# SDFIdk/malstroem

Measured on AMD Instinct MI355X. Metric: Mcells/s fill->D8->accum->label on 16384^2 f32 DEM, higher is better.
Workload: dtype f32 fill / f64 no-flats+D8+accum / u8 flowdir / i32 labels; 1 GPU; 16384x16384 float32 DEM (spectral fBm beta=2 seed 42 (SURVEY 8d recipe)): fill+depths -> no-flats fill -> D8 -> accumulation -> CCL+label_stats -> watersheds+label_count -> pour points; parallelism=1 GPU, one device context, fill_rounds=8, noflat_rounds=85, fill_tiles=70225, fill_visits=43659, fill_cycles=0, noflat_visits=409461, noflat_cycles=409461, nlabels=4637017, fill_algorithm=1, fill_launches=8, noflat_algorithm=2, pour_algorithm=1

## Files before the change

### malstroem_amd/csrc/accum.hip

```cpp
#include "common.hpp"
#include <type_traits>

namespace mh {
namespace {

constexpr int AT = 64;
constexpr int PERIM = 4 * AT - 4;
constexpr int NODE_STRIDE = 256;
constexpr int FS = AT + 32;
constexpr int WOFF = 16;
constexpr uint64_t SRC = 1ull << 63;
constexpr uint64_t TAINT = 1ull << 63;
constexpr uint32_t TAINT32 = 1u << 31;
constexpr int R_SHIFT = 13;
constexpr uint32_t A_MASK = 0x1fffu, R_MASK = 0xfffu, SENT13 = A_MASK;
constexpr uint16_t NO_EXIT = 0xffffu;
#ifndef ACC_ATN
#define ACC_ATN 256
#endif
constexpr int ATN = ACC_ATN;
constexpr int CPT = AT * AT / ATN;
constexpr int MAX_DOUBLINGS = 12;
constexpr int G_SHIFT = 44;
constexpr uint64_t G_ONE = 1ull << G_SHIFT, G_SUM = G_ONE - 1, G_PEND = 0x7ffffull;
// ... 581 lines not shown
{
    const int tile = blockIdx.x;
    if (!touched[tile]) return;
    __shared__ unsigned long long S[AT * AT];
    __shared__ uint16_t P[AT * AT];
    __shared__ uint32_t wl_cell[PERIM + AT * 2];
    __shared__ unsigned long long wl_add[PERIM + AT * 2];
    __shared__ uint32_t wl_n;
    const int ti = tile / ntc, tj = tile - ti * ntc;
    const int64_t r0 = (int64_t)ti * AT, c0 = (int64_t)tj * AT;
    const int tid = threadIdx.x;
    auto halo_row = [&](int64_t rr) { return (fixed_top && rr == 0) || (fixed_bot && rr == H - 1); };
    if (tid == 0) wl_n = 0;
    for (int i = tid; i < AT * AT; i += ATN) {
        const int r = i / AT, c = i - r * AT;
        const int64_t rr = r0 + r, cc = c0 + c;
        const bool inside = rr < H && cc < W;
        const bool owned = inside && !halo_row(rr);
        const double own = owned ? out[rr * W + cc] : 0.0;
        S[i] = own > 0.0 ? (unsigned long long)own : 0ull;
        uint16_t nx = (uint16_t)SENT13;
        const unsigned code = inside ? fd[rr * W + cc] : 8u;
        if (owned && code <= 7u) {
            const int nr = r + dir_dr((int)code), nc = c + dir_dc((int)code);
            if (nr >= 0 && nr < AT && nc >= 0 && nc < AT && (r0 + nr) < H && (c0 + nc) < W && !halo_row(r0 + nr)) nx = (uint16_t)(nr * AT + nc);
        }
        P[i] = nx;
    }
    __syncthreads();
    if (tid < PERIM) {
        const unsigned long long d = nd.inflow[(int64_t)tile * NODE_STRIDE + tid];
        int r, c;
        perim_cell(tid, r, c);
        if (d != 0ull && (r0 + r) < H && (c0 + c) < W && !halo_row(r0 + r)) {
            const uint32_t kk = atomicAdd(&wl_n, 1u);
            wl_cell[kk] = (uint32_t)(r * AT + c);
            wl_add[kk] = d;
        }
    }
    for (int side = 0; side < 2; ++side) {
        const int64_t hr = side == 0 ? 0 : H - 1;
        if ((side == 0 ? !fixed_top : !fixed_bot) || hr < r0 || hr >= r0 + AT) continue;
        if (tid < AT && c0 + tid < W) {
            const int r = (int)(hr - r0), c = tid;
            const unsigned code = fd[hr * W + c0 + c];
            const double X = out[hr * W + c0 + c];
            if (code <= 7u && dir_dr((int)code) != 0 && X > 0.0) {
                const int nr = r + dir_dr((int)code), nc = c + dir_dc((int)code);
                if (nr >= 0 && nr < AT && nc >= 0 && nc < AT && (r0 + nr) < H && (c0 + nc) < W && !halo_row(r0 + nr)) {
                    const uint32_t kk = atomicAdd(&wl_n, 1u);
                    wl_cell[kk] = (uint32_t)(nr * AT + nc);
                    wl_add[kk] = (unsigned long long)X;
                }
            }
        }
    }
    __syncthreads();
    const uint32_t nw = wl_n;
    for (uint32_t w = tid; w < nw; w += ATN) {
        uint32_t a = wl_cell[w];
        const unsigned long long v = wl_add[w];
        do {
            if (S[a] == 0ull) break;
            atomicAdd(&S[a], v);
            a = P[a];
        } while (a != SENT13);
    }
    __syncthreads();
    for (int i = tid; i < AT * AT; i += ATN) {
        const int r = i / AT, c = i - r * AT;
        const int64_t rr = r0 + r, cc = c0 + c;
        if (rr < H && cc < W && !halo_row(rr)) out[rr * W + cc] = (double)S[i];
    }
}
}

int accum_band_delta_dev(const uint8_t *d_fd, double *d_out, int64_t H, int64_t W, hipStream_t s, int fixed_top, int fixed_bot, AccumKeep *keep, bool *done)
{
    *done = false;
    if (!keep || !keep->valid || keep->H != H || keep->W != W || keep->fixed_top != fixed_top || keep->fixed_bot != fixed_bot || !keep->nodes.p) return MHIP_OK;
    static const bool off = [] { const char *e = dev_env("MHIP_BAND_ACC"); return e && std::string(e) == "full"; }();
    if (off) return MHIP_OK;
    const int ntr = (int)cdiv(H, AT), ntc = (int)cdiv(W, AT);
    const int64_t ntiles = (int64_t)ntr * ntc, nnodes = ntiles * NODE_STRIDE;
    char *b = keep->nodes.as<char>();
    Nodes nd;
    nd.gstate = reinterpret_cast<uint64_t *>(b + keep->o[0]);
    nd.inflow = reinterpret_cast<uint64_t *>(b + keep->o[1]);
    nd.arrived = reinterpret_cast<uint32_t *>(b + keep->o[2]);
    nd.next = reinterpret_cast<int32_t *>(b + keep->o[3]);
    nd.dst = reinterpret_cast<int32_t *>(b + keep->o[4]);
    nd.exit_of = reinterpret_cast<uint16_t *>(b + keep->o[5]);
    nd.flags = reinterpret_cast<uint8_t *>(b + keep->o[6]);
    nd.halo_first = reinterpret_cast<int32_t *>(b + keep->o[7]);
    nd.bexit = reinterpret_cast<int32_t *>(b + keep->o[8]);
    DevBuf aux;
    MH_TRY(aux.alloc((size_t)ntiles + 64));
    uint8_t *touched = aux.as<uint8_t>() + 64;
    unsigned int *flag = aux.as<unsigned int>();
    MH_HIP(hipMemsetAsync(aux.p, 0, (size_t)ntiles + 64, s));
    MH_HIP(hipMemsetAsync(nd.inflow, 0, 8 * (size_t)nnodes, s));
    hipLaunchKernelGGL(accum_delta_graph_kernel, dim3((unsigned)cdiv(2 * W, 256)), dim3(256), 0, s, nd, d_fd, (const double *)d_out, H, W, ntc, ntiles, fixed_top,
                       fixed_bot, touched, flag);
    MH_HIP(hipGetLastError());
    unsigned int h_flag = 0;
    MH_HIP(hipMemcpyAsync(&h_flag, flag, 4, hipMemcpyDeviceToHost, s));
    MH_HIP(stream_sync(s));
    keep->valid = false;
    if (h_flag) return MHIP_OK;
    hipLaunchKernelGGL(accum_delta_tile_kernel, dim3((unsigned)ntiles), dim3(ATN), 0, s, d_fd, d_out, H, W, ntc, nd, fixed_top, fixed_bot, (const uint8_t *)touched);
    MH_HIP(hipGetLastError());
    MH_HIP(stream_sync(s));
    *done = true;
    return MHIP_OK;
}

namespace {
struct NodeLayout {
    size_t o_gstate, o_inflow, o_arrived, o_next, o_dst, o_exit, o_flags, o_halo, o_bexit, bytes;
    NodeLayout(int64_t nnodes, int64_t W, bool exit_map)
    {
        auto align = [](size_t x) { return (x + 255) & ~size_t(255); };
        o_gstate = 0; o_inflow = align(o_gstate + 8 * (size_t)nnodes); o_arrived = align(o_inflow + 8 * (size_t)nnodes);
        o_next = align(o_arrived + 4 * (size_t)nnodes); o_dst = align(o_next + 4 * (size_t)nnodes);
        o_exit = align(o_dst + 4 * (size_t)nnodes); o_flags = align(o_exit + 2 * (size_t)nnodes);
        o_halo = align(o_flags + (size_t)nnodes);
        o_bexit = align(o_halo + (exit_map ? 8 * (size_t)W : 0));
        bytes = o_bexit + (exit_map ? 4 * (size_t)nnodes : 0);
    }
};
inline int64_t accum_nodes(int64_t H, int64_t W) { return cdiv(H, AT) * cdiv(W, AT) * NODE_STRIDE; }
}

AccumPrep::~AccumPrep()
{
    if (valid && ready) (void)hipEventSynchronize(ready);
}

int accum_prepare_dev(AccumPrep *prep, int64_t H, int64_t W, hipStream_t s, hipEvent_t ready)
{
    prep->valid = false;
    const int64_t nnodes = accum_nodes(H, W);
    if (nnodes >= (int64_t)INT32_MAX || H * W >= (1ll << 37)) return MHIP_OK;
    const NodeLayout L(nnodes, W, false);
    MH_TRY(prep->nodes.alloc(L.bytes));
    MH_HIP(hipMemsetAsync(prep->nodes.as<char>() + L.o_inflow, 0, L.o_next - L.o_inflow, s));
    MH_HIP(hipEventRecord(ready, s));
    prep->ready = ready; prep->H = H; prep->W = W;
    prep->valid = true;
    return MHIP_OK;
}

int accum_dev(const uint8_t *d_fd, double *d_out, int64_t H, int64_t W, hipStream_t s, int fixed_top, int fixed_bot, int halo_zero,
              int32_t *d_exit_map, PourLink *pour, AccumKeep *keep, AccumPrep *prep)
{
    const int ntr = (int)cdiv(H, AT), ntc = (int)cdiv(W, AT);
    const int64_t ntiles = (int64_t)ntr * ntc, nnodes = ntiles * NODE_STRIDE;
    if (nnodes >= (int64_t)INT32_MAX || H * W >= (1ll << 37)) {
        set_error("accumulated_flow: raster too large for the int32 perimeter-node domain");
        return MHIP_ELIMIT;
    }
    DevBuf buf;
    const NodeLayout L(nnodes, W, d_exit_map != nullptr);
    const size_t o_gstate = L.o_gstate, o_inflow = L.o_inflow, o_arrived = L.o_arrived, o_next = L.o_next, o_dst = L.o_dst, o_exit = L.o_exit,
                 o_flags = L.o_flags, o_halo = L.o_halo, o_bexit = L.o_bexit;
    const bool prepared = prep && prep->valid && prep->H == H && prep->W == W && !d_exit_map && !keep;
    if (prepared) {
        buf.p = prep->nodes.p; buf.bytes = prep->nodes.bytes;
        prep->nodes.p = nullptr; prep->nodes.bytes = 0;
        prep->valid = false;
        MH_HIP(hipStreamWaitEvent(s, prep->ready, 0));
    } else
        MH_TRY(buf.alloc(L.bytes));
    char *b = buf.as<char>();
    Nodes nd;
    nd.gstate = reinterpret_cast<uint64_t *>(b + o_gstate);
    nd.inflow = reinterpret_cast<uint64_t *>(b + o_inflow);
    nd.arrived = reinterpret_cast<uint32_t *>(b + o_arrived);
    nd.next = reinterpret_cast<int32_t *>(b + o_next);
    nd.dst = reinterpret_cast<int32_t *>(b + o_dst);
    nd.exit_of = reinterpret_cast<uint16_t *>(b + o_exit);
    nd.flags = reinterpret_cast<uint8_t *>(b + o_flags);
    nd.halo_first = d_exit_map ? reinterpret_cast<int32_t *>(b + o_halo) : nullptr;
    nd.bexit = d_exit_map ? reinterpret_cast<int32_t *>(b + o_bexit) : nullptr;
    if (d_exit_map) MH_HIP(hipMemsetAsync(nd.halo_first, 0xff, 8 * (size_t)W, s));
    if (!prepared) MH_HIP(hipMemsetAsync(nd.inflow, 0, o_next - o_inflow, s));
    const unsigned gn = (unsigned)cdiv(nnodes, 256);
    const bool walk_final = (!(fixed_top || fixed_bot) || halo_zero) && (!d_exit_map || halo_zero) && H * W < (int64_t)0x7fffffff;
    if (walk_final)
        hipLaunchKernelGGL((accum_tile_kernel<false, false, true>), dim3((unsigned)ntiles), dim3(ATN), 0, s, d_fd, d_out, H, W, ntc, nd, fixed_top, fixed_bot, halo_zero);
    else if ((fixed_top || fixed_bot) && !halo_zero)
        hipLaunchKernelGGL((accum_tile_kernel<false, true>), dim3((unsigned)ntiles), dim3(ATN), 0, s, d_fd, d_out, H, W, ntc, nd, fixed_top, fixed_bot, halo_zero);
    else
        hipLaunchKernelGGL((accum_tile_kernel<false, false>), dim3((unsigned)ntiles), dim3(ATN), 0, s, d_fd, d_out, H, W, ntc, nd, fixed_top, fixed_bot, halo_zero);
    hipLaunchKernelGGL(accum_link_kernel, dim3(gn), dim3(256), 0, s, nd, nnodes);
    if (d_exit_map)
        hipLaunchKernelGGL(accum_band_exit_kernel, dim3((unsigned)cdiv(2 * W, 256)), dim3(256), 0, s, nd, H, W, ntc, ntiles, fixed_top, fixed_bot, d_exit_map);
    hipLaunchKernelGGL(accum_mark_kernel, dim3(gn), dim3(256), 0, s, nd, nnodes);
    hipLaunchKernelGGL(accum_graph_walk_kernel, dim3(gn), dim3(256), 0, s, nd, nnodes);
    if (walk_final) {
        PourCandDev pc;
        if (pour && pour->wait && pour->wait(pour->arg) == 1 && pour->dev.key) {
            MH_HIP(hipStreamWaitEvent(s, pour->ev, 0));
            pc = pour->dev;
            pour->consumed = true;
        }
        hipLaunchKernelGGL(accum_final_walk_kernel, dim3((unsigned)ntiles), dim3(ATN), 0, s, d_fd, d_out, H, W, ntc, nd, pc, fixed_top, fixed_bot);
    }
    else if ((!(fixed_top || fixed_bot) || halo_zero) && H * W < (int64_t)0x7fffffff)
        hipLaunchKernelGGL((accum_tile_kernel<true, false>), dim3((unsigned)ntiles), dim3(ATN), 0, s, d_fd, d_out, H, W, ntc, nd, fixed_top, fixed_bot, halo_zero);
    else
        hipLaunchKernelGGL((accum_tile_kernel<true, true>), dim3((unsigned)ntiles), dim3(ATN), 0, s, d_fd, d_out, H, W, ntc, nd, fixed_top, fixed_bot, halo_zero);
    MH_HIP(hipGetLastError());
    MH_HIP(stream_sync(s));
    if (keep) {
        keep->valid = false;
        if (d_exit_map) {
            keep->nodes.release();
            keep->nodes.p = buf.p; keep->nodes.bytes = buf.bytes;
            buf.p = nullptr; buf.bytes = 0;
            const size_t offs[9] = {o_gstate, o_inflow, o_arrived, o_next, o_dst, o_exit, o_flags, o_halo, o_bexit};
            for (int k = 0; k < 9; ++k) keep->o[k] = offs[k];
            keep->H = H; keep->W = W; keep->fixed_top = fixed_top; keep->fixed_bot = fixed_bot;
            keep->valid = true;
        }
    }
#ifdef MH_PROFILE_ACCUM
    {
        unsigned long long pr[2][8];
        MH_HIP(hipMemcpyFromSymbol(pr, HIP_SYMBOL(g_accum_prof), sizeof(pr)));
        for (int f = 0; f < 2; ++f)
            fprintf(stderr, "[accum profile phase %d] ticks/tile (thread 0): load=%.0f init=%.0f solve=%.0f publish/write=%.0f\n", f ? 3 : 1,
                    pr[f][0] / (double)ntiles, pr[f][1] / (double)ntiles, pr[f][2] / (double)ntiles, pr[f][3] / (double)ntiles);
        unsigned long long z[2][8] = {};
        MH_HIP(hipMemcpyToSymbol(HIP_SYMBOL(g_accum_prof), z, sizeof(z)));
    }
#endif
    return MHIP_OK;
}

}
```

### malstroem_amd/csrc/common.hpp

```cpp
#pragma once
#include <hip/hip_runtime.h>
#include <cstdint>
#include <cstdio>
#include <cstring>
#include <string>
#include <vector>

#include "../../include/malstroem_hip.h"

struct mhip_polygons;
struct mhip_flowpaths;

namespace mh {

void set_error(const char *fmt, ...);
const char *get_error();
const char *dev_env(const char *name);
hipError_t stream_sync(hipStream_t s);
int require_device();

#define MH_HIP(expr)                                                                             \
    do {                                                                                         \
        hipError_t _e = (expr);                                                                  \
        if (_e != hipSuccess) {                                                                  \
            mh::set_error("%s failed: %s (%s:%d)", #expr, hipGetErrorString(_e), __FILE__, __LINE__); \
            return MHIP_EHIP;                                                                    \
        }                                                                                        \
    } while (0)

#define MH_TRY(expr)                \
    do {                            \
        int _rc = (expr);           \
        if (_rc != MHIP_OK) return _rc; \
    } while (0)

#define MH_ARG(cond, msg)                   \
    do {                                    \
        if (!(cond)) {                      \
            mh::set_error("invalid argument: %s", msg); \
            return MHIP_EINVAL;             \
        }                                   \
    } while (0)

int pool_alloc(void **p, size_t bytes);
void pool_free(void *p, size_t bytes);

struct DevBuf {
    void *p = nullptr;
    size_t bytes = 0;
    DevBuf() = default;
    DevBuf(const DevBuf &) = delete;
    DevBuf &operator=(const DevBuf &) = delete;
    ~DevBuf() { release(); }
    int alloc(size_t n)
    {
        if (n == 0) n = 16;
        if (p && bytes >= n && bytes <= 2 * n + 4096) return MHIP_OK;
        release();
        MH_TRY(pool_alloc(&p, n));
        bytes = n;
        return MHIP_OK;
    }
    void release()
    {
        if (p) pool_free(p, bytes);
        p = nullptr;
        bytes = 0;
    }
    template <typename T> T *as() const { return reinterpret_cast<T *>(p); }
};

int upload(DevBuf &b, const void *host, size_t bytes, hipStream_t s);
int download(void *host, const DevBuf &b, size_t bytes, hipStream_t s);
int64_t build_rank_lut(const uint8_t *keep, int64_t nlab, std::vector<int32_t> &lut);
inline bool hyps_res_ok(double res) { return res > 0.0 && res <= 1.7976931348623157e308; }
int trace_on_device(const uint8_t *d_fd, const int32_t *d_lab, int64_t H, int64_t W, const int64_t *cells_rc, int64_t n, int use_bg,
                    int32_t bg, int32_t *out_label, int32_t *out_found, int64_t *out_len, const int64_t *offsets, int64_t *out_cells,
                    hipStream_t s);

__host__ __device__ inline int dir_dr(int k) { return (k == 0 || k == 1 || k == 7) ? -1 : (k >= 3 && k <= 5) ? 1 : 0; }
__host__ __device__ inline int dir_dc(int k) { return (k >= 1 && k <= 3) ? 1 : (k >= 5 && k <= 7) ? -1 : 0; }

__device__ __forceinline__ unsigned d8_code(double z, double u, double ur, double r, double dr, double d, double dl,
                                            double l, double ul)
{
    const double INV_SQRT2 = 0.7071067811865475;
    unsigned i = 8;
    double dzmax = 0.0, dz;
#define MH_D8_STEP(expr, k)          \
    dz = (expr);                     \
    i = dz > dzmax ? (k) : i;        \
    dzmax = fmax(dzmax, dz);
    MH_D8_STEP(__dsub_rn(z, u), 0u)
    MH_D8_STEP(__dmul_rn(__dsub_rn(z, ur), INV_SQRT2), 1u)
    MH_D8_STEP(__dsub_rn(z, r), 2u)
    MH_D8_STEP(__dmul_rn(__dsub_rn(z, dr), INV_SQRT2), 3u)
    MH_D8_STEP(__dsub_rn(z, d), 4u)
    MH_D8_STEP(__dmul_rn(__dsub_rn(z, dl), INV_SQRT2), 5u)
    MH_D8_STEP(__dsub_rn(z, l), 6u)
    MH_D8_STEP(__dmul_rn(__dsub_rn(z, ul), INV_SQRT2), 7u)
#undef MH_D8_STEP
    return i;
}

__device__ __forceinline__ unsigned edge_code(int64_t r, int64_t c, int64_t maxr, int64_t maxc)
{
    unsigned code = 8;
    if (r == 0) code = 0;
    if (r == maxr) code = 4;
    if (c == 0) code = 6;
    if (c == maxc) code = 2;
    if (r == 0 && c == 0) code = 7;
    if (r == 0 && c == maxc) code = 1;
    if (r == maxr && c == 0) code = 5;
    if (r == maxr && c == maxc) code = 3;
    return code;
}

__host__ __device__ inline uint32_t f32_key(float f)
{
    uint32_t u;
    memcpy(&u, &f, 4);
    return (u & 0x80000000u) ? ~u : (u | 0x80000000u);
}
__host__ __device__ inline float key_f32(uint32_t k)
{
    uint32_t u = (k & 0x80000000u) ? (k & 0x7fffffffu) : ~k;
    float f;
    memcpy(&f, &u, 4);
    return f;
}
__device__ __forceinline__ uint32_t dem_key(float v)
{
    if (v != v) return f32_key(__builtin_inff());
    return f32_key(v + 0.0f);
}
__host__ __device__ inline uint64_t f64_key(double f)
{
    uint64_t u;
    memcpy(&u, &f, 8);
    return (u & 0x8000000000000000ull) ? ~u : (u | 0x8000000000000000ull);
}
__host__ __device__ inline double key_f64(uint64_t k)
{
    uint64_t u = (k & 0x8000000000000000ull) ? (k & 0x7fffffffffffffffull) : ~k;
    double f;
    memcpy(&f, &u, 8);
    return f;
}

struct FillStats {
    int32_t rounds = 0;
    int64_t visits = 0;
    int64_t cycles = 0;
    int64_t tiles = 0;
    float hot_ms = 0;
    int32_t hot_launches = 0;
    int32_t algorithm = 0;
    uint32_t overflow = 0;
    bool have_minmax = false, dem_nan = false;
    float dem_min = 0.0f, dem_max = 0.0f;
    int32_t geo_reject = 0;
    int64_t geo_irregular = 0, geo_unreached = 0, geo_mismatch = 0;
};

struct FillRun {
    bool noflat = false;
    const float *dem = nullptr;
    void *out = nullptr;
    int64_t H = 0, W = 0;
    double sh = 0, dg = 0;
    const float *seed = nullptr;
    double seed_add = 0;
    int fixed_top = 0, fixed_bot = 0;
    int rounds_per_batch = 8;
    bool attach_only = false;
    struct Impl;
    Impl *impl;
    FillRun();
    ~FillRun();
    FillRun(const FillRun &) = delete;
    FillRun &operator=(const FillRun &) = delete;
    int begin(hipStream_t s, bool *active);
    int batch(hipStream_t s, bool *active);
    int activate_row(int side, hipStream_t s);
    int attach(hipStream_t s);
    int certify(hipStream_t s, bool *changed);
    int finish(hipStream_t s, FillStats *st);
};
void noflat_seed(FillRun &f, const float *d_filled, double sh, double dg, int64_t ncells_global);
struct PfRun;
struct FillHandover {
    PfRun *run = nullptr;
    const float *dem = nullptr;
    float *filled = nullptr, *depths = nullptr;
    int64_t H = 0, W = 0;
    const uint16_t *bslot = nullptr;
    const uint32_t *tabV = nullptr;
    int ntr = 0, ntc = 0;
    bool pending = false, queued = false, violated = false, repaired = false;
    bool suspect = false;
    FillStats st_repair;
    FillHandover() = default;
    FillHandover(const FillHandover &) = delete;
    FillHandover &operator=(const FillHandover &) = delete;
    ~FillHandover();
    void release();
};
int fill_handover_complete(FillHandover *ho, hipStream_t s);
int fill_handover_repair(FillHandover *ho, hipStream_t s);
int fill_plain_dev(const float *d_dem, float *d_out, int64_t H, int64_t W, hipStream_t s, FillStats *st, float *d_depths = nullptr,
                   bool *depths_done = nullptr, FillHandover *ho = nullptr);
int fill_check_f32_dev(const float *d_dem, const float *d_filled, int64_t H, int64_t W, int fixed_top, int fixed_bot, hipStream_t s,
                       unsigned int *d_flag);
int fill_plain_pflood_dev(const float *d_dem, float *d_out, float *d_depths, int64_t H, int64_t W, hipStream_t s, FillStats *st, bool *violated = nullptr,
                          uint32_t *overflow = nullptr, FillHandover *ho = nullptr);
struct PfRun {
    const float *dem = nullptr;
    float *out = nullptr;
    int64_t H = 0, W = 0;
    int fixed_top = 0, fixed_bot = 0;
    uint32_t overflow = 0;
    struct Impl;
    Impl *impl;
    PfRun();
    ~PfRun();
    PfRun(const PfRun &) = delete;
    PfRun &operator=(const PfRun &) = delete;
    int begin(hipStream_t s);
    int halo_changed(int side, hipStream_t s);
    int batch(hipStream_t s);
    int finish(hipStream_t s, float *d_depths, FillStats *st, bool *violated = nullptr, FillHandover *ho = nullptr);
    int finish_late(hipStream_t s, float *d_depths, bool *violated);
    int proof_flag(hipStream_t s, unsigned int *h_flag);
    int solve(hipStream_t s);
    int pack(hipStream_t s, int row0, int nrows);
    int publish_edges(hipStream_t s);
};
struct StageHook {
    enum Point { FIRST_VISIT = 0, TAIL_ROUNDS = 1, FINISH = 3 };
    void (*fn)(void *, hipStream_t) = nullptr;
    void *arg = nullptr;
    bool fired = false;
    int at = TAIL_ROUNDS;
    void fire(hipStream_t s)
    {
        if (fn && !fired) {
            fired = true;
            fn(arg, s);
        }
    }
    void fire_at(int point, hipStream_t s)
    {
        if (point == at) fire(s);
    }
};

struct GeoRun {
    const float *dem = nullptr, *filled = nullptr;
    double *out = nullptr;
    uint32_t *dist = nullptr;
    int64_t H = 0, W = 0;
    double sh = 0, dg = 0;
    int fixed_top = 0, fixed_bot = 0;
    bool allow_partial = false;
    double seed_add = 0;
    bool partial = false;
    StageHook *tail_hook = nullptr;
    uint8_t *d8_out = nullptr;
    unsigned int *d8_nodir = nullptr;
    bool d8_done = false;
    bool defer_out = false;
    bool out_deferred = false;
    FillHandover *handover = nullptr;
    struct Impl;
    Impl *impl;
    GeoRun();
    ~GeoRun();
    GeoRun(const GeoRun &) = delete;
    GeoRun &operator=(const GeoRun &) = delete;
    int begin(hipStream_t s, bool *applicable, bool *active);
    int batch(hipStream_t s, bool *active);
    int halo_changed(int side, hipStream_t s);
    int end(hipStream_t s, bool *ok, FillStats *st);
    int launch_rounds(hipStream_t s, int nb);
};
struct D8Sink {
    uint8_t *flowdir = nullptr;
    unsigned int *nodir = nullptr;
    bool done = false;
    uint32_t *dist = nullptr;
    bool defer = false, deferred = false;
};
int noflat_assemble_dev(const float *d_filled, const uint32_t *d_dist, double *d_out, int64_t n, double seed_add, hipStream_t s);
int fill_noflat_geodesic_dev(const float *d_dem, const float *d_filled, double *d_out, int64_t H, int64_t W, double sh, double dg, double seed_add,
                             hipStream_t s, FillStats *st, bool *partial, StageHook *tail_hook = nullptr, D8Sink *d8 = nullptr, FillHandover *ho = nullptr);
int noflat_verify_dev(const float *d_dem, const double *d_out, int64_t H, int64_t W, double sh, double dg, hipStream_t s, bool *ok, int fixed_top = 0,
                      int fixed_bot = 0);
int fill_noflat_dev(const float *d_dem, double *d_out, int64_t H, int64_t W, double sh, double dg, hipStream_t s,
                    FillStats *st = nullptr, const float *d_filled = nullptr, StageHook *tail_hook = nullptr, D8Sink *d8 = nullptr,
                    FillHandover *ho = nullptr);
int short_diag_dev(const float *d_dem, int64_t n, double *sh, double *dg, hipStream_t s);
int depths_dev(const float *d_filled, const float *d_dem, float *d_out, int64_t n, hipStream_t s);
int d8_dev(const double *d_z, uint8_t *d_out, int64_t H, int64_t W, int edges_outward, hipStream_t s, int64_t row_off = 0,
           int64_t Hg = 0, unsigned int *d_interior_nodir = nullptr);
void short_diag_from_minmax(float mn, float mx, bool has_nan, double *sh, double *dg);
int minmax_dev(const float *d_x, int64_t n, float *mn, float *mx, int *has_nan, hipStream_t s);
int row_update_dev(void *d_dst, const void *d_src, int64_t nbytes, int *changed, hipStream_t s);
int copy_bandwidth_dev(size_t bytes, int reps, double *gbs, hipStream_t s);
int read_bandwidth_dev(size_t bytes, int reps, double *gbs, hipStream_t s);
int row_update_async(void *d_dst, const void *d_src, int64_t nbytes, int *d_changed, hipStream_t s);
int trace_downstream_dev(const uint8_t *d_fd, const int32_t *d_lab, int64_t H, int64_t W, const int64_t *d_cells, int64_t n, int use_bg,
                         int32_t bg, int32_t *d_label, int32_t *d_found, int64_t *d_len, const int64_t *d_offsets, int64_t *d_out_cells,
                         hipStream_t s);
int comm_unique_id(void *id128);
int comm_available();
int comm_create(void **comm, const void *id128, int rank, int nranks);
void comm_destroy(void *comm);
int comm_exchange_rows(void *comm, int rank, int nranks, const void *first_row, const void *last_row, void *stage, size_t rowbytes,
                       hipStream_t s);
int comm_allreduce_max(void *comm, double *d_value, hipStream_t s);
struct PourCandDev {
    uint16_t *mask0 = nullptr;
    uint2 *list = nullptr;
    uint32_t *tile_cnt = nullptr;
    unsigned long long *tile_key0 = nullptr;
    uint32_t *flags = nullptr;
    int components = 0;
    unsigned long long *key = nullptr;
    uint32_t nlab = 0;
};
constexpr uint32_t POUR_TILE_CAP = 512;
struct PourLink {
    PourCandDev dev;
    hipEvent_t ev = nullptr;
    void (*notify)(void *, int) = nullptr;
    int (*wait)(void *) = nullptr;
    void *arg = nullptr;
    bool consumed = false;
};
struct AccumKeep {
    DevBuf nodes;
    size_t o[9] = {};
    int64_t H = 0, W = 0;
    int fixed_top = 0, fixed_bot = 0;
    bool valid = false;
};
struct AccumPrep {
    DevBuf nodes;
    int64_t H = 0, W = 0;
    hipEvent_t ready = nullptr;
    bool valid = false;
    ~AccumPrep();
};
int accum_prepare_dev(AccumPrep *prep, int64_t H, int64_t W, hipStream_t s, hipEvent_t ready);
int accum_dev(const uint8_t *d_fd, double *d_out, int64_t H, int64_t W, hipStream_t s, int fixed_top = 0, int fixed_bot = 0, int halo_zero = 0,
              int32_t *d_exit_map = nullptr, PourLink *pour = nullptr, AccumKeep *keep = nullptr, AccumPrep *prep = nullptr);
int accum_band_delta_dev(const uint8_t *d_fd, double *d_out, int64_t H, int64_t W, hipStream_t s, int fixed_top, int fixed_bot, AccumKeep *keep, bool *done);
int ccl8_f32_dev(const float *d_data, int32_t *d_labels, int32_t *d_tmp, int64_t H, int64_t W, int64_t *nlabels,
                 hipStream_t s, DevBuf *stats_out = nullptr);
int label_emit_stats_dev(const int32_t *d_parent, const unsigned long long *d_rootbits, const uint32_t *d_wordprefix, const float *d_data,
                         int32_t *d_labels, int64_t H, int64_t W, int64_t nlab, mhip_stat_record *d_rec, hipStream_t s);
int ccl8_u8_dev(const uint8_t *d_data, int32_t *d_labels, int32_t *d_tmp, int64_t H, int64_t W, int64_t *nlabels,
                hipStream_t s);
struct CclKeep {
    DevBuf bits, wprefix;
    int64_t H = 0, W = 0, nlocal = 0;
    bool valid = false;
};
int ccl8_f32_begin_dev(const float *d_data, int32_t *d_labels, int32_t *d_tmp, int64_t H, int64_t W, int64_t *nlabels, hipStream_t s, CclKeep *keep);
int ccl_emit_rows_dev(const int32_t *d_parent, const unsigned long long *d_rootbits, const uint32_t *d_wordprefix, int32_t *d_labels, int64_t base,
                      int64_t count, hipStream_t s);
int label_emit_sparse_dev(const int32_t *d_parent, const unsigned long long *d_rootbits, const uint32_t *d_wordprefix, const float *d_data,
                          int32_t *d_labels, int64_t H, int64_t W, int ht, int64_t H_owned, int64_t nlocal, int32_t offset,
                          const int32_t *d_dropped, const int32_t *d_target, int32_t ndropped, int64_t nlab_global, mhip_stat_record *d_rec,
                          hipStream_t s);
int relabel_lut_dev(int32_t *d_labels, const int32_t *d_lut, int64_t nlab, int64_t n, hipStream_t s);
int relabel_range_dev(int32_t *d_labels, int64_t n, int32_t lo, int32_t hi, const int32_t *d_lut, const int32_t *d_fid, const int32_t *d_fnew, int32_t nf,
                      hipStream_t s);
int band_trace_dev(const uint8_t *d_fd, const int32_t *d_lab, int64_t Hl, int64_t W, int64_t row_lo, int64_t own0, int64_t own1, int64_t Hg,
                   const int64_t *d_cells, const int32_t *d_src, int64_t n, int use_bg, int32_t bg, int32_t *d_label, int32_t *d_status,
                   int32_t *d_src_out, int64_t *d_exit, int64_t *d_len, const int64_t *d_offsets, int64_t *d_out_cells, hipStream_t s);
int relabel_sparse_dev(int32_t *d_labels, int64_t n, int64_t nlocal, int32_t offset, const int32_t *d_dropped, const int32_t *d_target,
                       int32_t ndropped, hipStream_t s);
int keep_mask_dev(const int32_t *d_labels, const uint8_t *d_keep, int64_t nlab, int64_t n, uint8_t *d_mask,
                  hipStream_t s);
int label_stats_dev(const float *d_data, const int32_t *d_labels, int64_t n, int64_t nlab, mhip_stat_record *d_rec,
                    hipStream_t s, int64_t W = 0, bool components = false);
int label_stats64_dev(const double *d_data, const int32_t *d_labels, int64_t n, int64_t nlab, mhip_stat_record *d_rec, hipStream_t s);
int label_stats_zero_sign_dev(const float *d_data, const int32_t *d_labels, int64_t n, int64_t nlab, mhip_stat_record *d_rec, hipStream_t s);
int label_stats_zero_sign_dev(const double *d_data, const int32_t *d_labels, int64_t n, int64_t nlab, mhip_stat_record *d_rec, hipStream_t s);
int label_arg_dev(const double *d_data, const int32_t *d_labels, int64_t H, int64_t W, int64_t nlab, bool is_max,
                  mhip_index_record *d_rec, hipStream_t s, bool components = false);
int label_count_dev(const int32_t *d_labels, int64_t n, int64_t nlab, int64_t *d_counts, hipStream_t s, int64_t W = 0);
int label_max_dev(const int32_t *d_labels, int64_t n, int32_t *out_max, hipStream_t s);
constexpr int64_t HYPS_MAX_BINS = (int64_t)1 << 30;
int hyps_layout_dev(const double *d_dmax, int64_t stride, int64_t nlab, double res, int64_t *d_offsets, int64_t *total, hipStream_t s);
int hyps_table_dev(const float *d_data, const int32_t *d_labels, int64_t n, int64_t W, int64_t nlab, double res, const int64_t *d_offsets,
                   int64_t total, uint32_t *d_counts, double *d_sums, int64_t *lds_spills, hipStream_t s, hipEvent_t ev0 = nullptr,
                   hipEvent_t ev1 = nullptr);
int hyps_levels_dev(int64_t nlab, const int64_t *d_offsets, const uint32_t *d_counts, const double *d_sums, const double *d_dmax, int64_t stride,
                    const double *d_q, mhip_final_record *d_rec, hipStream_t s);
int final_depths_dev(const float *d_data, const int32_t *d_labels, int64_t n, int64_t W, int64_t nlab, mhip_final_record *d_rec, float *d_out,
                     hipStream_t s, hipEvent_t ev0 = nullptr, hipEvent_t ev1 = nullptr);
bool wet_at_events_ok(int64_t K, const float *values);
int wet_at_dev(const float *d_data, const int32_t *d_labels, int64_t n, int64_t W, int64_t nlab, int K, const double *d_drawdown, int64_t stride,
               const float *values, float *d_out, int64_t *d_wet, int64_t wet_stride, hipStream_t s, hipEvent_t ev0 = nullptr,
               hipEvent_t ev1 = nullptr);
bool flow_distance_scale_ok(double scale);
int flow_distance_dev(const uint8_t *d_fd, const int32_t *d_lab, int64_t H, int64_t W, double scale, int64_t nlab, float *d_out, mhip_index_record *d_rec,
                      int64_t *unresolved, hipStream_t s);
int fdist_jumps_dev(uint4 *&cur, uint4 *&nxt, int64_t W, int64_t ntc, int64_t ntiles, unsigned int *d_open, hipStream_t s);
int hand_check(double threshold, double scale);
int hand_dev(const uint8_t *d_fd, const double *d_acc, const float *d_elev, const int32_t *d_lab, int64_t H, int64_t W, double threshold, double scale,
             float nodata, float *d_hand, float *d_dist, int64_t *undrained, hipStream_t s);
int burn_check(int64_t nseg, const mhip_burn_segment *segs, int64_t nline, const mhip_burn_line *lines, const mhip_burn_result *results);
int burn_lines_dev(float *d_dem, int64_t H, int64_t W, int64_t nseg, const mhip_burn_segment *segs, int64_t nline, const mhip_burn_line *lines,
                   double nodata, mhip_burn_result *results, hipStream_t s);
int zones_check(int64_t H, int64_t W, int64_t nvert, const double *xy, int64_t nring, const int64_t *ring_offsets, const int32_t *ring_zone,
                int64_t nzone, int grow);
int zones_rasterize_dev(int32_t *d_out, int64_t H, int64_t W, int64_t nvert, const double *xy, int64_t nring, const int64_t *ring_offsets,
                        const int32_t *ring_zone, int64_t nzone, int grow, hipStream_t s);
int zone_stats_dev(const float *d_data, const int32_t *d_zones, int64_t n, int64_t W, int64_t nzone, mhip_zone_record *d_rec, hipStream_t s);
int polygonize_check(int64_t H, int64_t W);
int polygons_fetch_dev(const mhip_polygons *p, int32_t *xy, int64_t *ring_offsets, int32_t *ring_label);
int polygonize_dev(const int32_t *d_lab, int64_t H, int64_t W, DevBuf &d_xy, DevBuf &d_off, DevBuf &d_rl, int64_t *nring, int64_t *nvert, hipStream_t s);
int flowpaths_check(int64_t H, int64_t W, double threshold);
int flowpaths_dev(const uint8_t *d_fd, const double *d_acc, const int32_t *d_lab, int64_t H, int64_t W, double threshold, mhip_flowpaths *p, hipStream_t s);
int flowpaths_fetch_dev(const mhip_flowpaths *p, int32_t *xy, int64_t *reach_offsets, mhip_reach_record *records);
int watersheds_dev(const uint8_t *d_fd, int32_t *d_labels, int64_t H, int64_t W, int32_t unassigned, hipStream_t s,
                   bool band_mode = false, const unsigned int *d_known_interior_nodir = nullptr, const int32_t *d_src = nullptr, PourLink *pour = nullptr);
int pour_finish_dev(unsigned long long *d_key, const unsigned long long *d_tile_key0, int64_t ntiles, int64_t nlab, int64_t W, mhip_index_record *d_rec,
                    hipStream_t s);
int band_pseudo_labels_dev(int32_t *d_ws, int64_t H, int64_t W, int top, int bottom, hipStream_t s);
int negative_lut_dev(int32_t *d_lab, int64_t n, const int32_t *d_lut, int64_t nlut, hipStream_t s);
constexpr int32_t BAND_ROOT = 1, BAND_ROOTLESS = 0x7fffffff;
int band_root_labels_dev(int32_t *d_out, int64_t H, int64_t W, int64_t row_off, int64_t Hg, hipStream_t s);
int band_hide_rootless_dev(const int32_t *d_lab, const int32_t *d_rooted, int32_t *d_out, int64_t n, hipStream_t s);
int band_show_rootless_dev(int32_t *d_ws, const int32_t *d_lab, int64_t n, hipStream_t s);

__host__ __device__ inline int64_t cdiv(int64_t a, int64_t b) { return (a + b - 1) / b; }

constexpr int TR = 32;
struct TileGeom {
    int64_t n, W;
    int64_t ntr, ntc;
};
__host__ __device__ inline TileGeom tile_geom(int64_t n, int64_t W)
{
    TileGeom g;
    g.n = n;
    g.W = (W > 0 && n % W == 0) ? W : 256;
    const int64_t H = cdiv(n, g.W);
    g.ntr = cdiv(H, TR);
    g.ntc = cdiv(g.W, 256);
    return g;
}
inline unsigned tile_grid(const TileGeom &g)
{
    const int64_t nt = g.ntr * g.ntc;
    return (unsigned)(nt < 2048 ? (nt > 0 ? nt : 1) : 2048);
}

#ifdef __HIPCC__
__device__ __forceinline__ int64_t downstream(const uint8_t *fd, int64_t i, int64_t H, int64_t W)
{
    const unsigned code = fd[i];
    if (code > 7u) return -1;
    const int64_t r = i / W, c = i - r * W;
    const int64_t nr = r + dir_dr((int)code), nc = c + dir_dc((int)code);
    if (nr < 0 || nr >= H || nc < 0 || nc >= W) return -1;
    return nr * W + nc;
}
constexpr int WS_TILE = 64;
__device__ __forceinline__ int ws_perim_slot(int lr, int lc)
{
    if (lr == 0) return lc;
    if (lr == WS_TILE - 1) return WS_TILE + lc;
    if (lc == 0) return 2 * WS_TILE + (lr - 1);
    if (lc == WS_TILE - 1) return 2 * WS_TILE + (WS_TILE - 2) + (lr - 1);
    return -1;
}
__device__ __forceinline__ int64_t ws_node_of(int32_t cell, uint32_t W, int ntc)
{
    const uint32_t r = (uint32_t)cell / W, c = (uint32_t)cell - r * W;
    const int slot = ws_perim_slot((int)(r & 63u), (int)(c & 63u));
    return slot < 0 ? -1 : (int64_t)((r >> 6) * (uint32_t)ntc + (c >> 6)) * 256 + slot;
}

constexpr int32_t FD_NONE = 0x7fffffff;
constexpr int32_t FD_DONE = (int32_t)0x80000000;
constexpr double FD_SQRT2 = 1.4142135623730951;
__device__ __forceinline__ uint32_t fd_step(unsigned code) { return (code & 1u) ? 0x10000u : 1u; }
__device__ __forceinline__ bool fd_resolve(uint2 s, const uint4 *__restrict__ Nn, uint32_t W, int ntc, uint32_t &no, uint32_t &nd, int32_t &T)
{
    int32_t t = (int32_t)s.x;
    no = s.y & 0xffffu;
    nd = s.y >> 16;
    if (t >= 0 && t != FD_NONE) {
        const int64_t node = ws_node_of(t, W, ntc);
        uint4 m = make_uint4((uint32_t)FD_NONE, 0u, 0u, 0u);
        if (node >= 0) m = Nn[node];
        t = (int32_t)m.x;
        no += m.y;
        nd += m.z;
    }
    T = t & ~FD_DONE;
    return t < 0;
}
__device__ __forceinline__ double fd_u(uint32_t no, uint32_t nd) { return __dadd_rn((double)no, __dmul_rn((double)nd, FD_SQRT2)); }
// ... 53 lines not shown
```

### malstroem_amd/csrc/ctx.hip

```cpp
#include <mutex>
#include <new>
#include <string>
#include <vector>

#include "ctx.hpp"

namespace mh {

static void drop_hyps(mhip_ctx *c)
{
    c->hyps_total = -1;
    c->have[MHIP_R_FINALDEPTHS] = false;
    c->wetat_events = -1;
    c->wetat_out.release();
}

static void drop_flow_distance(mhip_ctx *c)
{
    std::lock_guard<std::mutex> lk(c->fdist_mu);
    c->fdist_unresolved = -1;
    c->fdist_out.release();
    c->fdist_rec.release();
}

// ... 55 lines not shown
        break;
    }
}

int ctx_copy_rows(mhip_ctx *c, void *dev_base, size_t elem_bytes, int64_t row0, int64_t nrows, void *host, hipMemcpyKind kind)
{
    MH_HIP(hipSetDevice(c->device));
    const size_t rowb = elem_bytes * (size_t)c->W;
    char *dev = (char *)dev_base + rowb * (size_t)(c->ht + row0);
    const bool up = kind == hipMemcpyHostToDevice;
    MH_HIP(hipMemcpyAsync(up ? (void *)dev : host, up ? host : (void *)dev, rowb * (size_t)nrows, kind, cs(c)));
    MH_HIP(stream_sync(cs(c)));
    return MHIP_OK;
}

int ctx_noflat(mhip_ctx *c, double **g)
{
    if (c->noflat_pending) {
        MH_HIP(hipSetDevice(c->device));
        MH_TRY(noflat_assemble_dev(c->r[MHIP_R_FILLED].as<float>(), c->r[MHIP_R_NGDIST].as<uint32_t>(), c->r[MHIP_R_NOFLAT].as<double>(), c->H * c->W, 0.0,
                                   c->stream));
        c->noflat_pending = false;
        if (cs(c) != c->stream) MH_HIP(stream_sync(c->stream));
    }
    if (g) *g = c->r[MHIP_R_NOFLAT].as<double>();
    return MHIP_OK;
}

int ctx_fetch(mhip_ctx *c, const DevBuf &buf, size_t bytes, void *host)
{
    MH_HIP(hipSetDevice(c->device));
    return download(host, buf, bytes, c->stream);
}

int ctx_fork_join_events(mhip_ctx *c)
{
    if (c->ev_fork) return MHIP_OK;
    for (hipEvent_t *e : {&c->ev_flowdir, &c->ev_join, &c->ev_label, &c->ev_tail, &c->ev_fork}) MH_HIP(hipEventCreateWithFlags(e, hipEventDisableTiming));
    return MHIP_OK;
}

int ctx_ensure_labels_final(mhip_ctx *c, hipStream_t s)
{
    if (!c->labels_filtered) return ctx_apply_keep_on(c, nullptr, s);
    return MHIP_OK;
}

int ctx_label_max(mhip_ctx *c, hipStream_t s)
{
    if (c->nlabels < 0) {
        int32_t m = 0;
        MH_TRY(label_max_dev(c->r[MHIP_R_LABELS].as<int32_t>(), c->H * c->W, &m, s));
        c->nlabels = m < 0 ? 0 : m;
    }
    return MHIP_OK;
}

int ctx_apply_keep_on(mhip_ctx *c, const uint8_t *keep, hipStream_t s)
{
    MH_ARG(c && c->have[MHIP_R_LABELS] && c->nlabels_raw >= 0 && !c->labels_filtered, "ctx_apply_keep needs a fresh LABEL run");
    const int64_t n = c->H * c->W;
    const int64_t nraw = c->nlabels_raw;
    const bool components = c->labels_components;
    ctx_wrote(c, MHIP_R_LABELS);
    c->nlabels_raw = nraw;
    c->labels_components = components;
    if (keep) {
        std::vector<int32_t> lut;
        c->nlabels = build_rank_lut(keep, c->nlabels_raw, lut);
        DevBuf d_lut;
        MH_TRY(d_lut.alloc(lut.size() * 4));
        MH_HIP(hipMemcpyAsync(d_lut.p, lut.data(), lut.size() * 4, hipMemcpyHostToDevice, s));
        MH_TRY(relabel_lut_dev(c->r[MHIP_R_LABELS].as<int32_t>(), d_lut.as<int32_t>(), c->nlabels_raw, n, s));
        MH_TRY(c->stats.alloc(sizeof(mhip_stat_record) * (size_t)(c->nlabels + 1)));
        MH_TRY(label_stats_dev(c->r[MHIP_R_DEPTHS].as<float>(), c->r[MHIP_R_LABELS].as<int32_t>(), n, c->nlabels,
                               c->stats.as<mhip_stat_record>(), s, c->W, c->labels_components));
    } else {
        c->nlabels = c->nlabels_raw;
        MH_TRY(c->stats.alloc(sizeof(mhip_stat_record) * (size_t)(c->nlabels + 1)));
        MH_HIP(hipMemcpyAsync(c->stats.p, c->raw_stats.p, sizeof(mhip_stat_record) * (size_t)(c->nlabels + 1),
                              hipMemcpyDeviceToDevice, s));
    }
    c->labels_filtered = true;
    c->stats_valid = true;
    return MHIP_OK;
}

}

using namespace mh;

extern "C" {

int mhip_comm_available(void) { return comm_available(); }

int mhip_comm_unique_id(void *id128)
{
    MH_ARG(id128, "comm_unique_id(id128)");
    MH_TRY(require_device());
    return comm_unique_id(id128);
}

int mhip_ctx_create_band(mhip_ctx **out, int64_t H_global, int64_t W, int64_t row0, int64_t H_local, int device, int rank,
                         int nranks, const void *nccl_unique_id)
{
    MH_ARG(out && H_global >= 1 && W >= 1 && H_local >= 1 && row0 >= 0 && row0 + H_local <= H_global, "ctx_create_band geometry");
    MH_ARG(rank >= 0 && nranks >= 1 && rank < nranks, "ctx_create_band(rank, nranks)");
    MH_TRY(require_device());
    MH_HIP(hipSetDevice(device));
    void *comm = nullptr;
    if (nccl_unique_id) MH_TRY(comm_create(&comm, nccl_unique_id, rank, nranks));
    mhip_ctx *c = new mhip_ctx();
    c->comm = comm;
    c->ht = row0 > 0 ? 1 : 0;
    c->hb = row0 + H_local < H_global ? 1 : 0;
    c->H_owned = H_local;
    c->H = H_local + c->ht + c->hb;
    c->W = W; c->H_global = H_global; c->row0 = row0;
    c->device = device; c->rank = rank; c->nranks = nranks;
    int prio_least = 0, prio_greatest = 0;
    (void)hipDeviceGetStreamPriorityRange(&prio_least, &prio_greatest);
    if (hipStreamCreateWithPriority(&c->stream, hipStreamDefault, prio_greatest) != hipSuccess) {
        comm_destroy(c->comm);
        delete c;
        set_error("hipStreamCreate failed");
        return MHIP_EHIP;
    }
    *out = c;
    return MHIP_OK;
}

int mhip_ctx_create(mhip_ctx **out, int64_t H, int64_t W, int device)
{
    return mhip_ctx_create_band(out, H, W, 0, H, device, 0, 1, nullptr);
}

int mhip_ctx_destroy(mhip_ctx *c)
{
    if (!c) return MHIP_OK;
    (void)hipSetDevice(c->device);
    (void)stream_sync(c->stream);
    for (StageTimer &t : c->timers)
        for (hipEvent_t e : {t.a, t.b})
            if (e) (void)hipEventDestroy(e);
    (void)hipStreamDestroy(c->stream);
    for (hipStream_t st : {c->stream_b, c->stream_c}) {
        if (st) {
            (void)stream_sync(st);
            (void)hipStreamDestroy(st);
        }
    }
    for (hipEvent_t e : {c->ev_fork, c->ev_flowdir, c->ev_join, c->ev_label, c->ev_tail, c->ev_cand, c->ev_prep})
        if (e) (void)hipEventDestroy(e);
    delete c->geo;
    delete c->pf;
    delete c->run[0];
    delete c->run[1];
    comm_destroy(c->comm);
    comm_destroy(c->comm_b);
    delete c;
    return MHIP_OK;
}

int mhip_ctx_comm_add_side(mhip_ctx *c, const void *nccl_unique_id)
{
    MH_ARG(c && nccl_unique_id && c->comm && !c->comm_b, "ctx_comm_add_side(ctx, id) needs a band context with a communicator and no side communicator yet");
    MH_HIP(hipSetDevice(c->device));
    return comm_create(&c->comm_b, nccl_unique_id, c->rank, c->nranks);
}

int mhip_ctx_side_begin(mhip_ctx *c)
{
    MH_ARG(c, "ctx");
    MH_HIP(hipSetDevice(c->device));
    if (!c->stream_b) MH_HIP(hipStreamCreateWithFlags(&c->stream_b, hipStreamNonBlocking));
    MH_TRY(ctx_fork_join_events(c));
    MH_HIP(hipEventRecord(c->ev_fork, c->stream));
    MH_HIP(hipStreamWaitEvent(c->stream_b, c->ev_fork, 0));
    t_side_ctx = c;
    return MHIP_OK;
}

int mhip_ctx_side_end(mhip_ctx *c)
{
    MH_ARG(c && t_side_ctx == c, "ctx_side_end without ctx_side_begin on this thread");
    MH_HIP(hipSetDevice(c->device));
    MH_HIP(stream_sync(c->stream_b));
    t_side_ctx = nullptr;
    return MHIP_OK;
}

int mhip_ctx_upload(mhip_ctx *c, int which, const void *host)
{
    MH_ARG(c && host && which >= 0 && which < MHIP_R_COUNT_, "ctx_upload(ctx, which, host)");
    return mhip_ctx_upload_rows(c, which, 0, c->H_owned, host);
}

int mhip_ctx_upload_dem(mhip_ctx *c, const float *dem) { return mhip_ctx_upload(c, MHIP_R_DEM, dem); }

int mhip_ctx_upload_rows(mhip_ctx *c, int which, int64_t row0, int64_t nrows, const void *host)
{
    MH_ARG(c && host && which >= 0 && which < MHIP_R_COUNT_ && row0 >= 0 && nrows >= 1 && row0 + nrows <= c->H_owned,
           "ctx_upload_rows(ctx, which, row0, nrows, host)");
    MH_HIP(hipSetDevice(c->device));
    MH_TRY(ctx_raster(c, which));
    MH_TRY(ctx_settle(c, which, true));
    ctx_wrote(c, which, true);
    c->have[which] = false;
    MH_TRY(ctx_copy_rows(c, c->r[which].p, raster_elem(which), row0, nrows, const_cast<void *>(host), hipMemcpyHostToDevice));
    if (row0 + nrows == c->H_owned) {
        c->have[which] = true;
        if (which == MHIP_R_LABELS) c->labels_filtered = true;
    }
    return MHIP_OK;
}

int mhip_ctx_download_rows(mhip_ctx *c, int which, int64_t row0, int64_t nrows, void *host)
{
    MH_ARG(c && host && which >= 0 && which < MHIP_R_COUNT_ && row0 >= 0 && nrows >= 1 && row0 + nrows <= c->H_owned,
           "ctx_download_rows(ctx, which, row0, nrows, host)");
    MH_ARG(c->have[which], "raster has not been computed or uploaded");
    MH_TRY(ctx_settle(c, which, false));
    return ctx_copy_rows(c, c->r[which].p, raster_elem(which), row0, nrows, host, hipMemcpyDeviceToHost);
}

int mhip_ctx_download(mhip_ctx *c, int which, void *host)
{
    MH_ARG(c && host && which >= 0 && which < MHIP_R_COUNT_, "ctx_download(ctx, which, host)");
    return mhip_ctx_download_rows(c, which, 0, c->H_owned, host);
}

int mhip_ctx_trace_downstream(mhip_ctx *c, const int64_t *cells_rc, int64_t n, int use_background, int32_t background, int32_t *out_label,
                              int32_t *out_found, int64_t *out_len, const int64_t *offsets, int64_t *out_cells)
{
    MH_ARG(c && n >= 0 && (n == 0 || cells_rc), "ctx_trace_downstream(ctx, cells, n, ...)");
    MH_ARG(c->have[MHIP_R_FLOWDIR] && c->have[MHIP_R_LABELS], "ctx_trace_downstream needs flow directions and labels");
    MH_ARG(!c->ht && !c->hb, "stream tracing runs on an undivided raster");
    if (n == 0) return MHIP_OK;
    MH_HIP(hipSetDevice(c->device));
    return trace_on_device(c->r[MHIP_R_FLOWDIR].as<uint8_t>(), c->r[MHIP_R_LABELS].as<int32_t>(), c->H, c->W, cells_rc, n, use_background,
                           background, out_label, out_found, out_len, offsets, out_cells, c->stream);
}

int mhip_ctx_sync(mhip_ctx *c)
{
    MH_ARG(c, "ctx");
    MH_HIP(stream_sync(c->stream));
    return MHIP_OK;
}

int mhip_ctx_stage_ms(mhip_ctx *c, int stage, float *ms)
{
    MH_ARG(c && ms, "ctx_stage_ms(ctx, stage, ms)");
    const int k = timer_slot(stage);
    MH_ARG(k >= 0 && c->timers[k].valid, "stage has not been run");
    MH_HIP(hipEventSynchronize(c->timers[k].b));
    MH_HIP(hipEventElapsedTime(ms, c->timers[k].a, c->timers[k].b));
    return MHIP_OK;
}

int mhip_ctx_kernel_ms(mhip_ctx *c, const char *kernel, float *ms_total, int32_t *launches)
{
    MH_ARG(c && kernel && ms_total && launches, "ctx_kernel_ms(ctx, kernel, ms, launches)");
    const std::string k(kernel);
    if (k == "d8") {
        *launches = 1;
        return mhip_ctx_stage_ms(c, MHIP_STAGE_FLOWDIR, ms_total);
    }
    if (k == "d8_steady") {
        MH_ARG(c->have[MHIP_R_NOFLAT] && !c->ht && !c->hb, "d8_steady needs the no-flats surface on an undivided context");
        MH_HIP(hipSetDevice(c->device));
        double *g = nullptr;
        MH_TRY(ctx_noflat(c, &g));
        MH_TRY(ctx_raster(c, MHIP_R_FLOWDIR));
        MH_TRY(c->nodir_cnt.alloc(4));
        constexpr int REPS = 16;
        StageTimer *t;
        MH_TRY(ctx_timer(c, D8_STEADY_SLOT, &t));
        hipStream_t s = c->stream;
        ctx_wrote(c, MHIP_R_FLOWDIR);
        MH_HIP(hipMemsetAsync(c->nodir_cnt.p, 0, 4, s));
        for (int i = 0; i < REPS + 2; ++i) {
            if (i == 2) MH_HIP(hipEventRecord(t->a, s));
            MH_TRY(d8_dev(g, c->r[MHIP_R_FLOWDIR].as<uint8_t>(), c->H, c->W, 1, s, 0, c->H_global, c->nodir_cnt.as<unsigned int>()));
        }
        MH_HIP(hipEventRecord(t->b, s));
        MH_HIP(hipEventSynchronize(t->b));
        MH_HIP(hipEventElapsedTime(ms_total, t->a, t->b));
        c->have[MHIP_R_FLOWDIR] = true;
        c->nodir_valid = true;
        c->flowdir_own = true;
        *launches = REPS;
        return MHIP_OK;
    }
    if (k == "hyps_table" || k == "final_depths") {
        *launches = 1;
        return mhip_ctx_stage_ms(c, k == "hyps_table" ? HYPS_KERNEL_SLOT : FINAL_KERNEL_SLOT, ms_total);
    }
    if (k == "wet_at") {
        *launches = 1;
        return mhip_ctx_stage_ms(c, WETAT_KERNEL_SLOT, ms_total);
    }
    if (k == "fill_round") {
        *launches = c->fill_rounds;
        return mhip_ctx_stage_ms(c, MHIP_STAGE_FILL, ms_total);
    }
    if (k == "noflat_round") {
        *launches = c->noflat_rounds;
        return mhip_ctx_stage_ms(c, MHIP_STAGE_NOFLAT, ms_total);
    }
    set_error("unknown kernel family '%s'", kernel);
    return MHIP_EINVAL;
}

int mhip_ctx_get_i64(mhip_ctx *c, const char *key, int64_t *value)
{
    MH_ARG(c && key && value, "ctx_get_i64(ctx, key, value)");
    const std::string k(key);
    if (k == "nlabels_raw") *value = c->nlabels_raw;
    else if (k == "nlabels") {
        if (c->nlabels < 0 && c->have[MHIP_R_LABELS]) {
            MH_HIP(hipSetDevice(c->device));
            MH_TRY(ctx_label_max(c, c->stream));
        }
        *value = c->nlabels;
    }
    else if (k == "fill_rounds") *value = c->fill_rounds;
    else if (k == "noflat_rounds") *value = c->noflat_rounds;
    else if (k == "fill_visits") *value = c->fill_st.visits;
    else if (k == "fill_cycles") *value = c->fill_st.cycles;
    else if (k == "fill_tiles") *value = c->fill_st.tiles;
    else if (k == "fill_algorithm") *value = c->fill_st.algorithm;
    else if (k == "fill_handover") *value = c->fill_handover;
    else if (k == "fill_handover_rechecks") *value = c->fill_handover_rechecks;
    else if (k == "fill_overflow") *value = c->fill_st.overflow;
    else if (k == "fill_launches") *value = c->fill_st.rounds;
    else if (k == "fill_hot_launches") *value = c->fill_st.hot_launches;
    else if (k == "noflat_hot_launches") *value = c->noflat_st.hot_launches;
    else if (k == "accum_algorithm") *value = c->accum_algorithm;
    else if (k == "flowdir_computed") *value = (c->have[MHIP_R_FLOWDIR] && c->flowdir_own) ? 1 : 0;
    else if (k == "pour_algorithm") *value = c->pour_algorithm;
    else if (k == "noflat_algorithm") *value = c->noflat_st.algorithm;
    else if (k == "noflat_pending") *value = c->noflat_pending ? 1 : 0;
    else if (k == "noflat_visits") *value = c->noflat_st.visits;
    else if (k == "noflat_reject") *value = c->noflat_st.geo_reject;
    else if (k == "noflat_reject_irregular") *value = c->noflat_st.geo_irregular;
    else if (k == "noflat_reject_unreached") *value = c->noflat_st.geo_unreached;
    else if (k == "noflat_reject_mismatch") *value = c->noflat_st.geo_mismatch;
    else if (k == "noflat_cycles") *value = c->noflat_st.cycles;
    else if (k == "hyps_bins") *value = c->hyps_total;
    else if (k == "hyps_lds_spills") *value = c->hyps_spills;
    else if (k == "wet_at_events") *value = c->wetat_events;
    else if (k == "flow_distance_unresolved") *value = c->fdist_unresolved;
    else if (k == "hand_undrained") *value = c->hand_undrained;
    else if (k == "zones") *value = c->nzone;
    else if (k == "H") *value = c->H;
    else if (k == "W") *value = c->W;
    else {
        set_error("unknown key '%s'", key);
        return MHIP_EINVAL;
    }
    return MHIP_OK;
}

int mhip_ctx_get_f64(mhip_ctx *c, const char *key, double *value)
{
    MH_ARG(c && key && value, "ctx_get_f64(ctx, key, value)");
    const std::string k(key);
    if (k == "short") *value = c->sh;
    else if (k == "diag") *value = c->dg;
    else if (k == "fill_hot_ms") *value = c->fill_st.hot_ms;
    else if (k == "noflat_hot_ms") *value = c->noflat_st.hot_ms;
    else {
        set_error("unknown key '%s'", key);
        return MHIP_EINVAL;
    }
    return MHIP_OK;
}

int mhip_ctx_raw_stats(mhip_ctx *c, mhip_stat_record *records)
{
    MH_ARG(c && records && c->raw_stats.p && c->nlabels_raw >= 0, "ctx_raw_stats needs a LABEL run");
    return ctx_fetch(c, c->raw_stats, sizeof(mhip_stat_record) * (size_t)(c->nlabels_raw + 1), records);
}

int mhip_ctx_apply_keep(mhip_ctx *c, const uint8_t *keep)
{
    MH_ARG(c, "ctx");
    MH_HIP(hipSetDevice(c->device));
    return ctx_apply_keep_on(c, keep, c->stream);
}

int mhip_ctx_stats(mhip_ctx *c, mhip_stat_record *records)
{
    MH_ARG(c && records && c->stats_valid && c->labels_filtered, "ctx_stats needs LABEL + apply_keep (or mhip_ctx_hyps) on the resident depths and labels");
    return ctx_fetch(c, c->stats, sizeof(mhip_stat_record) * (size_t)(c->nlabels + 1), records);
}

int mhip_ctx_watershed_counts(mhip_ctx *c, int64_t *counts)
{
    MH_ARG(c && counts && c->ws_counts_valid, "ctx_watershed_counts needs a WATERSHED run on the resident labels");
    return ctx_fetch(c, c->ws_counts, 8 * (size_t)(c->nlabels + 1), counts);
}

int mhip_ctx_pourpoints(mhip_ctx *c, mhip_index_record *records)
{
    MH_ARG(c && records && c->pour_valid, "ctx_pourpoints needs a POURPOINTS run on the resident labels and accumulated flow");
    return ctx_fetch(c, c->pour, sizeof(mhip_index_record) * (size_t)(c->nlabels + 1), records);
}

int mhip_ctx_hyps(mhip_ctx *c, double res, int64_t *total)
{
    MH_ARG(c && total && hyps_res_ok(res), "ctx_hyps(ctx, 0 < res < inf, total)");
    MH_ARG(!(c->nranks > 1 || c->ht || c->hb), "hypsometry on a row band is not built (the tables of the bands add up: a later step); use an undivided context");
    MH_ARG(c->have[MHIP_R_DEPTHS] && c->have[MHIP_R_LABELS] && !c->ccl_pending, "ctx_hyps needs the DEPTHS and LABELS rasters");
    MH_ARG(c->labels_filtered, "ctx_hyps needs mhip_ctx_apply_keep after the LABEL run");
    MH_HIP(hipSetDevice(c->device));
    hipStream_t s = c->stream;
    const int64_t n = c->H * c->W;
    c->hyps_total = -1;
    if (!c->stats_valid) {
        MH_TRY(ctx_label_max(c, s));
        MH_TRY(c->stats.alloc(sizeof(mhip_stat_record) * (size_t)(c->nlabels + 1)));
        MH_TRY(label_stats_dev(c->r[MHIP_R_DEPTHS].as<float>(), c->r[MHIP_R_LABELS].as<int32_t>(), n, c->nlabels, c->stats.as<mhip_stat_record>(), s,
                               c->W, c->labels_components));
        c->stats_valid = true;
    }
    const int64_t nlab = c->nlabels;
    MH_TRY(c->hyps_off.alloc(8 * (size_t)(nlab + 2)));
    StageTimer *k;
    MH_TRY(ctx_timer(c, HYPS_KERNEL_SLOT, &k));
    MH_TRY(stage_begin(c, MHIP_STAGE_HYPS, s));
    int64_t tot = 0;
    MH_TRY(hyps_layout_dev(c->stats.as<double>() + 1, 4, nlab, res, c->hyps_off.as<int64_t>(), &tot, s));
    MH_TRY(c->hyps_cnt.alloc(4 * (size_t)tot));
    MH_TRY(c->hyps_sum.alloc(8 * (size_t)tot));
    MH_TRY(hyps_table_dev(c->r[MHIP_R_DEPTHS].as<float>(), c->r[MHIP_R_LABELS].as<int32_t>(), n, c->W, nlab, res, c->hyps_off.as<int64_t>(), tot,
                          c->hyps_cnt.as<uint32_t>(), c->hyps_sum.as<double>(), &c->hyps_spills, s, k->a, k->b));
    MH_TRY(stage_end(c, MHIP_STAGE_HYPS, s));
    k->valid = true;
    c->hyps_total = tot;
    *total = tot;
    return MHIP_OK;
}

int mhip_ctx_hyps_fetch(mhip_ctx *c, int64_t *offsets, int64_t *counts, double *sums)
{
    MH_ARG(c && offsets && counts && sums, "ctx_hyps_fetch(ctx, offsets, counts, sums)");
    MH_ARG(c->hyps_total >= 0, "ctx_hyps_fetch needs mhip_ctx_hyps on the resident depths and labels");
    MH_HIP(hipSetDevice(c->device));
    hipStream_t s = c->stream;
    const size_t tot = (size_t)c->hyps_total;
    std::vector<uint32_t> c32(tot + 1);
    MH_HIP(hipMemcpyAsync(offsets, c->hyps_off.p, 8 * (size_t)(c->nlabels + 2), hipMemcpyDeviceToHost, s));
    if (tot) {
        MH_HIP(hipMemcpyAsync(c32.data(), c->hyps_cnt.p, 4 * tot, hipMemcpyDeviceToHost, s));
        MH_HIP(hipMemcpyAsync(sums, c->hyps_sum.p, 8 * tot, hipMemcpyDeviceToHost, s));
    }
    MH_HIP(stream_sync(s));
    for (size_t k = 0; k < tot; ++k) counts[k] = (int64_t)c32[k];
    return MHIP_OK;
}

int mhip_ctx_final_depths(mhip_ctx *c, const double *q, mhip_final_record *records)
{
    MH_ARG(c && q && records, "ctx_final_depths(ctx, q, records)");
    MH_ARG(c->hyps_total >= 0 && c->stats_valid, "ctx_final_depths needs mhip_ctx_hyps on the resident depths and labels");
    MH_HIP(hipSetDevice(c->device));
    hipStream_t s = c->stream;
    const int64_t nlab = c->nlabels, n = c->H * c->W;
    DevBuf d_q;
    MH_TRY(upload(d_q, q, 8 * (size_t)(nlab + 1), s));
    MH_TRY(c->hyps_rec.alloc(sizeof(mhip_final_record) * (size_t)(nlab + 1)));
    MH_TRY(ctx_raster(c, MHIP_R_FINALDEPTHS));
    c->have[MHIP_R_FINALDEPTHS] = false;
    StageTimer *k;
    MH_TRY(ctx_timer(c, FINAL_KERNEL_SLOT, &k));
    MH_TRY(stage_begin(c, MHIP_STAGE_FINALDEPTHS, s));
    MH_TRY(hyps_levels_dev(nlab, c->hyps_off.as<int64_t>(), c->hyps_cnt.as<uint32_t>(), c->hyps_sum.as<double>(), c->stats.as<double>() + 1, 4,
                           d_q.as<double>(), c->hyps_rec.as<mhip_final_record>(), s));
    MH_TRY(final_depths_dev(c->r[MHIP_R_DEPTHS].as<float>(), c->r[MHIP_R_LABELS].as<int32_t>(), n, c->W, nlab, c->hyps_rec.as<mhip_final_record>(),
                            c->r[MHIP_R_FINALDEPTHS].as<float>(), s, k->a, k->b));
    MH_TRY(stage_end(c, MHIP_STAGE_FINALDEPTHS, s));
    k->valid = true;
    c->have[MHIP_R_FINALDEPTHS] = true;
    return ctx_fetch(c, c->hyps_rec, sizeof(mhip_final_record) * (size_t)(nlab + 1), records);
}
// ... 230 lines not shown
```

### malstroem_amd/csrc/ctx.hpp

```cpp
#pragma once
#include <atomic>
#include <condition_variable>
#include <functional>
#include <mutex>
#include <thread>

#include "common.hpp"

namespace mh {

class SideThread {
    std::thread th_;
    std::mutex mu_;
    std::condition_variable cv_;
    std::function<void()> task_;
    bool busy_ = false, stop_ = false;

public:
    ~SideThread()
    {
        {
            std::lock_guard<std::mutex> lk(mu_);
            stop_ = true;
        }
        cv_.notify_all();
        if (th_.joinable()) th_.join();
    }
    void run(std::function<void()> f)
    {
        std::unique_lock<std::mutex> lk(mu_);
        if (!th_.joinable())
            th_ = std::thread([this] {
                std::unique_lock<std::mutex> l2(mu_);
                for (;;) {
                    cv_.wait(l2, [this] { return stop_ || (busy_ && task_); });
                    if (stop_) return;
                    std::function<void()> f2 = std::move(task_);
                    task_ = nullptr;
                    l2.unlock();
                    f2();
                    l2.lock();
                    busy_ = false;
                    cv_.notify_all();
                }
            });
        task_ = std::move(f);
        busy_ = true;
        cv_.notify_all();
    }
    void wait()
    {
        std::unique_lock<std::mutex> lk(mu_);
        cv_.wait(lk, [this] { return !busy_; });
    }
};

struct StageTimer {
    hipEvent_t a = nullptr, b = nullptr;
    bool valid = false;
};
constexpr int N_STAGE_BITS = 9;
constexpr int WETAT_KERNEL_SLOT = 1 << 27, FINAL_KERNEL_SLOT = 1 << 28, HYPS_KERNEL_SLOT = 1 << 29, D8_STEADY_SLOT = 1 << 30;
constexpr int N_TIMERS = N_STAGE_BITS + 4;

}

struct mhip_ctx {
    mh::SideThread side;
    int64_t H = 0, W = 0;
    int64_t H_global = 0, row0 = 0, H_owned = 0;
    int ht = 0, hb = 0;
    mh::FillRun *run[2] = {nullptr, nullptr};
    mh::GeoRun *geo = nullptr;
    uint32_t pf_overflow = 0;
    mh::PfRun *pf = nullptr;
    bool pf_done = false;
    mh::DevBuf nodir_cnt;
    bool nodir_valid = false;
    bool flowdir_own = false;
    int device = 0, rank = 0, nranks = 1;
    hipStream_t stream = nullptr;
    mh::DevBuf r[MHIP_R_COUNT_];
    bool have[MHIP_R_COUNT_] = {};
    bool noflat_pending = false;
    mh::DevBuf tmp_i32;
    mh::CclKeep ccl_keep;
    bool ccl_pending = false;
    bool pf_depths = false;
    mh::DevBuf raw_stats, stats, ws_counts, pour;
    mh::AccumKeep acc_keep;
    int accum_algorithm = 0;
    mh::DevBuf pp_mask0, pp_list, pp_tiles, pp_misc, pp_key;
    hipEvent_t ev_cand = nullptr;
    hipEvent_t ev_prep = nullptr;
    int pour_algorithm = 0;
    int64_t nlabels_raw = -1, nlabels = -1;
    bool labels_components = false;
    bool labels_filtered = false;
    std::atomic<bool> stats_valid{false};
    std::atomic<bool> ws_counts_valid{false};
    std::atomic<bool> pour_valid{false};
    mh::DevBuf hyps_off, hyps_cnt, hyps_sum, hyps_rec;
    int64_t hyps_total = -1, hyps_spills = 0;
    mh::DevBuf wetat_out;
    int wetat_events = -1;
    mh::DevBuf fdist_out, fdist_rec;
    std::atomic<int64_t> fdist_unresolved{-1};
    std::mutex fdist_mu;
    mh::DevBuf hand_out, hand_dist;
    std::atomic<int64_t> hand_undrained{-1};
    int hand_src = -1;
    bool hand_labels = false;
    std::mutex hand_mu;
    mh::DevBuf zones;
    int64_t nzone = -1;
    double sh = 0, dg = 0;
    int32_t fill_rounds = 0, noflat_rounds = 0;
    int64_t fill_handover_rechecks = 0;
    int32_t fill_handover = 0;
    mh::FillStats fill_st, noflat_st;
    mh::StageTimer timers[mh::N_TIMERS];
    void *comm = nullptr;
    void *comm_b = nullptr;
    mh::DevBuf comm_stage, comm_word, comm_flags, comm_stage_b;
    hipStream_t stream_b = nullptr, stream_c = nullptr;
    hipEvent_t ev_fork = nullptr, ev_flowdir = nullptr, ev_join = nullptr, ev_label = nullptr, ev_tail = nullptr;
};

namespace mh {

inline size_t raster_elem(int which)
{
    switch (which) {
    case MHIP_R_DEM: case MHIP_R_FILLED: case MHIP_R_DEPTHS: case MHIP_R_LABELS: case MHIP_R_WATERSHEDS: case MHIP_R_NGDIST:
    case MHIP_R_FINALDEPTHS: return 4;
    case MHIP_R_NOFLAT: case MHIP_R_ACCUM: return 8;
    case MHIP_R_FLOWDIR: return 1;
    default: return 0;
    }
}

inline int ctx_raster(mhip_ctx *c, int which)
{
    if (!c->r[which].p) MH_TRY(c->r[which].alloc(raster_elem(which) * (size_t)(c->H * c->W)));
    return MHIP_OK;
}

inline int timer_slot(int stage)
{
    for (int b = 0; b < N_STAGE_BITS; ++b)
        if (stage == 1 << b) return b;
    return stage == FINAL_KERNEL_SLOT ? N_STAGE_BITS : stage == HYPS_KERNEL_SLOT ? N_STAGE_BITS + 1 : stage == D8_STEADY_SLOT ? N_STAGE_BITS + 2 :
           stage == WETAT_KERNEL_SLOT ? N_STAGE_BITS + 3 : -1;
}
inline int ctx_timer(mhip_ctx *c, int stage, StageTimer **t)
{
    const int k = timer_slot(stage);
    MH_ARG(k >= 0, "not a stage");
    *t = &c->timers[k];
    if (!(*t)->a) {
        hipEvent_t e0, e1;
        MH_HIP(hipEventCreate(&e0));
        MH_HIP(hipEventCreate(&e1));
        (*t)->a = e0;
        (*t)->b = e1;
    }
    return MHIP_OK;
}
inline int stage_begin(mhip_ctx *c, int stage, hipStream_t s)
{
    StageTimer *t;
    MH_TRY(ctx_timer(c, stage, &t));
    MH_HIP(hipEventRecord(t->a, s));
    return MHIP_OK;
}
inline int stage_end(mhip_ctx *c, int stage, hipStream_t s)
{
    StageTimer &t = c->timers[timer_slot(stage)];
    MH_HIP(hipEventRecord(t.b, s));
    t.valid = true;
    return MHIP_OK;
}

inline thread_local mhip_ctx *t_side_ctx = nullptr;
static inline hipStream_t cs(mhip_ctx *c) { return (t_side_ctx == c && c->stream_b) ? c->stream_b : c->stream; }
static inline bool on_side(mhip_ctx *c) { return t_side_ctx == c; }

void ctx_wrote(mhip_ctx *c, int which, bool uploaded = false);
int ctx_noflat(mhip_ctx *c, double **g = nullptr);
inline int ctx_settle(mhip_ctx *c, int which, bool write)
{
    if (which == MHIP_R_NOFLAT || (write && (which == MHIP_R_FILLED || which == MHIP_R_NGDIST))) return ctx_noflat(c);
    return MHIP_OK;
}
int ctx_copy_rows(mhip_ctx *c, void *dev_base, size_t elem_bytes, int64_t row0, int64_t nrows, void *host, hipMemcpyKind kind);
int ctx_fetch(mhip_ctx *c, const DevBuf &buf, size_t bytes, void *host);
int ctx_fork_join_events(mhip_ctx *c);
int ctx_apply_keep_on(mhip_ctx *c, const uint8_t *keep, hipStream_t s);
int ctx_ensure_labels_final(mhip_ctx *c, hipStream_t s);
int ctx_label_max(mhip_ctx *c, hipStream_t s);

}
```

### malstroem_amd/csrc/ctx_run.hip

```cpp
#include <atomic>
#include <future>
#include <string>

#include "ctx.hpp"

using namespace mh;

constexpr int LABEL_START_DEFAULT = 3;
constexpr int FILL_HANDOVER_DEFAULT = 1;
constexpr int NOFLAT_LAZY_DEFAULT = 1;

static bool fill_handover_env()
{
    const char *e = dev_env("MHIP_FILL_HANDOVER");
    return e ? e[0] != '0' : FILL_HANDOVER_DEFAULT != 0;
}

static bool noflat_lazy_env()
{
    const char *e = dev_env("MHIP_NOFLAT_LAZY");
    return e ? e[0] != '0' : NOFLAT_LAZY_DEFAULT != 0;
}

static int stage_depths(mhip_ctx *c, hipStream_t s)
{
    MH_ARG(c->have[MHIP_R_FILLED] && c->have[MHIP_R_DEM], "depths need the filled surface");
    MH_TRY(ctx_raster(c, MHIP_R_DEPTHS));
    MH_TRY(depths_dev(c->r[MHIP_R_FILLED].as<float>(), c->r[MHIP_R_DEM].as<float>(), c->r[MHIP_R_DEPTHS].as<float>(), c->H * c->W, s));
    ctx_wrote(c, MHIP_R_DEPTHS);
    c->have[MHIP_R_DEPTHS] = true;
    return MHIP_OK;
}

static int stage_fill(mhip_ctx *c, hipStream_t s, bool with_depths = true, FillHandover *ho = nullptr)
{
    const int64_t H = c->H, W = c->W;
    MH_ARG(c->have[MHIP_R_DEM], "FILL needs the DEM");
    MH_TRY(ctx_raster(c, MHIP_R_FILLED));
    MH_TRY(ctx_raster(c, MHIP_R_DEPTHS));
    MH_TRY(stage_begin(c, MHIP_STAGE_FILL, s));
    FillStats st;
    bool depths_done = false;
    MH_TRY(fill_plain_dev(c->r[MHIP_R_DEM].as<float>(), c->r[MHIP_R_FILLED].as<float>(), H, W, s, &st, c->r[MHIP_R_DEPTHS].as<float>(),
                          &depths_done, ho));
    ctx_wrote(c, MHIP_R_FILLED);
    ctx_wrote(c, MHIP_R_DEPTHS);
    const bool owed = ho && ho->pending;
    c->have[MHIP_R_FILLED] = !owed;
    c->have[MHIP_R_DEPTHS] = depths_done && !owed;
    if (with_depths && !depths_done) MH_TRY(stage_depths(c, s));
    MH_TRY(stage_end(c, MHIP_STAGE_FILL, s));
    c->fill_rounds = st.rounds;
    c->fill_st = st;
    return MHIP_OK;
}

static void ctx_handover_settled(mhip_ctx *c, FillHandover *ho)
{
    if (!ho || ho->pending || c->have[MHIP_R_FILLED]) return;
    c->have[MHIP_R_FILLED] = true;
    c->have[MHIP_R_DEPTHS] = true;
    c->fill_handover = ho->queued ? 1 : 0;
    if (ho->suspect) ++c->fill_handover_rechecks;
    if (ho->repaired) {
        c->fill_st.algorithm = 4;
        c->fill_st.rounds += ho->st_repair.rounds;
        c->fill_st.visits += ho->st_repair.visits;
        c->fill_st.cycles += ho->st_repair.cycles;
        c->fill_rounds = c->fill_st.rounds;
    }
}

static int stage_noflat(mhip_ctx *c, hipStream_t s, bool shdg_done = false, StageHook *tail_hook = nullptr, bool with_flowdir = false,
                        bool *flowdir_done = nullptr, FillHandover *ho = nullptr)
{
    const int64_t H = c->H, W = c->W, n = H * W;
    MH_ARG(c->have[MHIP_R_DEM], "NOFLAT needs the DEM");
    MH_TRY(ctx_raster(c, MHIP_R_NOFLAT));
    c->noflat_pending = false;
    MH_TRY(stage_begin(c, MHIP_STAGE_NOFLAT, s));
    if (!shdg_done) {
        if ((c->have[MHIP_R_FILLED] || (ho && ho->pending)) && c->fill_st.have_minmax) short_diag_from_minmax(c->fill_st.dem_min, c->fill_st.dem_max, c->fill_st.dem_nan, &c->sh, &c->dg);
        else MH_TRY(short_diag_dev(c->r[MHIP_R_DEM].as<float>(), n, &c->sh, &c->dg, s));
    }
    FillStats st;
    if (!c->have[MHIP_R_FILLED] && !(ho && ho->pending)) {
        MH_TRY(ctx_raster(c, MHIP_R_FILLED));
        FillStats st0;
        MH_TRY(fill_plain_dev(c->r[MHIP_R_DEM].as<float>(), c->r[MHIP_R_FILLED].as<float>(), H, W, s, &st0));
        ctx_wrote(c, MHIP_R_FILLED);
        c->have[MHIP_R_FILLED] = true;
    }
    D8Sink d8;
    static const bool fuse_d8 = [] { const char *e = dev_env("MHIP_D8_FUSE"); return !(e && e[0] == '0'); }();
    if (with_flowdir && fuse_d8 && !c->ht && !c->hb) {
        MH_TRY(ctx_raster(c, MHIP_R_FLOWDIR));
        MH_TRY(c->nodir_cnt.alloc(4));
        MH_HIP(hipMemsetAsync(c->nodir_cnt.p, 0, 4, s));
        d8.flowdir = c->r[MHIP_R_FLOWDIR].as<uint8_t>();
        d8.nodir = c->nodir_cnt.as<unsigned int>();
        if (c->nranks == 1 && noflat_lazy_env()) {
            MH_TRY(ctx_raster(c, MHIP_R_NGDIST));
            d8.dist = c->r[MHIP_R_NGDIST].as<uint32_t>();
            d8.defer = true;
        }
    }
    const int rc_nf = fill_noflat_dev(c->r[MHIP_R_DEM].as<float>(), c->r[MHIP_R_NOFLAT].as<double>(), H, W, c->sh, c->dg, s, &st,
                                      c->r[MHIP_R_FILLED].as<float>(), tail_hook, d8.flowdir ? &d8 : nullptr, ho);
    ctx_handover_settled(c, ho);
    MH_TRY(rc_nf);
    if (flowdir_done) *flowdir_done = d8.done;
    MH_TRY(stage_end(c, MHIP_STAGE_NOFLAT, s));
    c->noflat_rounds = st.rounds;
    c->noflat_st = st;
    ctx_wrote(c, MHIP_R_NOFLAT);
    c->have[MHIP_R_NOFLAT] = true;
    c->noflat_pending = d8.deferred;
    return MHIP_OK;
}

static int stage_flowdir(mhip_ctx *c, hipStream_t s)
{
    MH_ARG(c->have[MHIP_R_NOFLAT], "FLOWDIR needs the no-flats surface");
    double *g = nullptr;
    MH_TRY(ctx_noflat(c, &g));
    MH_TRY(ctx_raster(c, MHIP_R_FLOWDIR));
    MH_TRY(stage_begin(c, MHIP_STAGE_FLOWDIR, s));
    ctx_wrote(c, MHIP_R_FLOWDIR);
    MH_TRY(c->nodir_cnt.alloc(4));
    MH_HIP(hipMemsetAsync(c->nodir_cnt.p, 0, 4, s));
    MH_TRY(d8_dev(g, c->r[MHIP_R_FLOWDIR].as<uint8_t>(), c->H, c->W, 1, s, c->row0 - c->ht, c->H_global, c->nodir_cnt.as<unsigned int>()));
    MH_TRY(stage_end(c, MHIP_STAGE_FLOWDIR, s));
    c->have[MHIP_R_FLOWDIR] = true;
    c->flowdir_own = true;
    c->nodir_valid = !c->ht && !c->hb;
    return MHIP_OK;
}

static int stage_flowdir_fused(mhip_ctx *c, hipStream_t s)
{
    MH_TRY(stage_begin(c, MHIP_STAGE_FLOWDIR, s));
    MH_TRY(stage_end(c, MHIP_STAGE_FLOWDIR, s));
    ctx_wrote(c, MHIP_R_FLOWDIR);
    c->have[MHIP_R_FLOWDIR] = true;
    c->nodir_valid = true;
    c->flowdir_own = true;
    return MHIP_OK;
}

static int stage_accum(mhip_ctx *c, hipStream_t s, PourLink *pour = nullptr, AccumPrep *prep = nullptr)
{
    MH_ARG(c->have[MHIP_R_FLOWDIR], "ACCUM needs flow directions");
    MH_TRY(ctx_raster(c, MHIP_R_ACCUM));
    MH_TRY(stage_begin(c, MHIP_STAGE_ACCUM, s));
    bool delta_done = false;
    if ((c->ht || c->hb) && c->acc_keep.valid)
        MH_TRY(accum_band_delta_dev(c->r[MHIP_R_FLOWDIR].as<uint8_t>(), c->r[MHIP_R_ACCUM].as<double>(), c->H, c->W, s, c->ht, c->hb, &c->acc_keep, &delta_done));
    c->accum_algorithm = delta_done ? 1 : 0;
    ctx_wrote(c, MHIP_R_ACCUM);
    if (!delta_done)
        MH_TRY(accum_dev(c->r[MHIP_R_FLOWDIR].as<uint8_t>(), c->r[MHIP_R_ACCUM].as<double>(), c->H, c->W, s, c->ht, c->hb, 0, nullptr, pour, nullptr,
                         prep));
    MH_TRY(stage_end(c, MHIP_STAGE_ACCUM, s));
    c->have[MHIP_R_ACCUM] = true;
    return MHIP_OK;
}

static int stage_label(mhip_ctx *c, hipStream_t s)
{
    const int64_t H = c->H, W = c->W, n = H * W;
    MH_ARG(c->have[MHIP_R_DEPTHS] || c->have[MHIP_R_FILLED], "LABEL needs bluespot depths");
    MH_TRY(ctx_raster(c, MHIP_R_LABELS));
    if (!c->tmp_i32.p) MH_TRY(c->tmp_i32.alloc(4 * (size_t)n));
    MH_TRY(stage_begin(c, MHIP_STAGE_LABEL, s));
    if (!c->have[MHIP_R_DEPTHS]) MH_TRY(stage_depths(c, s));
    ctx_wrote(c, MHIP_R_LABELS);
    MH_TRY(ccl8_f32_dev(c->r[MHIP_R_DEPTHS].as<float>(), c->r[MHIP_R_LABELS].as<int32_t>(), c->tmp_i32.as<int32_t>(), H, W,
                        &c->nlabels_raw, s, &c->raw_stats));
    MH_TRY(stage_end(c, MHIP_STAGE_LABEL, s));
    c->have[MHIP_R_LABELS] = true;
    c->labels_components = true;
    c->labels_filtered = false;
    c->nlabels = c->nlabels_raw;
    return MHIP_OK;
}

static int pour_link_buffers(mhip_ctx *c, PourLink *pl, hipStream_t s)
{
    const int64_t H = c->H, W = c->W;
    const int64_t ntiles = cdiv(H, 64) * cdiv(W, 64);
    MH_TRY(c->pp_mask0.alloc(2 * 256 * (size_t)ntiles));
    MH_TRY(c->pp_list.alloc(8 * (size_t)POUR_TILE_CAP * (size_t)ntiles));
    MH_TRY(c->pp_tiles.alloc(12 * (size_t)ntiles));
    MH_TRY(c->pp_misc.alloc(16));
    MH_TRY(c->pp_key.alloc(8 * (size_t)(c->nlabels + 1)));
    MH_HIP(hipMemsetAsync(c->pp_misc.p, 0, 16, s));
    MH_HIP(hipMemsetAsync(c->pp_key.p, 0, 8 * (size_t)(c->nlabels + 1), s));
    pl->dev.mask0 = c->pp_mask0.as<uint16_t>();
    pl->dev.list = c->pp_list.as<uint2>();
    pl->dev.tile_key0 = c->pp_tiles.as<unsigned long long>();
    pl->dev.tile_cnt = reinterpret_cast<uint32_t *>(c->pp_tiles.as<unsigned long long>() + ntiles);
    pl->dev.flags = c->pp_misc.as<uint32_t>() + 1;
    pl->dev.components = c->labels_components ? 1 : 0;
    pl->dev.key = c->pp_key.as<unsigned long long>();
    pl->dev.nlab = (uint32_t)c->nlabels;
    pl->ev = c->ev_cand;
    return MHIP_OK;
}

static int stage_watershed(mhip_ctx *c, hipStream_t s, PourLink *pour = nullptr)
{
    const int64_t H = c->H, W = c->W, n = H * W;
    MH_ARG(c->have[MHIP_R_LABELS] && c->have[MHIP_R_FLOWDIR], "WATERSHED needs labels and flow directions");
    MH_TRY(ctx_ensure_labels_final(c, s));
    MH_TRY(ctx_label_max(c, s));
    MH_TRY(ctx_raster(c, MHIP_R_WATERSHEDS));
    MH_TRY(stage_begin(c, MHIP_STAGE_WATERSHED, s));
    ctx_wrote(c, MHIP_R_WATERSHEDS);
    if (pour) MH_TRY(pour_link_buffers(c, pour, s));
    MH_TRY(watersheds_dev(c->r[MHIP_R_FLOWDIR].as<uint8_t>(), c->r[MHIP_R_WATERSHEDS].as<int32_t>(), H, W, 0, s, false,
                          c->nodir_valid ? c->nodir_cnt.as<unsigned int>() : nullptr, c->r[MHIP_R_LABELS].as<int32_t>(), pour));
    MH_TRY(c->ws_counts.alloc(8 * (size_t)(c->nlabels + 1)));
    MH_TRY(label_count_dev(c->r[MHIP_R_WATERSHEDS].as<int32_t>(), n, c->nlabels, c->ws_counts.as<int64_t>(), s, W));
    MH_TRY(stage_end(c, MHIP_STAGE_WATERSHED, s));
    c->have[MHIP_R_WATERSHEDS] = true;
    c->ws_counts_valid = true;
    return MHIP_OK;
}

static int stage_pourpoints(mhip_ctx *c, hipStream_t s, PourLink *pour = nullptr)
{
    const int64_t H = c->H, W = c->W;
    MH_ARG(c->have[MHIP_R_LABELS] && (c->have[MHIP_R_ACCUM] || c->have[MHIP_R_NOFLAT]),
           "POURPOINTS needs labels and accumulated flow or the no-flats surface");
    MH_TRY(ctx_ensure_labels_final(c, s));
    MH_TRY(ctx_label_max(c, s));
    MH_TRY(c->pour.alloc(sizeof(mhip_index_record) * (size_t)(c->nlabels + 1)));
    double *g = nullptr;
    if (!c->have[MHIP_R_ACCUM]) MH_TRY(ctx_noflat(c, &g));
    MH_TRY(stage_begin(c, MHIP_STAGE_POURPOINTS, s));
    bool from_keys = false;
    if (pour && pour->consumed && c->have[MHIP_R_ACCUM]) {
        uint32_t h[3] = {0, 1, 1};
        MH_HIP(hipMemcpyAsync(h, c->pp_misc.p, 12, hipMemcpyDeviceToHost, s));
        MH_TRY(pour_finish_dev(c->pp_key.as<unsigned long long>(), c->pp_tiles.as<unsigned long long>(), cdiv(H, 64) * cdiv(W, 64), c->nlabels, W,
                               c->pour.as<mhip_index_record>(), s));
        MH_HIP(stream_sync(s));
        from_keys = !h[1] && !h[2];
    }
    c->pour_algorithm = from_keys ? 1 : 0;
    if (from_keys) {
    } else if (c->have[MHIP_R_ACCUM])
        MH_TRY(label_arg_dev(c->r[MHIP_R_ACCUM].as<double>(), c->r[MHIP_R_LABELS].as<int32_t>(), H, W, c->nlabels, true,
                             c->pour.as<mhip_index_record>(), s, c->labels_components));
    else
        MH_TRY(label_arg_dev(g, c->r[MHIP_R_LABELS].as<int32_t>(), H, W, c->nlabels, false, c->pour.as<mhip_index_record>(), s));
    MH_TRY(stage_end(c, MHIP_STAGE_POURPOINTS, s));
    c->pour_valid = true;
    return MHIP_OK;
}

static int label_start_env()
{
    const char *e = dev_env("MHIP_LABEL_START");
    const int v = e ? atoi(e) : LABEL_START_DEFAULT;
    return v >= 0 && v <= 3 ? v : LABEL_START_DEFAULT;
}

extern "C" int mhip_ctx_run(mhip_ctx *c, int mask)
{
    MH_ARG(c, "ctx");
    MH_HIP(hipSetDevice(c->device));
    hipStream_t s = c->stream;
    if (c->nranks > 1 || c->ht || c->hb) {
        MH_ARG((mask & ~(MHIP_STAGE_FLOWDIR | MHIP_STAGE_ACCUM)) == 0,
               "this stage runs through the band entry points on a row band (mhip_ctx_fill_*, mhip_ctx_band_*)");
    }
    const bool serial_env = [] { const char *e = dev_env("MHIP_SERIAL"); return e && e[0] == '1'; }();
    const int side_a = mask & (MHIP_STAGE_NOFLAT | MHIP_STAGE_FLOWDIR | MHIP_STAGE_ACCUM);
    const int side_b = mask & (MHIP_STAGE_LABEL | MHIP_STAGE_WATERSHED);
    const bool overlap = side_a && side_b && !serial_env;
    FillHandover handover;
    FillHandover *const ho =
        ((mask & MHIP_STAGE_FILL) && (mask & MHIP_STAGE_NOFLAT) && c->nranks == 1 && !c->ht && !c->hb && fill_handover_env()) ? &handover : nullptr;
    c->fill_handover = 0;

    if (!overlap) {
        if (mask & MHIP_STAGE_FILL) MH_TRY(stage_fill(c, s, true, ho));
        bool fd_done = false;
        if (mask & MHIP_STAGE_NOFLAT) MH_TRY(stage_noflat(c, s, false, nullptr, (mask & MHIP_STAGE_FLOWDIR) != 0, &fd_done, ho));
        if (mask & MHIP_STAGE_FLOWDIR) MH_TRY(fd_done ? stage_flowdir_fused(c, s) : stage_flowdir(c, s));
        if (mask & MHIP_STAGE_ACCUM) MH_TRY(stage_accum(c, s));
        if (mask & MHIP_STAGE_LABEL) MH_TRY(stage_label(c, s));
        if (mask & MHIP_STAGE_WATERSHED) MH_TRY(stage_watershed(c, s));
        if (mask & MHIP_STAGE_POURPOINTS) MH_TRY(stage_pourpoints(c, s));
        return MHIP_OK;
    }

    StageTimer *t;
    for (int st : {MHIP_STAGE_FILL, MHIP_STAGE_NOFLAT, MHIP_STAGE_FLOWDIR, MHIP_STAGE_ACCUM, MHIP_STAGE_LABEL, MHIP_STAGE_WATERSHED,
                   MHIP_STAGE_POURPOINTS})
        if (mask & st) MH_TRY(ctx_timer(c, st, &t));
    auto side_stream = [&](hipStream_t *st) -> int {
        int least = 0, greatest = 0;
        MH_HIP(hipDeviceGetStreamPriorityRange(&least, &greatest));
        MH_HIP(hipStreamCreateWithPriority(st, hipStreamNonBlocking, least));
        return MHIP_OK;
    };
    if (!c->stream_b) MH_TRY(side_stream(&c->stream_b));
    if (!c->stream_c) MH_TRY(side_stream(&c->stream_c));
    MH_TRY(ctx_fork_join_events(c));
    if (!c->ev_cand) MH_HIP(hipEventCreateWithFlags(&c->ev_cand, hipEventDisableTiming));
    if (!c->ev_prep) MH_HIP(hipEventCreateWithFlags(&c->ev_prep, hipEventDisableTiming));
    hipStream_t sb = c->stream_b;
    const bool do_fill = (mask & MHIP_STAGE_FILL) != 0;
    MH_ARG(c->have[MHIP_R_DEM] || !(mask & (MHIP_STAGE_FILL | MHIP_STAGE_NOFLAT)), "FILL / NOFLAT need the DEM");

    std::promise<int> fill_done, shdg_done, flowdir_ready, label_ready, tail_reached;
    std::future<int> fill_fut = fill_done.get_future(), shdg_fut = shdg_done.get_future(), tail_fut = tail_reached.get_future();
    struct TailCtx {
        mhip_ctx *c;
        std::promise<int> *p;
        FillHandover *ho;
    } tail_ctx{c, &tail_reached, ho};
    StageHook tail_hook;
    tail_hook.arg = &tail_ctx;
    tail_hook.fn = [](void *arg, hipStream_t st) {
        TailCtx *t = static_cast<TailCtx *>(arg);
        ctx_handover_settled(t->c, t->ho);
        t->p->set_value(hipEventRecord(t->c->ev_tail, st) == hipSuccess ? MHIP_OK : MHIP_EHIP);
    };
    std::future<int> flowdir_fut = flowdir_ready.get_future(), label_fut = label_ready.get_future();
    struct CandHand {
        std::promise<int> p;
        std::future<int> f;
        std::atomic<bool> set{false};
    } cand_hand;
    cand_hand.f = cand_hand.p.get_future();
    PourLink pour_link;
    pour_link.arg = &cand_hand;
    pour_link.notify = [](void *a, int v) {
        CandHand *h = static_cast<CandHand *>(a);
        if (!h->set.exchange(true)) h->p.set_value(v);
    };
    pour_link.wait = [](void *a) { return static_cast<CandHand *>(a)->f.get(); };
    static const bool pour_pass = [] { const char *e = dev_env("MHIP_POUR"); return e && std::string(e) == "pass"; }();
    PourLink *const pour = ((mask & MHIP_STAGE_ACCUM) && (mask & MHIP_STAGE_WATERSHED) && (mask & MHIP_STAGE_POURPOINTS) && !pour_pass) ? &pour_link : nullptr;
    AccumPrep acc_prep;
    const bool prep_accum = (mask & MHIP_STAGE_ACCUM) && (mask & (MHIP_STAGE_NOFLAT | MHIP_STAGE_FLOWDIR)) && !c->ht && !c->hb;
    const bool ws_needs_new_flowdir = (mask & MHIP_STAGE_WATERSHED) && (mask & MHIP_STAGE_FLOWDIR);
    int rc_b = MHIP_OK;
    char err_b[512] = "";
    bool shdg_set = false, label_set = false;
    c->side.run([&] {
        rc_b = [&]() -> int {
            MH_HIP(hipSetDevice(c->device));
            int rc_e = MHIP_OK;
            if ((mask & MHIP_STAGE_NOFLAT) && !do_fill) rc_e = short_diag_dev(c->r[MHIP_R_DEM].as<float>(), c->H * c->W, &c->sh, &c->dg, sb);
            if (rc_e != MHIP_OK) snprintf(err_b, sizeof(err_b), "%s", get_error());
            shdg_done.set_value(rc_e);
            shdg_set = true;
            int rc_l = rc_e == MHIP_OK ? fill_fut.get() : rc_e;
            if (rc_l == MHIP_OK) rc_l = tail_fut.get();
            if (rc_l == MHIP_OK && hipStreamWaitEvent(sb, c->ev_tail, 0) != hipSuccess) rc_l = MHIP_EHIP;
            if (rc_l == MHIP_OK && (mask & MHIP_STAGE_LABEL)) rc_l = stage_label(c, sb);
            else if (rc_l == MHIP_OK && do_fill && !c->have[MHIP_R_DEPTHS]) rc_l = stage_depths(c, sb);
            if (rc_l == MHIP_OK && (mask & (MHIP_STAGE_WATERSHED | MHIP_STAGE_POURPOINTS)) && c->have[MHIP_R_LABELS]) {
                rc_l = ctx_ensure_labels_final(c, sb);
                if (rc_l == MHIP_OK) rc_l = ctx_label_max(c, sb);
            }
            if (rc_l == MHIP_OK && hipEventRecord(c->ev_label, sb) != hipSuccess) rc_l = MHIP_EHIP;
            if (rc_l != MHIP_OK && !err_b[0]) snprintf(err_b, sizeof(err_b), "%s", get_error());
            label_ready.set_value(rc_l);
            label_set = true;
            MH_TRY(rc_l);
            hipStream_t sw = sb;
            if (mask & MHIP_STAGE_WATERSHED) {
                sw = c->stream_c;
                MH_HIP(hipStreamWaitEvent(sw, c->ev_label, 0));
                if (ws_needs_new_flowdir) {
                    MH_TRY(flowdir_fut.get());
                    MH_HIP(hipStreamWaitEvent(sw, c->ev_flowdir, 0));
                }
                MH_TRY(stage_watershed(c, sw, pour));
            }
            MH_HIP(hipEventRecord(c->ev_join, sw));
            return MHIP_OK;
        }();
        if (rc_b != MHIP_OK && !err_b[0]) snprintf(err_b, sizeof(err_b), "%s", get_error());
        if (!shdg_set) shdg_done.set_value(rc_b);
        if (!label_set) label_ready.set_value(rc_b);
        pour_link.notify(pour_link.arg, 0);
    });
    int rc_a = MHIP_OK;
    if (do_fill) rc_a = stage_fill(c, s, false, ho);
    if (rc_a == MHIP_OK && hipEventRecord(c->ev_fork, s) != hipSuccess) rc_a = MHIP_EHIP;
    fill_done.set_value(rc_a);
    const int rc_e = shdg_fut.get();
    if (rc_a == MHIP_OK) rc_a = [&]() -> int {
        MH_TRY(rc_e);
        if (do_fill && (mask & MHIP_STAGE_NOFLAT)) {
            if (c->fill_st.have_minmax) short_diag_from_minmax(c->fill_st.dem_min, c->fill_st.dem_max, c->fill_st.dem_nan, &c->sh, &c->dg);
            else MH_TRY(short_diag_dev(c->r[MHIP_R_DEM].as<float>(), c->H * c->W, &c->sh, &c->dg, s));
        }
        if (prep_accum) MH_TRY(accum_prepare_dev(&acc_prep, c->H, c->W, c->stream_c, c->ev_prep));
        const int label_start = label_start_env();
        const bool owed = ho && ho->pending;
        if (label_start == 0 && !owed) tail_hook.fire(s);
        tail_hook.at = label_start;
        const bool armed = label_start == StageHook::TAIL_ROUNDS || label_start == StageHook::FINISH || (label_start == StageHook::FIRST_VISIT && owed);
        bool fd_done = false;
        if (mask & MHIP_STAGE_NOFLAT)
            MH_TRY(stage_noflat(c, s, true, armed ? &tail_hook : nullptr, (mask & MHIP_STAGE_FLOWDIR) != 0, &fd_done, ho));
        if (mask & MHIP_STAGE_FLOWDIR) {
            MH_TRY(fd_done ? stage_flowdir_fused(c, s) : stage_flowdir(c, s));
            MH_HIP(hipEventRecord(c->ev_flowdir, s));
        }
        return MHIP_OK;
    }();
    tail_hook.fire(s);
    flowdir_ready.set_value(rc_a);
    if (rc_a == MHIP_OK && (mask & MHIP_STAGE_ACCUM)) rc_a = stage_accum(c, s, pour, &acc_prep);
    const int rc_l = label_fut.get();
    if (rc_a == MHIP_OK && rc_l == MHIP_OK && (mask & MHIP_STAGE_POURPOINTS)) {
        rc_a = hipStreamWaitEvent(s, c->ev_label, 0) == hipSuccess ? stage_pourpoints(c, s, pour) : MHIP_EHIP;
    }
    c->side.wait();
    if (rc_a != MHIP_OK) return rc_a;
    if (rc_b != MHIP_OK) {
        set_error("%s", err_b);
        return rc_b;
    }
    MH_HIP(hipStreamWaitEvent(s, c->ev_join, 0));
    return MHIP_OK;
}
```

### malstroem_amd/csrc/noflat_geo.hip

```cpp
#include <algorithm>
#include <cmath>
#include <cstdlib>
#include <mutex>
#include <string>
#include <type_traits>
#include <vector>

#include "common.hpp"
#include "handover_addr.hpp"

namespace mh {

namespace {

constexpr int WN = 64;
constexpr int TI = 62;
constexpr uint32_t DINF = 0xE0000000u;
constexpr uint32_t WMAX = 1u << 28;
constexpr uint32_t D_IRR = 0xFFFFFFFFu;
constexpr uint32_t M_NOFLAT = 0xFF00u;
constexpr uint32_t M_IRR = 0xFD00u;
constexpr uint32_t M_WALL = 0xFE00u;
constexpr int DPP_WF_SL1 = 0x130;
constexpr int DPP_WF_SR1 = 0x138;
#ifndef NG_MAXCYC
#define NG_MAXCYC 1
#endif
enum { C_IRREGULAR = 0, C_UNREACHED = 1, C_MISMATCH = 2, C_FATAL = 3, C_PROOF = 4, C_STATS = 8 };
static_assert(WN == ho::WN && TI == ho::TI, "handover_addr.hpp cuts the raster like this file");

__device__ __forceinline__ uint32_t from_left(uint32_t v) { return (uint32_t)__builtin_amdgcn_update_dpp(0, (int)v, DPP_WF_SR1, 0xf, 0xf, true); }
__device__ __forceinline__ uint32_t from_right(uint32_t v) { return (uint32_t)__builtin_amdgcn_update_dpp(0, (int)v, DPP_WF_SL1, 0xf, 0xf, true); }

__device__ __forceinline__ float fleft(float v)
{
    return __int_as_float(__builtin_amdgcn_update_dpp(0x7f800000, __float_as_int(v), DPP_WF_SR1, 0xf, 0xf, false));
}
__device__ __forceinline__ float fright(float v)
{
    return __int_as_float(__builtin_amdgcn_update_dpp(0x7f800000, __float_as_int(v), DPP_WF_SL1, 0xf, 0xf, false));
}

__device__ __forceinline__ uint32_t class_above(float V)
{
    const uint32_t b = __float_as_uint(V), ex = (b >> 23) & 0xffu;
    const uint32_t e = ((b >> 31) && (b & 0x7fffffu) == 0u) ? ex - 1u : ex;
    return (ex == 0u || ex == 255u) ? 255u : e;
}
__device__ __forceinline__ double class_ulp(uint32_t e) { return __longlong_as_double((long long)(e + 1023u - 127u - 52u) << 52); }

struct GeoArgs {
    int64_t H, W;
    int ntr, ntc, nt;
    const float *F;
    uint32_t *d;
    uint32_t *blk;
    uint32_t *hdr;
    uint8_t *mark;
    const int *list;
    const uint32_t *count;
    const uint32_t *tab;
    unsigned long long *counters;
    int maxcyc;
    int append, round_next;
    int *amark;
    int *list_next;
    uint32_t *count_next;
    int fixed_top, fixed_bot;
    const float *ho_dem;
    const uint16_t *ho_bslot;
    const uint32_t *ho_tabV;
    float *ho_F, *ho_depths;
};

template <int R> __device__ __forceinline__ void lds_put(uint32_t addr, uint32_t v) { asm volatile("ds_write_b32 %0, %1 offset:%2" : : "v"(addr), "v"(v), "n"(R) : "memory"); }
template <int R> __device__ __forceinline__ uint32_t lds_get(uint32_t addr)
{
    uint32_t v;
    asm volatile("ds_read_b32 %0, %1 offset:%2" : "=v"(v) : "v"(addr), "n"(R) : "memory");
    return v;
}
__device__ __forceinline__ void lds_wait() { asm volatile("s_waitcnt lgkmcnt(0)" : : : "memory"); }
template <int R0, int N> __device__ __forceinline__ void lds_put_rows(uint32_t addr, const uint32_t (&x)[WN])
{
    if constexpr (N > 0) {
        lds_put<R0 * (WN + 1) * 4>(addr, x[R0]);
        lds_put_rows<R0 + 1, N - 1>(addr, x);
    }
}
template <int R0, int N> __device__ __forceinline__ void lds_get_rows(uint32_t addr, uint32_t (&x)[WN])
{
    if constexpr (N > 0) {
        x[R0] = lds_get<R0 * (WN + 1) * 4>(addr);
        lds_get_rows<R0 + 1, N - 1>(addr, x);
    }
}
template <int C0, int N> __device__ __forceinline__ void lds_get_cols(uint32_t addr, uint32_t (&x)[WN])
{
    if constexpr (N > 0) {
        x[C0] = lds_get<C0 * 4>(addr);
        lds_get_cols<C0 + 1, N - 1>(addr, x);
    }
}
__device__ __forceinline__ void transpose32(uint32_t (&x)[WN], uint32_t scr_b, int lane)
{
    lds_put_rows<0, WN>(scr_b + 4u * lane, x);
    lds_wait();
    lds_get_cols<0, WN>(scr_b + 4u * (WN + 1) * lane, x);
    lds_wait();
#pragma unroll
    for (int c = 0; c < WN; ++c) asm volatile("" : "+v"(x[c]));
}

struct LaneW {
    __device__ __forceinline__ void get(uint32_t mword, const uint32_t *tab_l, uint32_t &s, uint32_t &g) const
    {
        const uint32_t e = (mword >> 8) & 0xffu;
        s = tab_l[e];
        g = tab_l[256 + e];
    }
};

template <bool DOWN, typename WT>
__device__ __forceinline__ void pass(uint32_t (&d)[WN], uint32_t (&ni)[WN], const WT wt, const uint32_t *tab_l, uint32_t &acc_all,
                                     uint32_t &acc_first, uint32_t &acc_last)
{
    constexpr int first = DOWN ? 1 : TI, dir = DOWN ? 1 : -1;
    constexpr int bC = DOWN ? 0 : 4, bL = DOWN ? 7 : 5, bR = DOWN ? 1 : 3;
#pragma unroll
    for (int r = 0; r < WN; ++r) asm volatile("" : "+v"(d[r]), "+v"(ni[r]));
#pragma unroll
    for (int i = 0; i < TI; ++i) {
        const int r = first + dir * i;
        const uint32_t behind = d[r - dir];
        const uint32_t bl = from_left(behind), br = from_right(behind);
        const uint32_t w = ni[r];
        uint32_t S, G;
        wt.get(w, tab_l, S, G);
        const uint32_t c0 = (behind + S) | (uint32_t)__builtin_amdgcn_sbfe((int)w, bC, 1);
        const uint32_t c1 = (bl + G) | (uint32_t)__builtin_amdgcn_sbfe((int)w, bL, 1);
        const uint32_t c2 = (br + G) | (uint32_t)__builtin_amdgcn_sbfe((int)w, bR, 1);
        const uint32_t cu = d[r];
        const uint32_t nv = min(min(c0, c1), min(c2, cu));
        const uint32_t x = nv ^ cu;
        acc_all |= x;
        asm volatile("" : "+v"(acc_all));
        if (r == 1) acc_first |= (w & 0x83u) != 0x83u ? x : 0u;
        if (r == TI) acc_last |= (w & 0x38u) != 0x38u ? x : 0u;
        d[r] = nv;
        __builtin_amdgcn_sched_barrier(0);
    }
}

template <typename WT>
__device__ __forceinline__ void relax(uint32_t (&d)[WN], uint32_t (&ni)[WN], const WT wt, const uint32_t *tab_l, uint32_t scr_b, int lane, int maxcyc,
                                      unsigned &wake, bool &changed, bool &capped, unsigned &cycles)
{
    const uint64_t INNER = ((1ull << TI) - 1) << 1, B1 = 2ull, B62 = 1ull << TI;
    capped = true;
#pragma nounroll
    for (int cyc = 0; cyc < maxcyc; ++cyc) {
        uint64_t chg = 0;
// ... 1003 lines not shown
        if (mine) {
            const double dv = (double)dem[r * W + c];
            double want = dv;
            if (r > 0 && r < H - 1 && inner_col) {
                const double md = fmin(fmin(al, ar), fmin(nl, nr)) + dg;
                const double me = fmin(fmin(a, bl), fmin(br, n)) + sh;
                want = fmax(fmin(md, me), dv);
            }
            const bool halo = (r == 0 && fixed_top) || (r == H - 1 && fixed_bot);
            bad += (b == want || halo) ? 0u : 1u;
            if (STORE) G[r * W + c] = b;
            if (D8) {
                unsigned code;
                if (r == 0 || r == H - 1 || c == 0 || c == W - 1) code = edge_code(r, c, H - 1, W - 1);
                else {
                    code = d8_code(b, a, ar, br, nr, n, nl, bl, al);
                    anynodir |= code == 8u ? 1u : 0u;
                }
                flowdir[r * W + c] = (uint8_t)code;
            }
        }
        a = b;
        b = n;
    }
    if (unreached) atomicAdd(&counters[C_UNREACHED], (unsigned long long)unreached);
    if (bad) atomicAdd(&counters[C_MISMATCH], (unsigned long long)bad);
    if (D8 && __any(anynodir != 0u) && lane == 0) *nodir = 1u;
}

#ifndef NG_FINISH_AHEAD
#define NG_FINISH_AHEAD 1
#endif
#ifndef NG_FINISH_WAVES
#define NG_FINISH_WAVES 8
#endif
#if NG_FINISH_WAVES < 8
#define NG_FINISH_RESIDENCY __attribute__((amdgpu_waves_per_eu(1, NG_FINISH_WAVES)))
#else
#define NG_FINISH_RESIDENCY
#endif
#if NG_FINISH_AHEAD
template <bool STORE>
__device__ __forceinline__ void ng_finish_ahead(const float *__restrict__ F, const uint32_t *__restrict__ d, const float *__restrict__ dem,
                                                double *__restrict__ G, int64_t H, int64_t W, double sh, double dg, double seed_add, int fixed_top,
                                                int fixed_bot, unsigned long long *counters, uint8_t *__restrict__ flowdir, unsigned int *nodir)
{
    const int lane = threadIdx.x & 63, wave = threadIdx.x >> 6;
    const int64_t c = ((int64_t)blockIdx.x * 4 + wave) * TI + lane - 1;
    const int64_t rb = (int64_t)blockIdx.y * FRB;
    const bool col_in = c >= 0 && c < W;
    const int64_t cc = c < 0 ? 0 : (c < W ? c : W - 1);
    const bool mine = lane >= 1 && lane <= TI && col_in;
    const bool inner_col = c > 0 && c + 1 < W;
    const double PINF = __builtin_inf();
    unsigned unreached = 0, bad = 0, anynodir = 0;
    struct Row {
        float f, z;
        uint32_t dd;
    };
    auto load = [&](int64_t r) -> Row {
        const int64_t at = (r < 0 ? 0 : (r < H ? r : H - 1)) * W + cc;
        return Row{F[at], dem[at], d[at]};
    };
    auto value = [&](int64_t r, const Row &x) -> double {
        if (!(r >= 0 && r < H && col_in)) return PINF;
        bool beyond;
        const double v = ng_value(x.f, x.dd, seed_add, &beyond);
        unreached += beyond && mine && r >= rb && r < rb + FRB ? 1u : 0u;
        return v;
    };
    const Row xa = load(rb - 1), xb = load(rb);
    Row x0 = load(rb + 1), x1{0.0f, 0.0f, 0u};
    double a = value(rb - 1, xa), b = value(rb, xb);
    double dvb = (double)xb.z;
    auto row = [&](int i, const Row &xn, Row &xnn, auto more) {
        const int64_t r = rb + i;
        const double dv = dvb;
        if (decltype(more)::value) xnn = load(r + 2);
        const double n = value(r + 1, xn);
        dvb = (double)xn.z;
        asm volatile("" : "+v"(dvb));
        const double al = dleft(a), ar = dright(a), bl = dleft(b), br = dright(b), nl = dleft(n), nr = dright(n);
        if (mine && r < H) {
            double want = dv;
            if (r > 0 && r < H - 1 && inner_col) {
                const double md = fmin(fmin(al, ar), fmin(nl, nr)) + dg;
                const double me = fmin(fmin(a, bl), fmin(br, n)) + sh;
                want = fmax(fmin(md, me), dv);
            }
            const bool halo = (r == 0 && fixed_top) || (r == H - 1 && fixed_bot);
            bad += (b == want || halo) ? 0u : 1u;
            if (STORE) G[r * W + c] = b;
            unsigned code;
            if (r == 0 || r == H - 1 || c == 0 || c == W - 1) code = edge_code(r, c, H - 1, W - 1);
            else {
                code = d8_code(b, a, ar, br, nr, n, nl, bl, al);
                anynodir |= code == 8u ? 1u : 0u;
            }
            flowdir[r * W + c] = (uint8_t)code;
        }
        a = b;
        b = n;
    };
    static_assert(FRB % 2 == 0, "rows in pairs");
    int i = 0;
    for (; i < FRB - 2 && rb + i < H; i += 2) {
        row(i, x0, x1, std::true_type());
        row(i + 1, x1, x0, std::true_type());
    }
    if (i == FRB - 2 && rb + i < H) {
        row(i, x0, x1, std::true_type());
        row(i + 1, x1, x0, std::false_type());
    }
    if (unreached) atomicAdd(&counters[C_UNREACHED], (unsigned long long)unreached);
    if (bad) atomicAdd(&counters[C_MISMATCH], (unsigned long long)bad);
    if (__any(anynodir != 0u) && lane == 0) *nodir = 1u;
}
#define NG_FINISH_AHEAD_KERNEL(STORE)                                                                                                                  \
    template <>                                                                                                                                        \
    __global__ __launch_bounds__(256) NG_FINISH_RESIDENCY void ng_finish_kernel<true, STORE>(                                                          \
        const float *__restrict__ F, const uint32_t *__restrict__ d, const float *__restrict__ dem, double *__restrict__ G, int64_t H, int64_t W,      \
        double sh, double dg, double seed_add, int fixed_top, int fixed_bot, unsigned long long *counters, uint8_t *__restrict__ flowdir,              \
        unsigned int *nodir)                                                                                                                           \
    {                                                                                                                                                  \
        ng_finish_ahead<STORE>(F, d, dem, G, H, W, sh, dg, seed_add, fixed_top, fixed_bot, counters, flowdir, nodir);                                  \
    }
NG_FINISH_AHEAD_KERNEL(true)
NG_FINISH_AHEAD_KERNEL(false)
#undef NG_FINISH_AHEAD_KERNEL
#endif

uint32_t class_weight(double eps, int e)
{
    if (!(eps > 0.0) || std::isinf(eps)) return 0;
    int q;
    const double fr = std::frexp(eps, &q);
    const uint64_t M = (uint64_t)std::ldexp(fr, 53);
    const int k = (e - 127 - 52) - (q - 53);
    if (k <= 24 || k > 52) return 0;
    const uint64_t half = 1ull << (k - 1), rem = M & ((1ull << k) - 1);
    if (rem == half) return 0;
    const uint64_t w = (M >> k) + (rem > half ? 1 : 0);
    return (w >= 1 && w < WMAX) ? (uint32_t)w : 0;
}

}

struct GeoRun::Impl {
    DevBuf ws;
    uint32_t *d_tab = nullptr, *d_any = nullptr, *d_hdr = nullptr, *d_blk = nullptr;
    unsigned long long *d_cnt = nullptr;
    uint8_t *d_mark = nullptr;
    int *d_list = nullptr, *d_list2 = nullptr, *d_amark = nullptr;
    int ntr = 0, ntc = 0, round = 0, used = 0;
    std::vector<std::pair<hipEvent_t, hipEvent_t>> span;
    int span_rounds = 0;
    uint32_t last_count = 0xffffffffu;
    bool light = false;
    int light_from = 0;
    int64_t nt = 0;
    size_t lds = 0;
    int maxcyc = NG_MAXCYC;
    bool debug = false;
    unsigned long long irregular = 0;
};
namespace {
constexpr int MAXR = 8192, BATCH = 32, BATCH_HEAD = 16;
constexpr uint32_t LIGHT_TILES = 6144;
__global__ void ng_mark_row_kernel(uint8_t *mark, int ti, int ntc)
{
    const int tj = blockIdx.x * blockDim.x + threadIdx.x;
    if (tj < ntc) mark[(int64_t)ti * ntc + tj] = 1;
}
}

GeoRun::GeoRun() : impl(new Impl) {}
GeoRun::~GeoRun()
{
    for (auto &e : impl->span) {
        (void)hipEventDestroy(e.first);
        (void)hipEventDestroy(e.second);
    }
    delete impl;
}

int GeoRun::launch_rounds(hipStream_t s, int nb)
{
    {
        Impl &mm = *impl;
        hipEvent_t e0, e1;
        MH_HIP(hipEventCreate(&e0));
        MH_HIP(hipEventCreate(&e1));
        mm.span.emplace_back(e0, e1);
        MH_HIP(hipEventRecord(e0, s));
    }
    struct CloseSpan {
        Impl &m;
        hipStream_t s;
        ~CloseSpan() { (void)hipEventRecord(m.span.back().second, s); }
    } close_span{*impl, s};
    Impl &m = *impl;
    GeoArgs a;
    a.H = H; a.W = W; a.ntr = m.ntr; a.ntc = m.ntc; a.nt = (int)m.nt; a.F = filled; a.d = dist; a.tab = m.d_tab; a.counters = m.d_cnt;
    a.blk = m.d_blk; a.hdr = m.d_hdr; a.mark = m.d_mark; a.list = m.d_list; a.fixed_top = fixed_top; a.fixed_bot = fixed_bot;
    a.append = 0; a.round_next = 0; a.amark = m.d_amark; a.list_next = nullptr; a.count_next = nullptr;
    a.ho_dem = nullptr; a.ho_bslot = nullptr; a.ho_tabV = nullptr; a.ho_F = nullptr; a.ho_depths = nullptr;
    const unsigned grid = (unsigned)std::min<int64_t>((m.nt + 3) / 4, 512);
    for (int k = 0; k < nb; ++k, ++m.round) {
        a.maxcyc = m.maxcyc;
        a.count = m.d_any + m.round;
        if (!m.round && handover && handover->pending) {
            a.ho_dem = handover->dem; a.ho_bslot = handover->bslot; a.ho_tabV = handover->tabV;
            a.ho_F = handover->filled; a.ho_depths = handover->depths;
            hipLaunchKernelGGL(ng_handover_kernel, dim3(grid), dim3(256), m.lds, s, a);
            handover->queued = true;
            (void)hipEventRecord(m.span.back().first, s);
            continue;
        }
        if (!m.round) {
            hipLaunchKernelGGL(ng_first_kernel, dim3(grid), dim3(256), m.lds, s, a);
            (void)hipEventRecord(m.span.back().first, s);
            continue;
        }
        if (!m.light || m.round == m.light_from)
            hipLaunchKernelGGL(ng_compact_kernel, dim3((unsigned)(((m.nt + 7) / 8 + 255) / 256)), dim3(256), 0, s, reinterpret_cast<unsigned long long *>(m.d_mark),
                               (int)((m.nt + 7) / 8), m.d_list, m.d_any + m.round);
        if (m.light) {
            const bool odd = ((m.round - m.light_from) & 1) != 0;
            a.append = 1;
            a.round_next = m.round + 1;
            a.list = odd ? m.d_list2 : m.d_list;
            a.list_next = odd ? m.d_list : m.d_list2;
            a.count_next = m.d_any + m.round + 1;
        }
        if (m.light && tail_hook && tail_hook->at == StageHook::TAIL_ROUNDS)
            hipLaunchKernelGGL(ng_round_w1_kernel, dim3((unsigned)std::min<int64_t>(m.nt, 2048)), dim3(64), (WN * (WN + 1) + 512) * sizeof(uint32_t), s, a);
        else
            hipLaunchKernelGGL(ng_round_kernel, dim3(grid), dim3(256), m.lds, s, a);
    }
    MH_HIP(hipGetLastError());
    return MHIP_OK;
}

int GeoRun::begin(hipStream_t s, bool *applicable, bool *active)
{
    Impl &m = *impl;
    static const bool off = [] { const char *e = dev_env("MHIP_NOFLAT"); return e && std::string(e) == "iterative"; }();
    m.debug = dev_env("MHIP_NG_DEBUG") != nullptr;
    *applicable = false;
    *active = false;
    if (off || !filled || H < 3 || W < 3) return MHIP_OK;
    if (!(sh > 0.0) || !(dg > 0.0) || std::isinf(sh) || std::isinf(dg)) return MHIP_OK;
    std::vector<uint32_t> tab(512, 0u);
    bool any_class = false;
    for (int e = 0; e < 255; ++e) {
        const uint32_t S = class_weight(sh, e), G = class_weight(dg, e);
        if (S && G) {
            tab[e] = S;
            tab[256 + e] = G;
            any_class = true;
        }
    }
    if (!any_class) return MHIP_OK;

    const int64_t n = H * W;
    m.ntr = (int)((H - 2 + TI - 1) / TI);
    m.ntc = (int)((W - 2 + TI - 1) / TI);
    m.nt = (int64_t)m.ntr * m.ntc;
    auto align = [](size_t x) { return (x + 255) & ~size_t(255); };
    const size_t o_d = 0, o_tab = align(o_d + (dist ? 0 : 4 * (size_t)n)), o_cnt = align(o_tab + 2048);
    const size_t o_any = align(o_cnt + 8 * (C_STATS + 128 + 16)), o_mark = align(o_any + 4 * (size_t)(MAXR + BATCH));
    const size_t o_amark = align(o_mark + (size_t)m.nt + 8), o_list = align(o_amark + 4 * (size_t)m.nt), o_list2 = align(o_list + 4 * (size_t)m.nt);
    const size_t o_hdr = align(o_list2 + 4 * (size_t)m.nt), o_blk = align(o_hdr + 4 * (size_t)m.nt);
    MH_TRY(m.ws.alloc(o_blk + 4 * (size_t)m.nt * WN * WN + 256));
    char *b = m.ws.as<char>();
    if (!dist) dist = reinterpret_cast<uint32_t *>(b + o_d);
    m.d_tab = reinterpret_cast<uint32_t *>(b + o_tab);
    m.d_cnt = reinterpret_cast<unsigned long long *>(b + o_cnt);
    m.d_any = reinterpret_cast<uint32_t *>(b + o_any);
    m.d_mark = reinterpret_cast<uint8_t *>(b + o_mark);
    m.d_list = reinterpret_cast<int *>(b + o_list);
    m.d_list2 = reinterpret_cast<int *>(b + o_list2);
    m.d_amark = reinterpret_cast<int *>(b + o_amark);
    m.d_hdr = reinterpret_cast<uint32_t *>(b + o_hdr);
    m.d_blk = reinterpret_cast<uint32_t *>(b + o_blk);
    MH_HIP(hipMemsetAsync(b + o_cnt, 0, o_list - o_cnt, s));
    MH_HIP(hipMemcpyAsync(m.d_tab, tab.data(), 2048, hipMemcpyHostToDevice, s));
    if (fixed_top) MH_HIP(hipMemsetAsync(dist, 0xE0, 4 * (size_t)W, s));
    if (fixed_bot) MH_HIP(hipMemsetAsync(dist + (H - 1) * W, 0xE0, 4 * (size_t)W, s));

    m.lds = (4 * WN * (WN + 1) + 512) * sizeof(uint32_t);
    {
        static std::mutex mu;
        static bool attr_done[64] = {};
        int dev = 0;
        MH_HIP(hipGetDevice(&dev));
        std::lock_guard<std::mutex> lk(mu);
        if (dev < 0 || dev >= 64 || !attr_done[dev]) {
            MH_HIP(hipFuncSetAttribute((const void *)ng_round_kernel, hipFuncAttributeMaxDynamicSharedMemorySize, (int)m.lds));
            MH_HIP(hipFuncSetAttribute((const void *)ng_first_kernel, hipFuncAttributeMaxDynamicSharedMemorySize, (int)m.lds));
            MH_HIP(hipFuncSetAttribute((const void *)ng_handover_kernel, hipFuncAttributeMaxDynamicSharedMemorySize, (int)m.lds));
            if (dev >= 0 && dev < 64) attr_done[dev] = true;
        }
    }
    m.round = 0;
    m.last_count = 0xffffffffu;
    m.used = 0;
    if (handover && handover->pending &&
        !(handover->ntr == m.ntr && handover->ntc == m.ntc && handover->H == H && handover->W == W && handover->filled == filled && handover->dem == dem &&
          !fixed_top && !fixed_bot))
        MH_TRY(fill_handover_complete(handover, s));
    const bool took = handover && handover->pending;
    MH_TRY(launch_rounds(s, 1));
    unsigned long long h_c[5] = {0, 0, 0, 0, 0};
    MH_HIP(hipMemcpyAsync(h_c, m.d_cnt, sizeof(h_c), hipMemcpyDeviceToHost, s));
    MH_HIP(stream_sync(s));
    if (took) {
        if (h_c[C_PROOF] != 0 || dev_env("MHIP_HO_RECHECK") != nullptr) {
            handover->suspect = true;
            m.ws.release();
            return MHIP_OK;
        }
        handover->release();
    }
    m.used = 1;
    m.irregular = h_c[C_IRREGULAR];
    if (h_c[C_FATAL] || (m.irregular && !allow_partial)) {
        if (m.debug) fprintf(stderr, "[noflat geodesic] %llu irregular flat cells, %llu NaN cells: float64 relaxation\n", m.irregular, h_c[C_FATAL]);
        return MHIP_OK;
    }
    *applicable = true;
    *active = true;
    return MHIP_OK;
}

int GeoRun::batch(hipStream_t s, bool *active)
{
    Impl &m = *impl;
    const char *eb = dev_env("MHIP_NG_BATCH");
    const int nb_env = eb && atoi(eb) >= 1 && atoi(eb) <= BATCH ? atoi(eb) : 0;
    for (;;) {
        const int nb = nb_env ? nb_env : (!m.light ? BATCH_HEAD : (m.last_count <= 64 ? 8 : (m.last_count <= 512 ? 16 : BATCH)));
        if (m.round + BATCH > MAXR) {
            set_error("no-flats fill (geodesic) did not converge within %d rounds", MAXR);
            return MHIP_ENOTCONV;
        }
        MH_TRY(launch_rounds(s, nb));
        if (tail_hook) tail_hook->fire_at(StageHook::TAIL_ROUNDS, s);
        uint32_t h_any[BATCH];
        MH_HIP(hipMemcpyAsync(h_any, m.d_any + (m.round - nb), sizeof(uint32_t) * nb, hipMemcpyDeviceToHost, s));
        MH_HIP(stream_sync(s));
        for (int k = 0; k < nb; ++k) {
            if (!h_any[k]) {
                *active = false;
                m.light = false;
                return MHIP_OK;
            }
            ++m.used;
        }
        m.last_count = h_any[nb - 1];
        if (!m.light && h_any[nb - 1] <= LIGHT_TILES) {
            m.light = true;
            m.light_from = m.round;
        }
    }
}

int GeoRun::halo_changed(int side, hipStream_t s)
{
    Impl &m = *impl;
    hipLaunchKernelGGL(ng_mark_row_kernel, dim3((unsigned)((m.ntc + 255) / 256)), dim3(256), 0, s, m.d_mark, side == 0 ? 0 : m.ntr - 1, m.ntc);
    MH_HIP(hipGetLastError());
    return MHIP_OK;
}

int GeoRun::end(hipStream_t s, bool *ok, FillStats *st)
{
    Impl &m = *impl;
    const int64_t n = H * W;
    partial = m.irregular != 0 && allow_partial;
    if (dev_env("MHIP_NG_CORRUPT") && W > 8)
        MH_HIP(hipMemsetAsync(dist + (H / 2) * W + 1, 0x01, 4 * (size_t)(W - 2), s));
    d8_done = false;
    const bool with_d8 = !partial && d8_out && d8_nodir && !fixed_top && !fixed_bot;
    if (tail_hook) tail_hook->fire_at(StageHook::FINISH, s);
    const bool no_store = with_d8 && defer_out;
    out_deferred = false;
    if (no_store)
        hipLaunchKernelGGL((ng_finish_kernel<true, false>), dim3((unsigned)((W + 4 * TI - 1) / (4 * TI)), (unsigned)((H + FRB - 1) / FRB)), dim3(256), 0, s, filled, dist,
                           dem, out, H, W, sh, dg, seed_add, fixed_top, fixed_bot, m.d_cnt, d8_out, d8_nodir);
    else if (with_d8)
        hipLaunchKernelGGL(ng_finish_kernel<true>, dim3((unsigned)((W + 4 * TI - 1) / (4 * TI)), (unsigned)((H + FRB - 1) / FRB)), dim3(256), 0, s, filled, dist, dem,
                           out, H, W, sh, dg, seed_add, fixed_top, fixed_bot, m.d_cnt, d8_out, d8_nodir);
    else if (!partial)
        hipLaunchKernelGGL(ng_finish_kernel<false>, dim3((unsigned)((W + 4 * TI - 1) / (4 * TI)), (unsigned)((H + FRB - 1) / FRB)), dim3(256), 0, s, filled, dist, dem,
                           out, H, W, sh, dg, seed_add, fixed_top, fixed_bot, m.d_cnt, (uint8_t *)nullptr, (unsigned int *)nullptr);
    else
        hipLaunchKernelGGL(ng_assemble_kernel, dim3((unsigned)((n + 1023) / 1024)), dim3(256), 0, s, filled, dist, out, n, seed_add, m.d_cnt);
    MH_HIP(hipGetLastError());
    unsigned long long h_all[C_STATS + 128 + 16];
    MH_HIP(hipMemcpyAsync(h_all, m.d_cnt, sizeof(h_all), hipMemcpyDeviceToHost, s));
    MH_HIP(stream_sync(s));
    if (allow_partial && h_all[C_UNREACHED]) partial = true;
    if (st) {
        *st = FillStats();
        st->geo_irregular = (int64_t)m.irregular;
        st->geo_unreached = (int64_t)h_all[C_UNREACHED];
        st->geo_mismatch = (int64_t)h_all[C_MISMATCH];
        st->rounds = m.used;
        st->tiles = m.nt;
        st->algorithm = partial ? 3 : 2;
        for (auto &e : m.span) {
            float ms = 0;
            if (hipEventElapsedTime(&ms, e.first, e.second) == hipSuccess) st->hot_ms += ms;
            else (void)hipGetLastError();
        }
        st->hot_launches = m.used > 0 ? m.used - 1 : 0;
        for (int k = 0; k < 64; ++k) {
            st->visits += (int64_t)h_all[C_STATS + 2 * k];
            st->cycles += (int64_t)h_all[C_STATS + 2 * k + 1];
        }
    }
    if (m.debug) {
        std::vector<uint32_t> cnt((size_t)m.round);
        MH_HIP(hipMemcpy(cnt.data(), m.d_any, 4 * (size_t)m.round, hipMemcpyDeviceToHost));
        unsigned long long v = 0, cy = 0;
        for (int k = 0; k < 64; ++k) {
            v += h_all[C_STATS + 2 * k];
            cy += h_all[C_STATS + 2 * k + 1];
        }
        fprintf(stderr, "[noflat geodesic] tiles %lld, visits %llu, cycles %llu; tiles per round:", (long long)m.nt, v, cy);
        for (int k = 1; k < m.round && k < 200; ++k) fprintf(stderr, " %u", cnt[k]);
#ifdef NG_PROFILE
        for (int o = 0; o < 2; ++o) {
            const unsigned long long *q = h_all + C_STATS + 128 + 8 * o;
            if (q[0]) fprintf(stderr, "\n[noflat visits, %s] %llu: ticks per visit: setup+issue %.0f, wait for loads %.0f, relax %.0f, store %.0f", o ? "open" : "masked", q[0],
                              (double)q[1] / q[0], (double)q[2] / q[0], (double)q[3] / q[0], (double)q[4] / q[0]);
        }
#endif
        fprintf(stderr, "\n[noflat geodesic] %lld x %lld: rounds %d, unreached %llu, mismatches %llu\n", (long long)H, (long long)W, m.used, h_all[C_UNREACHED],
                h_all[C_MISMATCH]);
    }
    *ok = partial ? true : !(h_all[C_UNREACHED] || h_all[C_MISMATCH]);
    d8_done = with_d8 && !partial && *ok;
    if (no_store) {
        if (d8_done) out_deferred = true;
        else MH_TRY(noflat_assemble_dev(filled, dist, out, n, seed_add, s));
    }
    m.ws.release();
    return MHIP_OK;
}

int noflat_assemble_dev(const float *d_filled, const uint32_t *d_dist, double *d_out, int64_t n, double seed_add, hipStream_t s)
{
    hipLaunchKernelGGL(ng_assemble_kernel, dim3((unsigned)((n + 1023) / 1024)), dim3(256), 0, s, d_filled, d_dist, d_out, n, seed_add,
                       (unsigned long long *)nullptr);
    MH_HIP(hipGetLastError());
    return MHIP_OK;
}

int noflat_verify_dev(const float *d_dem, const double *d_out, int64_t H, int64_t W, double sh, double dg, hipStream_t s, bool *ok, int fixed_top,
                      int fixed_bot)
{
    DevBuf cnt;
    MH_TRY(cnt.alloc(8 * (C_STATS + 128 + 16)));
    MH_HIP(hipMemsetAsync(cnt.p, 0, 8 * (C_STATS + 128), s));
    hipLaunchKernelGGL(ng_verify_kernel, dim3((unsigned)((W + 255) / 256), (unsigned)((H + VRB - 1) / VRB)), dim3(256), 0, s, d_dem, d_out, H, W, sh, dg, fixed_top,
                       fixed_bot, cnt.as<unsigned long long>());
    MH_HIP(hipGetLastError());
    unsigned long long bad = 0;
    MH_HIP(hipMemcpyAsync(&bad, cnt.as<unsigned long long>() + C_MISMATCH, 8, hipMemcpyDeviceToHost, s));
    MH_HIP(stream_sync(s));
    *ok = bad == 0;
    return MHIP_OK;
}

int fill_noflat_geodesic_dev(const float *d_dem, const float *d_filled, double *d_out, int64_t H, int64_t W, double sh, double dg, double seed_add,
                             hipStream_t s, FillStats *st, bool *partial, StageHook *tail_hook, D8Sink *d8, FillHandover *ho)
{
    GeoRun g;
    g.handover = ho;
    g.tail_hook = tail_hook;
    if (d8) {
        g.d8_out = d8->flowdir; g.d8_nodir = d8->nodir; d8->done = false; d8->deferred = false;
        if (d8->dist) g.dist = d8->dist;
        g.defer_out = d8->defer && d8->dist;
    }
    g.dem = d_dem; g.filled = d_filled; g.out = d_out; g.H = H; g.W = W; g.sh = sh; g.dg = dg;
    g.allow_partial = partial != nullptr && seed_add == seed_add && seed_add < 1e300;
    g.seed_add = seed_add;
    bool applicable = false, active = false, ok = false;
    MH_TRY(g.begin(s, &applicable, &active));
    if (ho && ho->pending) {
        const bool again = ho->suspect;
        MH_TRY(fill_handover_complete(ho, s));
        if (again) {
            g.handover = nullptr;
            MH_TRY(g.begin(s, &applicable, &active));
        }
    }
    if (tail_hook) tail_hook->fire_at(StageHook::FIRST_VISIT, s);
    if (!applicable) {
        if (st) st->geo_reject = 1;
        return MHIP_ELIMIT;
    }
    while (active) MH_TRY(g.batch(s, &active));
    MH_TRY(g.end(s, &ok, st));
    if (partial) *partial = g.partial;
    if (d8) { d8->done = g.d8_done; d8->deferred = g.out_deferred; }
    if (!ok && st) st->geo_reject = 2;
    return ok ? MHIP_OK : MHIP_ELIMIT;
}

}
```

### malstroem_amd/csrc/pflood.hip

```cpp
#include "common.hpp"
#include <algorithm>
#include <vector>

namespace mh {

namespace {

constexpr int WN = 64, TI = 62, NC = WN * WN;
constexpr int NBMAX = 1024;
constexpr int HE = 2048;
constexpr int HEU = 2032;
constexpr int SE = 512;
constexpr int SPMAX = 192;
constexpr int LMAX = 256;
constexpr int NSMAX = 128;
constexpr int LH = 1024;
constexpr uint32_t KINV = 0xFFFFFFFFu;
constexpr uint32_t EMPTY = 0xFFFFFFFFu;
constexpr int OCEAN = 255, NOLAB = 254;
constexpr unsigned PF_OV_NB = 1u, PF_OV_PAIRS = 2u, PF_OV_NS = 4u, PF_OV_SPILL = 8u, PF_OV_LINKS = 16u, PF_OV_EMAX = 32u, PF_OV_HALO = 64u;
constexpr uint8_t C_VALID = 1, C_BORDER = 2, C_RING = 4;

struct PfArgs {
    int64_t H, W;
// ... 1352 lines not shown
                const uint32_t lab = a.ringLab[(size_t)tile * 256 + ring_pos(hs == 0 ? 0 : WN - 1, t)];
                if (lab < (uint32_t)NSMAX) atomicMin(&minw[lab], dem_key(filled[r * a.W + c]));
            }
        }
    }
    __syncthreads();
    const int nl0 = a.tileNL0[tile];
    if (t < NSMAX && minw[t] != EMPTY && minw[t] < f32_key(__builtin_inff())) {
        const int i = nl0 + atomicAdd(&s_n, 1);
        if (i < LMAX) a.links[(size_t)tile * LMAX + i] = ((unsigned long long)((uint32_t)t << 16 | 4u << 8 | (uint32_t)OCEAN) << 32) | minw[t];
        else atomicOr(a.flags, PF_OV_HALO);
    }
    __syncthreads();
    const int n = min(nl0 + s_n, LMAX);
    for (int i = n + t; i < LMAX; i += 128) a.links[(size_t)tile * LMAX + i] = ~0ull;
    if (t == 0) a.tileNL[tile] = n;
}

__global__ __launch_bounds__(256) void pf_edge_rows_kernel(PfArgs a, float *__restrict__ filled, int64_t r)
{
    const int64_t c = (int64_t)blockIdx.x * 256 + threadIdx.x;
    if (c >= a.W) return;
    const float d = a.dem[r * a.W + c];
    float f = d;
    if (c > 0 && c < a.W - 1) {
        const int tile = (int)((r - 1) / TI) * a.ntc + (int)((c - 1) / TI);
        const size_t i = (size_t)tile * NBMAX + a.bslot[r * a.W + c];
        const int lab = a.tabL[i];
        const uint32_t lev = max(a.tabV[i], lab == OCEAN ? 0u : a.Lv[(size_t)tile * NSMAX + lab]);
        const uint32_t k = max(dem_key(d), lev);
        f = k >= f32_key(__builtin_inff()) ? __builtin_inff() : key_f32(k);
    }
    filled[r * a.W + c] = f;
}

__global__ void pf_append_row_kernel(unsigned int *mark, int *list, unsigned int *count, int first, int n)
{
    const int i = blockIdx.x * blockDim.x + threadIdx.x;
    if (i < n && atomicExch(&mark[first + i], 1u) == 0u) list[atomicAdd(count, 1u)] = first + i;
}
__global__ void pf_fill_f32_kernel(float *p, int64_t n, float v)
{
    const int64_t i = (int64_t)blockIdx.x * blockDim.x + threadIdx.x;
    if (i < n) p[i] = v;
}
__global__ void pf_raise_level_kernel(PfArgs a, int64_t r, int64_t c, uint32_t key)
{
    const int tile = (int)((r - 1) / TI) * a.ntc + (int)((c - 1) / TI);
    const size_t i = (size_t)tile * NBMAX + min((int)a.bslot[r * a.W + c], NBMAX - 1);
    a.tabV[i] = max(a.tabV[i], key);
}

}

__global__ __launch_bounds__(256) void pf_minmax_kernel(const uint32_t *__restrict__ mm, int64_t npairs, uint32_t *out)
{
    __shared__ uint32_t lo_l[4], hi_l[4];
    uint32_t klo = 0xffffffffu, khi = 0u;
    for (int64_t i = (int64_t)blockIdx.x * 256 + threadIdx.x; i < npairs; i += (int64_t)gridDim.x * 256) {
        const uint2 v = reinterpret_cast<const uint2 *>(mm)[i];
        klo = v.x < klo ? v.x : klo;
        khi = v.y > khi ? v.y : khi;
    }
#pragma unroll
    for (int o = 32; o > 0; o >>= 1) {
        const uint32_t lo2 = (uint32_t)__shfl_xor((int)klo, o), hi2 = (uint32_t)__shfl_xor((int)khi, o);
        klo = lo2 < klo ? lo2 : klo;
        khi = hi2 > khi ? hi2 : khi;
    }
    if ((threadIdx.x & 63) == 0) { lo_l[threadIdx.x >> 6] = klo; hi_l[threadIdx.x >> 6] = khi; }
    __syncthreads();
    if (threadIdx.x == 0) {
        for (int k = 1; k < 4; ++k) { klo = lo_l[k] < klo ? lo_l[k] : klo; khi = hi_l[k] > khi ? hi_l[k] : khi; }
        atomicMin(&out[0], klo);
        atomicMax(&out[1], khi);
    }
}

struct PfRun::Impl {
    DevBuf ws;
    PfArgs a;
    unsigned int *mark = nullptr;
    int *list = nullptr;
    unsigned int *any = nullptr;
    unsigned long long *visits = nullptr;
    unsigned long long *eblk = nullptr;
    int *ecount = nullptr;
    PfQueue *queue = nullptr;
    size_t queue_bytes = 0;
    unsigned int queue_cap = 0;
    unsigned long long queue_visits = 0;
    bool rounds_ran = false;
    bool solved_once = false;
    int64_t ntiles = 0;
    size_t nslots = 0;
    int nbr = 0, nbc = 0, round = 0, launches = 0;
    bool halo_dirty = false;
    uint32_t *mmout = nullptr;
    uint32_t h_mm[2] = {0xffffffffu, 0u};
    bool mm_valid = false;
    hipEvent_t k1_e0 = nullptr, k1_e1 = nullptr;
    ~Impl()
    {
        if (k1_e0) (void)hipEventDestroy(k1_e0);
        if (k1_e1) (void)hipEventDestroy(k1_e1);
    }
};
namespace {
constexpr int PF_MAXR = 1 << 14, PF_BATCH = 32;
}

PfRun::PfRun() : impl(new Impl) {}
PfRun::~PfRun() { delete impl; }

int PfRun::pack(hipStream_t s, int row0, int nrows)
{
    Impl &m = *impl;
    SolveArgs sa = {};
    sa.a = m.a;
    sa.nbr = m.nbr;
    sa.nbc = m.nbc;
    sa.eblk = m.eblk;
    sa.ecount = m.ecount;
    sa.row0 = row0;
    hipLaunchKernelGGL(pf_pack_kernel, dim3((unsigned)m.nbc, (unsigned)nrows), dim3(ST), 0, s, sa);
    MH_HIP(hipGetLastError());
    return MHIP_OK;
}

int PfRun::solve(hipStream_t s)
{
    Impl &m = *impl;
    std::vector<unsigned int> h_cnt(PF_BATCH + 1);
    unsigned int h_flag = 0;
    static const bool use_rounds = [] { const char *e = dev_env("MHIP_PF_SOLVE"); return e && std::string(e) == "rounds"; }();
    if (!use_rounds) {
        const int mode = m.solved_once ? 1 : 0;
        MH_HIP(hipMemsetAsync(m.queue, 0, offsetof(PfQueue, abort), s));
        MH_HIP(hipMemsetAsync(m.queue->slots, 0, (size_t)m.queue_cap * 4, s));
        const int n_init = mode == 0 ? ((m.nbr == 1 || m.nbc == 1) ? m.nbr * m.nbc : 2 * (m.nbc - 1) + 2 * (m.nbr - 1)) : 2 * m.nbc;
        hipLaunchKernelGGL(pf_queue_init_kernel, dim3((unsigned)cdiv(n_init, 256)), dim3(256), 0, s, m.queue, m.mark, m.nbr, m.nbc, mode, 0, m.nbr - 1, m.queue_cap - 1u);
        SolveArgs sa = {};
        sa.a = m.a;
        sa.mark_cur = m.mark;
        sa.visits = m.visits;
        sa.nbr = m.nbr;
        sa.nbc = m.nbc;
        sa.eblk = m.eblk;
        sa.first = dev_env("MHIP_PF_DEBUG") ? 2 : 0;
        hipLaunchKernelGGL(pf_solve_queue_kernel, dim3((unsigned)std::min<size_t>(m.nslots, 768)), dim3(ST), 0, s, sa, m.queue, (const int *)m.ecount);
        MH_HIP(hipGetLastError());
        m.launches += 2;
        unsigned int h_hdr[256 * 4 / 4];
        MH_HIP(hipMemcpyAsync(h_hdr, m.queue, sizeof(h_hdr), hipMemcpyDeviceToHost, s));
        MH_HIP(stream_sync(s));
        const PfQueue *hq = reinterpret_cast<const PfQueue *>(h_hdr);
        const unsigned int h_q[4] = {hq->head, hq->tail, hq->finished, hq->abort};
        h_flag = hq->flags[0];
        overflow = h_flag;
        if (!m.mm_valid) { m.h_mm[0] = hq->mm[0]; m.h_mm[1] = hq->mm[1]; }
        m.mm_valid = true;
        m.solved_once = true;
        if (h_flag) return MHIP_ELIMIT;
        if (dev_env("MHIP_PF_DEBUG")) {
            unsigned int h_d[2] = {0, 0};
            MH_HIP(hipMemcpy(h_d, m.queue->pad2, 8, hipMemcpyDeviceToHost));
            fprintf(stderr, "[pf_solve queue] tickets taken %u, handed out %u, visits finished %u (lowered a seed: %u, LDS sweeps %u), abort %u\n", h_q[0], h_q[1], h_q[2],
                    h_d[0], h_d[1], h_q[3]);
        }
        m.queue_visits += h_q[2];
        if (!h_q[3] && h_q[2] == h_q[1]) return MHIP_OK;
        MH_HIP(hipMemsetAsync(m.mark, 0, m.nslots * 2 * 4, s));
        m.round = 0;
        MH_HIP(hipMemsetAsync(m.any, 0, (size_t)(PF_MAXR + 2) * 4, s));
    }
    m.rounds_ran = true;
    for (;;) {
        if (m.round + PF_BATCH + 1 >= PF_MAXR) {
            set_error("priority-flood seed graph did not converge within %d rounds", PF_MAXR);
            return MHIP_ENOTCONV;
        }
        for (int k = 0; k < PF_BATCH; ++k) {
            const int r = m.round + k;
            SolveArgs sa;
            sa.a = m.a;
            sa.mark_cur = m.mark + (size_t)(r & 1) * m.nslots;
            sa.mark_nxt = m.mark + (size_t)((r + 1) & 1) * m.nslots;
            sa.list_cur = m.list + (size_t)(r & 1) * m.nslots;
            sa.list_nxt = m.list + (size_t)((r + 1) & 1) * m.nslots;
            sa.count_cur = m.any + r;
            sa.count_nxt = m.any + r + 1;
            sa.visits = m.visits;
            sa.nbr = m.nbr;
            sa.nbc = m.nbc;
            sa.first = r == 0;
            sa.eblk = m.eblk;
            sa.row0 = 0;
            hipLaunchKernelGGL(pf_solve_kernel, dim3((unsigned)std::min<size_t>(m.nslots, 768)), dim3(ST), 0, s, sa);
        }
        m.launches += PF_BATCH;
        MH_HIP(hipGetLastError());
        MH_HIP(hipMemcpyAsync(h_cnt.data(), m.any + m.round + 1, sizeof(unsigned int) * PF_BATCH, hipMemcpyDeviceToHost, s));
        MH_HIP(hipMemcpyAsync(&h_flag, m.a.flags, 4, hipMemcpyDeviceToHost, s));
        if (!m.mm_valid) MH_HIP(hipMemcpyAsync(m.h_mm, m.mmout, 8, hipMemcpyDeviceToHost, s));
        MH_HIP(stream_sync(s));
        m.mm_valid = true;
        overflow = h_flag;
        if (h_flag) return MHIP_ELIMIT;
        if (dev_env("MHIP_PF_DEBUG")) {
            fprintf(stderr, "[pf_solve] rounds %d..%d appended work:", m.round, m.round + PF_BATCH - 1);
            for (int k = 0; k < PF_BATCH; ++k) fprintf(stderr, " %u", h_cnt[k]);
            fprintf(stderr, "\n");
        }
        m.round += PF_BATCH;
        for (int k = 0; k < PF_BATCH; ++k)
            if (h_cnt[k] == 0) {
                m.launches -= PF_BATCH - (k + 1);
                return MHIP_OK;
            }
    }
}

int PfRun::publish_edges(hipStream_t s)
{
    Impl &m = *impl;
    const unsigned g = (unsigned)cdiv(W, 256);
    if (fixed_top) hipLaunchKernelGGL(pf_edge_rows_kernel, dim3(g), dim3(256), 0, s, m.a, out, (int64_t)1);
    if (fixed_bot) hipLaunchKernelGGL(pf_edge_rows_kernel, dim3(g), dim3(256), 0, s, m.a, out, H - 2);
    MH_HIP(hipGetLastError());
    return MHIP_OK;
}

int PfRun::begin(hipStream_t s)
{
    Impl &m = *impl;
    if (H < 3 || W < 3) return MHIP_ELIMIT;
    if (fixed_bot && (H - 2) % TI != 0) return MHIP_ELIMIT;
    const int ntr = (int)cdiv(H - 2, TI), ntc = (int)cdiv(W - 2, TI);
    const int64_t ntiles = (int64_t)ntr * ntc;
    const size_t n = (size_t)(H * W);
    auto al = [](size_t x) { return (x + 255) & ~size_t(255); };
    size_t off = 0;
    const size_t o_bslot = off; off = al(off + n * 2);
    const size_t o_tabV = off; off = al(off + (size_t)ntiles * NBMAX * 4);
    const size_t o_tabL = off; off = al(off + (size_t)ntiles * NBMAX);
    const size_t o_ring = off; off = al(off + (size_t)ntiles * 256);
    const size_t o_spill = off; off = al(off + (size_t)ntiles * SPMAX * 8);
    const size_t o_links = off; off = al(off + (size_t)ntiles * LMAX * 8);
    const size_t o_rrec = off; off = al(off + (size_t)ntiles * 256 * 8);
    const size_t o_lv = off; off = al(off + (size_t)ntiles * NSMAX * 4);
    m.nbr = (int)cdiv(ntr, BT);
    m.nbc = (int)cdiv(ntc, BT);
    m.nslots = (size_t)m.nbr * m.nbc;
    m.ntiles = ntiles;
    const size_t o_nb = off; off = al(off + (size_t)ntiles * 4);
    const size_t o_ns = off; off = al(off + (size_t)ntiles * 4);
    const size_t o_nl = off; off = al(off + (size_t)ntiles * 4);
    const size_t o_nl0 = off; off = al(off + (size_t)ntiles * 4);
    const size_t o_ecnt = off; off = al(off + m.nslots * 4);
    const size_t o_act = off; off = al(off + m.nslots * 2 * 4);
    const size_t o_list = off; off = al(off + m.nslots * 2 * 4);
    const size_t o_cnt = off; off = al(off + (size_t)(PF_MAXR + 2) * 4 + 64 + 32 * 8);
    const size_t o_eblk = off; off = al(off + m.nslots * EMAX * 8);
    const size_t o_mm = off; off = al(off + (size_t)ntiles * (NT / 64) * 2 * 4 + 64);
    m.queue_cap = 1024;
    while (m.queue_cap < 2 * m.nslots + 1024) m.queue_cap <<= 1;
    m.queue_bytes = sizeof(PfQueue) + (size_t)m.queue_cap * 4;
    const size_t o_queue = off; off = al(off + m.queue_bytes);
    MH_TRY(m.ws.alloc(off));
    char *b = m.ws.as<char>();
    MH_HIP(hipMemsetAsync(b + o_nb, 0, o_eblk - o_nb, s));
    MH_HIP(hipMemsetAsync(b + o_ring, NOLAB, (size_t)ntiles * 256, s));
    PfArgs &a = m.a;
    a.H = H; a.W = W; a.ntr = ntr; a.ntc = ntc; a.dem = dem; a.fixed_top = fixed_top; a.fixed_bot = fixed_bot; a.stop = 0;
    a.bslot = reinterpret_cast<uint16_t *>(b + o_bslot);
    a.tabV = reinterpret_cast<uint32_t *>(b + o_tabV);
    a.tabL = reinterpret_cast<uint8_t *>(b + o_tabL);
    a.tileNB = reinterpret_cast<int *>(b + o_nb);
    a.ringLab = reinterpret_cast<uint8_t *>(b + o_ring);
    a.spill = reinterpret_cast<unsigned long long *>(b + o_spill);
    a.tileNS = reinterpret_cast<int *>(b + o_ns);
    a.links = reinterpret_cast<unsigned long long *>(b + o_links);
    a.ringRec = reinterpret_cast<unsigned long long *>(b + o_rrec);
    a.tileNL = reinterpret_cast<int *>(b + o_nl);
    a.tileNL0 = reinterpret_cast<int *>(b + o_nl0);
    a.Lv = reinterpret_cast<uint32_t *>(b + o_lv);
    m.any = reinterpret_cast<unsigned int *>(b + o_cnt);
    m.visits = reinterpret_cast<unsigned long long *>(m.any + (PF_MAXR + 2) + 2);
    a.prof = m.visits + 1;
    m.mark = reinterpret_cast<unsigned int *>(b + o_act);
    m.list = reinterpret_cast<int *>(b + o_list);
    m.eblk = reinterpret_cast<unsigned long long *>(b + o_eblk);
    a.mm = reinterpret_cast<uint32_t *>(b + o_mm);
    m.ecount = reinterpret_cast<int *>(b + o_ecnt);
    m.queue = reinterpret_cast<PfQueue *>(b + o_queue);
    a.flags = m.queue->flags;
    m.mmout = m.queue->mm;
    MH_HIP(hipMemsetAsync(&m.queue->abort, 0, 256, s));
    m.solved_once = false;
    m.queue_visits = 0;
    m.rounds_ran = false;
    m.mm_valid = false;
    {
        const uint32_t init[2] = {0xffffffffu, 0u};
        MH_HIP(hipMemcpyAsync(m.mmout, init, sizeof(init), hipMemcpyHostToDevice, s));
    }
    m.round = 0;
    m.halo_dirty = false;
// ... 232 lines not shown
```

### malstroem_amd/csrc/runtime.hip

```cpp
#include <cstdarg>
#include <chrono>
#include <map>
#include <mutex>

#include "common.hpp"

namespace mh {

static thread_local char g_err[512] = "";

void set_error(const char *fmt, ...)
{
    va_list ap;
    va_start(ap, fmt);
    vsnprintf(g_err, sizeof(g_err), fmt, ap);
    va_end(ap);
}
const char *get_error() { return g_err; }
const char *dev_env(const char *name)
{
    static const bool on = [] { const char *e = getenv("MHIP_DEVELOPER"); return e && e[0] == '1'; }();
    return on ? getenv(name) : nullptr;
}

hipError_t stream_sync(hipStream_t s)
{
    static const long spin_us = [] { const char *e = getenv("MALSTROEM_HIP_SPIN_US"); return e ? atol(e) : 3000L; }();
    if (spin_us > 0) {
        const auto t0 = std::chrono::steady_clock::now();
        for (;;) {
            const hipError_t e = hipStreamQuery(s);
            if (e != hipErrorNotReady) return e;
            if (std::chrono::duration_cast<std::chrono::microseconds>(std::chrono::steady_clock::now() - t0).count() > spin_us) break;
        }
    }
    return hipStreamSynchronize(s);
}

namespace {
std::mutex g_pool_mu;
std::multimap<std::pair<int, size_t>, void *> g_pool;
size_t g_pool_bytes = 0;
constexpr size_t POOL_CAP = 96ull << 30;
size_t round_size(size_t n) { return n < (1u << 20) ? ((n + 255) & ~size_t(255)) : ((n + (1u << 20) - 1) & ~size_t((1u << 20) - 1)); }
bool pool_poison()
{
    static const bool on = [] {
        const char *d = getenv("MHIP_DEVELOPER");
        if (!(d && d[0] == '1')) return false;
        const char *e = getenv("MHIP_POOL_POISON");
        return !(e && e[0] == '0');
    }();
    return on;
}
int poison_block(void *p, size_t rs)
{
    MH_HIP(hipMemsetAsync(p, 0xA5, rs, 0));
    MH_HIP(hipStreamSynchronize(0));
    return MHIP_OK;
}
}

int pool_alloc(void **p, size_t bytes)
{
    int dev = 0;
    (void)hipGetDevice(&dev);
    const size_t rs = round_size(bytes);
    {
        std::unique_lock<std::mutex> lk(g_pool_mu);
        auto it = g_pool.find({dev, rs});
        if (it != g_pool.end()) {
            *p = it->second;
            g_pool.erase(it);
            g_pool_bytes -= rs;
            lk.unlock();
            return pool_poison() ? poison_block(*p, rs) : MHIP_OK;
        }
    }
    hipError_t e = hipMalloc(p, rs);
    if (e != hipSuccess) {
        (void)hipGetLastError();
        {
            std::lock_guard<std::mutex> lk(g_pool_mu);
            for (auto &kv : g_pool) (void)hipFree(kv.second);
            g_pool.clear();
            g_pool_bytes = 0;
        }
        e = hipMalloc(p, rs);
    }
    if (e != hipSuccess) {
        *p = nullptr;
        set_error("hipMalloc(%zu) failed: %s", rs, hipGetErrorString(e));
        return MHIP_EHIP;
    }
    return pool_poison() ? poison_block(*p, rs) : MHIP_OK;
}

void pool_free(void *p, size_t bytes)
{
    int dev = 0;
    (void)hipGetDevice(&dev);
    const size_t rs = round_size(bytes);
    std::lock_guard<std::mutex> lk(g_pool_mu);
    if (g_pool_bytes + rs > POOL_CAP) {
        (void)hipFree(p);
        return;
    }
    g_pool.emplace(std::make_pair(dev, rs), p);
    g_pool_bytes += rs;
}

int require_device()
{
    int n = 0;
    if (hipGetDeviceCount(&n) != hipSuccess || n < 1) {
        (void)hipGetLastError();
        set_error("no HIP device available (libmalstroem_hip has no CPU fallback)");
        return MHIP_ENODEV;
    }
    return MHIP_OK;
}

int upload(DevBuf &b, const void *host, size_t bytes, hipStream_t s)
{
    MH_TRY(b.alloc(bytes));
    MH_HIP(hipMemcpyAsync(b.p, host, bytes, hipMemcpyHostToDevice, s));
    return MHIP_OK;
}
int download(void *host, const DevBuf &b, size_t bytes, hipStream_t s)
{
    MH_HIP(hipMemcpyAsync(host, b.p, bytes, hipMemcpyDeviceToHost, s));
    MH_HIP(stream_sync(s));
    return MHIP_OK;
}

int64_t build_rank_lut(const uint8_t *keep, int64_t nlab, std::vector<int32_t> &lut)
{
    lut.assign((size_t)nlab + 1, 0);
    int32_t run = 0;
    for (int64_t l = 1; l <= nlab; ++l)
        if (!keep || keep[l]) lut[(size_t)l] = ++run;
    return run;
}

}

using namespace mh;

extern "C" {

const char *mhip_last_error(void) { return get_error(); }
const char *mhip_version(void) { return "malstroem_hip 0.1 (gfx950)"; }

int mhip_device_count(void)
{
    int n = 0;
    if (hipGetDeviceCount(&n) != hipSuccess) {
        (void)hipGetLastError();
        return 0;
    }
    return n;
}

int mhip_set_device(int device)
{
    MH_TRY(require_device());
    MH_HIP(hipSetDevice(device));
    return MHIP_OK;
}

int mhip_read_bandwidth(int64_t bytes, int32_t reps, double *gbs)
{
    MH_ARG(bytes >= (1 << 20) && reps >= 1 && gbs, "read_bandwidth(bytes >= 1 MiB, reps >= 1, gbs)");
    MH_TRY(require_device());
    return read_bandwidth_dev((size_t)bytes & ~size_t(15), reps, gbs, 0);
}

int mhip_copy_bandwidth(int64_t bytes, int32_t reps, double *gbs)
{
    MH_ARG(bytes >= (1 << 20) && reps >= 1 && gbs, "copy_bandwidth(bytes >= 1 MiB, reps >= 1, gbs)");
    MH_TRY(require_device());
    return copy_bandwidth_dev((size_t)bytes & ~size_t(15), reps, gbs, 0);
}

}
```

Before: 12830 Mcells/s.

## Pipeline host readbacks via pinned mailbox and queue accumulation ahead of noflat sync

```diff
diff --git a/malstroem_amd/csrc/accum.hip b/malstroem_amd/csrc/accum.hip
--- a/malstroem_amd/csrc/accum.hip
+++ b/malstroem_amd/csrc/accum.hip
@@ -757,8 +757,9 @@
 }
 
 int accum_dev(const uint8_t *d_fd, double *d_out, int64_t H, int64_t W, hipStream_t s, int fixed_top, int fixed_bot, int halo_zero,
-              int32_t *d_exit_map, PourLink *pour, AccumKeep *keep, AccumPrep *prep)
-{
+              int32_t *d_exit_map, PourLink *pour, AccumKeep *keep, AccumPrep *prep, DevBuf *hold, AccumSplit *split)
+{
+    if (d_exit_map || keep) split = nullptr;
     const int ntr = (int)cdiv(H, AT), ntc = (int)cdiv(W, AT);
     const int64_t ntiles = (int64_t)ntr * ntc, nnodes = ntiles * NODE_STRIDE;
     if (nnodes >= (int64_t)INT32_MAX || H * W >= (1ll << 37)) {
@@ -770,11 +771,19 @@
     const size_t o_gstate = L.o_gstate, o_inflow = L.o_inflow, o_arrived = L.o_arrived, o_next = L.o_next, o_dst = L.o_dst, o_exit = L.o_exit,
                  o_flags = L.o_flags, o_halo = L.o_halo, o_bexit = L.o_bexit;
     const bool prepared = prep && prep->valid && prep->H == H && prep->W == W && !d_exit_map && !keep;
-    if (prepared) {
+    const bool resume = split && split->queued;
+    if (resume) {
+        buf.p = split->nodes.p; buf.bytes = split->nodes.bytes;
+        split->nodes.p = nullptr; split->nodes.bytes = 0;
+        split->queued = false;
+    } else if (prepared) {
         buf.p = prep->nodes.p; buf.bytes = prep->nodes.bytes;
         prep->nodes.p = nullptr; prep->nodes.bytes = 0;
         prep->valid = false;
-        MH_HIP(hipStreamWaitEvent(s, prep->ready, 0));
+        if (hipEventQuery(prep->ready) != hipSuccess) {
+            (void)hipGetLastError();
+            MH_HIP(hipStreamWaitEvent(s, prep->ready, 0));
+        }
     } else
         MH_TRY(buf.alloc(L.bytes));
     char *b = buf.as<char>();
@@ -789,20 +798,30 @@
     nd.halo_first = d_exit_map ? reinterpret_cast<int32_t *>(b + o_halo) : nullptr;
     nd.bexit = d_exit_map ? reinterpret_cast<int32_t *>(b + o_bexit) : nullptr;
     if (d_exit_map) MH_HIP(hipMemsetAsync(nd.halo_first, 0xff, 8 * (size_t)W, s));
-    if (!prepared) MH_HIP(hipMemsetAsync(nd.inflow, 0, o_next - o_inflow, s));
+    if (!prepared && !resume) MH_HIP(hipMemsetAsync(nd.inflow, 0, o_next - o_inflow, s));
     const unsigned gn = (unsigned)cdiv(nnodes, 256);
     const bool walk_final = (!(fixed_top || fixed_bot) || halo_zero) && (!d_exit_map || halo_zero) && H * W < (int64_t)0x7fffffff;
-    if (walk_final)
-        hipLaunchKernelGGL((accum_tile_kernel<false, false, true>), dim3((unsigned)ntiles), dim3(ATN), 0, s, d_fd, d_out, H, W, ntc, nd, fixed_top, fixed_bot, halo_zero);
-    else if ((fixed_top || fixed_bot) && !halo_zero)
-        hipLaunchKernelGGL((accum_tile_kernel<false, true>), dim3((unsigned)ntiles), dim3(ATN), 0, s, d_fd, d_out, H, W, ntc, nd, fixed_top, fixed_bot, halo_zero);
-    else
-        hipLaunchKernelGGL((accum_tile_kernel<false, false>), dim3((unsigned)ntiles), dim3(ATN), 0, s, d_fd, d_out, H, W, ntc, nd, fixed_top, fixed_bot, halo_zero);
-    hipLaunchKernelGGL(accum_link_kernel, dim3(gn), dim3(256), 0, s, nd, nnodes);
-    if (d_exit_map)
-        hipLaunchKernelGGL(accum_band_exit_kernel, dim3((unsigned)cdiv(2 * W, 256)), dim3(256), 0, s, nd, H, W, ntc, ntiles, fixed_top, fixed_bot, d_exit_map);
-    hipLaunchKernelGGL(accum_mark_kernel, dim3(gn), dim3(256), 0, s, nd, nnodes);
-    hipLaunchKernelGGL(accum_graph_walk_kernel, dim3(gn), dim3(256), 0, s, nd, nnodes);
+    if (!resume) {
+        if (walk_final)
+            hipLaunchKernelGGL((accum_tile_kernel<false, false, true>), dim3((unsigned)ntiles), dim3(ATN), 0, s, d_fd, d_out, H, W, ntc, nd, fixed_top, fixed_bot, halo_zero);
+        else if ((fixed_top || fixed_bot) && !halo_zero)
+            hipLaunchKernelGGL((accum_tile_kernel<false, true>), dim3((unsigned)ntiles), dim3(ATN), 0, s, d_fd, d_out, H, W, ntc, nd, fixed_top, fixed_bot, halo_zero);
+        else
+            hipLaunchKernelGGL((accum_tile_kernel<false, false>), dim3((unsigned)ntiles), dim3(ATN), 0, s, d_fd, d_out, H, W, ntc, nd, fixed_top, fixed_bot, halo_zero);
+        hipLaunchKernelGGL(accum_link_kernel, dim3(gn), dim3(256), 0, s, nd, nnodes);
+        if (d_exit_map)
+            hipLaunchKernelGGL(accum_band_exit_kernel, dim3((unsigned)cdiv(2 * W, 256)), dim3(256), 0, s, nd, H, W, ntc, ntiles, fixed_top, fixed_bot, d_exit_map);
+        hipLaunchKernelGGL(accum_mark_kernel, dim3(gn), dim3(256), 0, s, nd, nnodes);
+        hipLaunchKernelGGL(accum_graph_walk_kernel, dim3(gn), dim3(256), 0, s, nd, nnodes);
+    }
+    if (split && split->queue_only) {
+        MH_HIP(hipGetLastError());
+        split->nodes.release();
+        split->nodes.p = buf.p; split->nodes.bytes = buf.bytes;
+        buf.p = nullptr; buf.bytes = 0;
+        split->queued = true;
+        return MHIP_OK;
+    }
     if (walk_final) {
         PourCandDev pc;
         if (pour && pour->wait && pour->wait(pour->arg) == 1 && pour->dev.key) {
@@ -817,6 +836,12 @@
     else
         hipLaunchKernelGGL((accum_tile_kernel<true, true>), dim3((unsigned)ntiles), dim3(ATN), 0, s, d_fd, d_out, H, W, ntc, nd, fixed_top, fixed_bot, halo_zero);
     MH_HIP(hipGetLastError());
+    if (hold && !keep) {
+        hold->release();
+        hold->p = buf.p; hold->bytes = buf.bytes;
+        buf.p = nullptr; buf.bytes = 0;
+        return MHIP_OK;
+    }
     MH_HIP(stream_sync(s));
     if (keep) {
         keep->valid = false;
diff --git a/malstroem_amd/csrc/common.hpp b/malstroem_amd/csrc/common.hpp
--- a/malstroem_amd/csrc/common.hpp
+++ b/malstroem_amd/csrc/common.hpp
@@ -17,6 +17,34 @@
 const char *get_error();
 const char *dev_env(const char *name);
 hipError_t stream_sync(hipStream_t s);
+hipError_t event_sync(hipEvent_t e);
+
+constexpr int AHEAD_MAILBOX = 1;
+constexpr int AHEAD_STEP_END = 2;
+constexpr int AHEAD_ROUNDS = 4;
+constexpr int AHEAD_FINISH = 8;
+constexpr int AHEAD_ALL = 15;
+constexpr size_t MAIL_PF_HDR = 0, MAIL_GEO_CNT = 1024, MAIL_GEO_ANY = 4096, MAIL_POUR = 4608, MAIL_BYTES = 8192;
+struct Mailbox {
+    char *host = nullptr;
+    hipEvent_t ev = nullptr;
+    int mask = 0;
+    int redone = 0;
+    template <typename T> const T *at(size_t off) const { return reinterpret_cast<const T *>(host + off); }
+    bool on(int bit) const { return (mask & AHEAD_MAILBOX) && (mask & bit); }
+};
+int mailbox_create(Mailbox *mb);
+void mailbox_destroy(Mailbox *mb);
+Mailbox *mailbox();
+struct MailScope {
+    Mailbox *prev;
+    explicit MailScope(Mailbox *mb);
+    ~MailScope();
+    MailScope(const MailScope &) = delete;
+    MailScope &operator=(const MailScope &) = delete;
+};
+int mail_fetch(Mailbox *mb, size_t off, const void *dev, size_t bytes, hipStream_t s);
+inline hipError_t mail_wait(Mailbox *mb) { return event_sync(mb->ev); }
 int require_device();
 
 #define MH_HIP(expr)                                                                             \
@@ -272,6 +300,8 @@
     bool d8_done = false;
     bool defer_out = false;
     bool out_deferred = false;
+    void (*d8_ahead)(void *, hipStream_t) = nullptr;
+    void *d8_ahead_arg = nullptr;
     FillHandover *handover = nullptr;
     struct Impl;
     Impl *impl;
@@ -283,7 +313,8 @@
     int batch(hipStream_t s, bool *active);
     int halo_changed(int side, hipStream_t s);
     int end(hipStream_t s, bool *ok, FillStats *st);
-    int launch_rounds(hipStream_t s, int nb);
+    int launch_rounds(hipStream_t s, int nb, bool keep_open = false);
+    void close_span(hipStream_t s);
 };
 struct D8Sink {
     uint8_t *flowdir = nullptr;
@@ -291,6 +322,8 @@
     bool done = false;
     uint32_t *dist = nullptr;
     bool defer = false, deferred = false;
+    void (*ahead)(void *, hipStream_t) = nullptr;
+    void *ahead_arg = nullptr;
 };
 int noflat_assemble_dev(const float *d_filled, const uint32_t *d_dist, double *d_out, int64_t n, double seed_add, hipStream_t s);
 int fill_noflat_geodesic_dev(const float *d_dem, const float *d_filled, double *d_out, int64_t H, int64_t W, double sh, double dg, double seed_add,
@@ -346,6 +379,10 @@
     int fixed_top = 0, fixed_bot = 0;
     bool valid = false;
 };
+struct AccumSplit {
+    DevBuf nodes;
+    bool queue_only = false, queued = false;
+};
 struct AccumPrep {
     DevBuf nodes;
     int64_t H = 0, W = 0;
@@ -355,7 +392,7 @@
 };
 int accum_prepare_dev(AccumPrep *prep, int64_t H, int64_t W, hipStream_t s, hipEvent_t ready);
 int accum_dev(const uint8_t *d_fd, double *d_out, int64_t H, int64_t W, hipStream_t s, int fixed_top = 0, int fixed_bot = 0, int halo_zero = 0,
-              int32_t *d_exit_map = nullptr, PourLink *pour = nullptr, AccumKeep *keep = nullptr, AccumPrep *prep = nullptr);
+              int32_t *d_exit_map = nullptr, PourLink *pour = nullptr, AccumKeep *keep = nullptr, AccumPrep *prep = nullptr, DevBuf *hold = nullptr, AccumSplit *split = nullptr);
 int accum_band_delta_dev(const uint8_t *d_fd, double *d_out, int64_t H, int64_t W, hipStream_t s, int fixed_top, int fixed_bot, AccumKeep *keep, bool *done);
 int ccl8_f32_dev(const float *d_data, int32_t *d_labels, int32_t *d_tmp, int64_t H, int64_t W, int64_t *nlabels,
                  hipStream_t s, DevBuf *stats_out = nullptr);
diff --git a/malstroem_amd/csrc/ctx.hip b/malstroem_amd/csrc/ctx.hip
--- a/malstroem_amd/csrc/ctx.hip
+++ b/malstroem_amd/csrc/ctx.hip
@@ -231,6 +231,7 @@
     }
     for (hipEvent_t e : {c->ev_fork, c->ev_flowdir, c->ev_join, c->ev_label, c->ev_tail, c->ev_cand, c->ev_prep})
         if (e) (void)hipEventDestroy(e);
+    mailbox_destroy(&c->mail);
     delete c->geo;
     delete c->pf;
     delete c->run[0];
@@ -412,6 +413,8 @@
     else if (k == "fill_algorithm") *value = c->fill_st.algorithm;
     else if (k == "fill_handover") *value = c->fill_handover;
     else if (k == "fill_handover_rechecks") *value = c->fill_handover_rechecks;
+    else if (k == "ahead_mask") *value = c->mail.mask;
+    else if (k == "ahead_redone") *value = c->mail.redone;
     else if (k == "fill_overflow") *value = c->fill_st.overflow;
     else if (k == "fill_launches") *value = c->fill_st.rounds;
     else if (k == "fill_hot_launches") *value = c->fill_st.hot_launches;
diff --git a/malstroem_amd/csrc/ctx.hpp b/malstroem_amd/csrc/ctx.hpp
--- a/malstroem_amd/csrc/ctx.hpp
+++ b/malstroem_amd/csrc/ctx.hpp
@@ -125,6 +125,7 @@
     mh::DevBuf comm_stage, comm_word, comm_flags, comm_stage_b;
     hipStream_t stream_b = nullptr, stream_c = nullptr;
     hipEvent_t ev_fork = nullptr, ev_flowdir = nullptr, ev_join = nullptr, ev_label = nullptr, ev_tail = nullptr;
+    mh::Mailbox mail;
 };
 
 namespace mh {
diff --git a/malstroem_amd/csrc/ctx_run.hip b/malstroem_amd/csrc/ctx_run.hip
--- a/malstroem_amd/csrc/ctx_run.hip
+++ b/malstroem_amd/csrc/ctx_run.hip
@@ -71,8 +71,20 @@
     }
 }
 
+struct AccumAhead {
+    mhip_ctx *c = nullptr;
+    hipStream_t s = nullptr;
+    PourLink *pour = nullptr;
+    AccumPrep *prep = nullptr;
+    AccumSplit split;
+    bool fired = false, accepted = false;
+    int rc = MHIP_OK;
+    ~AccumAhead() { if (split.nodes.p) (void)stream_sync(s); }
+    static void fire(void *arg, hipStream_t st);
+};
+
 static int stage_noflat(mhip_ctx *c, hipStream_t s, bool shdg_done = false, StageHook *tail_hook = nullptr, bool with_flowdir = false,
-                        bool *flowdir_done = nullptr, FillHandover *ho = nullptr)
+                        bool *flowdir_done = nullptr, FillHandover *ho = nullptr, AccumAhead *ahead = nullptr)
 {
     const int64_t H = c->H, W = c->W, n = H * W;
     MH_ARG(c->have[MHIP_R_DEM], "NOFLAT needs the DEM");
@@ -104,13 +116,21 @@
             d8.dist = c->r[MHIP_R_NGDIST].as<uint32_t>();
             d8.defer = true;
         }
+        if (ahead) {
+            d8.ahead = AccumAhead::fire;
+            d8.ahead_arg = ahead;
+        }
     }
     const int rc_nf = fill_noflat_dev(c->r[MHIP_R_DEM].as<float>(), c->r[MHIP_R_NOFLAT].as<double>(), H, W, c->sh, c->dg, s, &st,
                                       c->r[MHIP_R_FILLED].as<float>(), tail_hook, d8.flowdir ? &d8 : nullptr, ho);
     ctx_handover_settled(c, ho);
     MH_TRY(rc_nf);
     if (flowdir_done) *flowdir_done = d8.done;
-    MH_TRY(stage_end(c, MHIP_STAGE_NOFLAT, s));
+    if (ahead && ahead->fired) {
+        MH_TRY(ahead->rc);
+        ahead->accepted = d8.done;
+    }
+    if (!(ahead && ahead->accepted)) MH_TRY(stage_end(c, MHIP_STAGE_NOFLAT, s));
     c->noflat_rounds = st.rounds;
     c->noflat_st = st;
     ctx_wrote(c, MHIP_R_NOFLAT);
@@ -137,10 +157,12 @@
     return MHIP_OK;
 }
 
-static int stage_flowdir_fused(mhip_ctx *c, hipStream_t s)
-{
-    MH_TRY(stage_begin(c, MHIP_STAGE_FLOWDIR, s));
-    MH_TRY(stage_end(c, MHIP_STAGE_FLOWDIR, s));
+static int stage_flowdir_fused(mhip_ctx *c, hipStream_t s, bool events = true)
+{
+    if (events) {
+        MH_TRY(stage_begin(c, MHIP_STAGE_FLOWDIR, s));
+        MH_TRY(stage_end(c, MHIP_STAGE_FLOWDIR, s));
+    }
     ctx_wrote(c, MHIP_R_FLOWDIR);
     c->have[MHIP_R_FLOWDIR] = true;
     c->nodir_valid = true;
@@ -148,10 +170,17 @@
     return MHIP_OK;
 }
 
-static int stage_accum(mhip_ctx *c, hipStream_t s, PourLink *pour = nullptr, AccumPrep *prep = nullptr)
+static int stage_accum(mhip_ctx *c, hipStream_t s, PourLink *pour = nullptr, AccumPrep *prep = nullptr, DevBuf *hold = nullptr, AccumAhead *ahead = nullptr)
 {
     MH_ARG(c->have[MHIP_R_FLOWDIR], "ACCUM needs flow directions");
     MH_TRY(ctx_raster(c, MHIP_R_ACCUM));
+    if (ahead && ahead->accepted && ahead->split.queued) {
+        MH_TRY(accum_dev(c->r[MHIP_R_FLOWDIR].as<uint8_t>(), c->r[MHIP_R_ACCUM].as<double>(), c->H, c->W, s, 0, 0, 0, nullptr, pour, nullptr, prep, hold,
+                         &ahead->split));
+        MH_TRY(stage_end(c, MHIP_STAGE_ACCUM, s));
+        c->have[MHIP_R_ACCUM] = true;
+        return MHIP_OK;
+    }
     MH_TRY(stage_begin(c, MHIP_STAGE_ACCUM, s));
     bool delta_done = false;
     if ((c->ht || c->hb) && c->acc_keep.valid)
@@ -160,10 +189,32 @@
     ctx_wrote(c, MHIP_R_ACCUM);
     if (!delta_done)
         MH_TRY(accum_dev(c->r[MHIP_R_FLOWDIR].as<uint8_t>(), c->r[MHIP_R_ACCUM].as<double>(), c->H, c->W, s, c->ht, c->hb, 0, nullptr, pour, nullptr,
-                         prep));
+                         prep, hold));
     MH_TRY(stage_end(c, MHIP_STAGE_ACCUM, s));
     c->have[MHIP_R_ACCUM] = true;
     return MHIP_OK;
+}
+
+void AccumAhead::fire(void *arg, hipStream_t st)
+{
+    AccumAhead *a = static_cast<AccumAhead *>(arg);
+    mhip_ctx *c = a->c;
+    a->fired = true;
+    a->rc = [&]() -> int {
+        MH_TRY(stage_end(c, MHIP_STAGE_NOFLAT, st));
+        MH_TRY(stage_begin(c, MHIP_STAGE_FLOWDIR, st));
+        MH_TRY(stage_end(c, MHIP_STAGE_FLOWDIR, st));
+        MH_HIP(hipEventRecord(c->ev_flowdir, st));
+        MH_TRY(stage_begin(c, MHIP_STAGE_ACCUM, st));
+        c->accum_algorithm = 0;
+        ctx_wrote(c, MHIP_R_ACCUM);
+        c->have[MHIP_R_ACCUM] = false;
+        a->split.queue_only = true;
+        const int rc = accum_dev(c->r[MHIP_R_FLOWDIR].as<uint8_t>(), c->r[MHIP_R_ACCUM].as<double>(), c->H, c->W, st, 0, 0, 0, nullptr, a->pour, nullptr,
+                                 a->prep, nullptr, &a->split);
+        a->split.queue_only = false;
+        return rc;
+    }();
 }
 
 static int stage_label(mhip_ctx *c, hipStream_t s)
@@ -228,7 +279,7 @@
     return MHIP_OK;
 }
 
-static int stage_pourpoints(mhip_ctx *c, hipStream_t s, PourLink *pour = nullptr)
+static int stage_pourpoints(mhip_ctx *c, hipStream_t s, PourLink *pour = nullptr, DevBuf *held = nullptr)
 {
     const int64_t H = c->H, W = c->W;
     MH_ARG(c->have[MHIP_R_LABELS] && (c->have[MHIP_R_ACCUM] || c->have[MHIP_R_NOFLAT]),
@@ -242,11 +293,19 @@
     bool from_keys = false;
     if (pour && pour->consumed && c->have[MHIP_R_ACCUM]) {
         uint32_t h[3] = {0, 1, 1};
-        MH_HIP(hipMemcpyAsync(h, c->pp_misc.p, 12, hipMemcpyDeviceToHost, s));
+        Mailbox *mb = mailbox();
+        if (mb) MH_TRY(mail_fetch(mb, MAIL_POUR, c->pp_misc.p, 12, s));
+        else MH_HIP(hipMemcpyAsync(h, c->pp_misc.p, 12, hipMemcpyDeviceToHost, s));
         MH_TRY(pour_finish_dev(c->pp_key.as<unsigned long long>(), c->pp_tiles.as<unsigned long long>(), cdiv(H, 64) * cdiv(W, 64), c->nlabels, W,
                                c->pour.as<mhip_index_record>(), s));
-        MH_HIP(stream_sync(s));
+        if (mb) {
+            MH_HIP(mail_wait(mb));
+            memcpy(h, mb->at<uint32_t>(MAIL_POUR), 12);
+            if (held) held->release();
+        } else
+            MH_HIP(stream_sync(s));
         from_keys = !h[1] && !h[2];
+        if (!from_keys && mb) ++mb->redone;
     }
     c->pour_algorithm = from_keys ? 1 : 0;
     if (from_keys) {
@@ -277,6 +336,17 @@
                "this stage runs through the band entry points on a row band (mhip_ctx_fill_*, mhip_ctx_band_*)");
     }
     const bool serial_env = [] { const char *e = dev_env("MHIP_SERIAL"); return e && e[0] == '1'; }();
+    c->mail.mask = 0;
+    c->mail.redone = 0;
+    if (c->nranks == 1 && !c->ht && !c->hb && !serial_env) {
+        const char *e = dev_env("MHIP_AHEAD");
+        const int m = e ? (atoi(e) & AHEAD_ALL) : AHEAD_ALL;
+        if (m & AHEAD_MAILBOX) {
+            MH_TRY(mailbox_create(&c->mail));
+            c->mail.mask = m;
+        }
+    }
+    MailScope mail_scope(&c->mail);
     const int side_a = mask & (MHIP_STAGE_NOFLAT | MHIP_STAGE_FLOWDIR | MHIP_STAGE_ACCUM);
     const int side_b = mask & (MHIP_STAGE_LABEL | MHIP_STAGE_WATERSHED);
     const bool overlap = side_a && side_b && !serial_env;
@@ -349,6 +419,11 @@
     AccumPrep acc_prep;
     const bool prep_accum = (mask & MHIP_STAGE_ACCUM) && (mask & (MHIP_STAGE_NOFLAT | MHIP_STAGE_FLOWDIR)) && !c->ht && !c->hb;
     const bool ws_needs_new_flowdir = (mask & MHIP_STAGE_WATERSHED) && (mask & MHIP_STAGE_FLOWDIR);
+    AccumAhead acc_ahead;
+    acc_ahead.c = c; acc_ahead.s = s; acc_ahead.pour = pour; acc_ahead.prep = &acc_prep;
+    const bool accum_ahead = (mask & MHIP_STAGE_ACCUM) && (mask & MHIP_STAGE_NOFLAT) && (mask & MHIP_STAGE_FLOWDIR) && prep_accum && mailbox() &&
+                             mailbox()->on(AHEAD_FINISH);
+    if (accum_ahead) MH_TRY(ctx_raster(c, MHIP_R_ACCUM));
     int rc_b = MHIP_OK;
     char err_b[512] = "";
     bool shdg_set = false, label_set = false;
@@ -411,19 +486,33 @@
         const bool armed = label_start == StageHook::TAIL_ROUNDS || label_start == StageHook::FINISH || (label_start == StageHook::FIRST_VISIT && owed);
         bool fd_done = false;
         if (mask & MHIP_STAGE_NOFLAT)
-            MH_TRY(stage_noflat(c, s, true, armed ? &tail_hook : nullptr, (mask & MHIP_STAGE_FLOWDIR) != 0, &fd_done, ho));
+            MH_TRY(stage_noflat(c, s, true, armed ? &tail_hook : nullptr, (mask & MHIP_STAGE_FLOWDIR) != 0, &fd_done, ho,
+                                accum_ahead ? &acc_ahead : nullptr));
+        if (acc_ahead.fired && !acc_ahead.accepted && acc_ahead.split.nodes.p) {
+            MH_HIP(stream_sync(s));
+            acc_ahead.split.nodes.release();
+            acc_ahead.split.queued = false;
+            ++c->mail.redone;
+        }
         if (mask & MHIP_STAGE_FLOWDIR) {
-            MH_TRY(fd_done ? stage_flowdir_fused(c, s) : stage_flowdir(c, s));
-            MH_HIP(hipEventRecord(c->ev_flowdir, s));
+            MH_TRY(fd_done ? stage_flowdir_fused(c, s, !acc_ahead.accepted) : stage_flowdir(c, s));
+            if (!acc_ahead.accepted) MH_HIP(hipEventRecord(c->ev_flowdir, s));
         }
         return MHIP_OK;
     }();
     tail_hook.fire(s);
     flowdir_ready.set_value(rc_a);
-    if (rc_a == MHIP_OK && (mask & MHIP_STAGE_ACCUM)) rc_a = stage_accum(c, s, pour, &acc_prep);
+    struct Held {
+        DevBuf b;
+        hipStream_t s;
+        explicit Held(hipStream_t st) : s(st) {}
+        ~Held() { if (b.p) (void)stream_sync(s); }
+    } held(s);
+    const bool end_ahead = pour && mailbox() && mailbox()->on(AHEAD_STEP_END);
+    if (rc_a == MHIP_OK && (mask & MHIP_STAGE_ACCUM)) rc_a = stage_accum(c, s, pour, &acc_prep, end_ahead ? &held.b : nullptr, &acc_ahead);
     const int rc_l = label_fut.get();
     if (rc_a == MHIP_OK && rc_l == MHIP_OK && (mask & MHIP_STAGE_POURPOINTS)) {
-        rc_a = hipStreamWaitEvent(s, c->ev_label, 0) == hipSuccess ? stage_pourpoints(c, s, pour) : MHIP_EHIP;
+        rc_a = hipStreamWaitEvent(s, c->ev_label, 0) == hipSuccess ? stage_pourpoints(c, s, pour, &held.b) : MHIP_EHIP;
     }
     c->side.wait();
     if (rc_a != MHIP_OK) return rc_a;
diff --git a/malstroem_amd/csrc/noflat_geo.hip b/malstroem_amd/csrc/noflat_geo.hip
--- a/malstroem_amd/csrc/noflat_geo.hip
+++ b/malstroem_amd/csrc/noflat_geo.hip
@@ -8,6 +8,7 @@
 
 #include "common.hpp"
 #include "handover_addr.hpp"
+#include "round_pipeline.hpp"
 
 namespace mh {
 
@@ -1317,12 +1318,11 @@
     unsigned long long *d_cnt = nullptr;
     uint8_t *d_mark = nullptr;
     int *d_list = nullptr, *d_list2 = nullptr, *d_amark = nullptr;
-    int ntr = 0, ntc = 0, round = 0, used = 0;
+    int ntr = 0, ntc = 0;
+    RoundPipe rp;
     std::vector<std::pair<hipEvent_t, hipEvent_t>> span;
     int span_rounds = 0;
-    uint32_t last_count = 0xffffffffu;
-    bool light = false;
-    int light_from = 0;
+    bool span_open = false;
     int64_t nt = 0;
     size_t lds = 0;
     int maxcyc = NG_MAXCYC;
@@ -1330,8 +1330,7 @@
     unsigned long long irregular = 0;
 };
 namespace {
-constexpr int MAXR = 8192, BATCH = 32, BATCH_HEAD = 16;
-constexpr uint32_t LIGHT_TILES = 6144;
+constexpr int MAXR = RoundPipe::MAXR, BATCH = RoundPipe::BATCH;
 __global__ void ng_mark_row_kernel(uint8_t *mark, int ti, int ntc)
 {
     const int tj = blockIdx.x * blockDim.x + threadIdx.x;
@@ -1349,21 +1348,23 @@
     delete impl;
 }
 
-int GeoRun::launch_rounds(hipStream_t s, int nb)
-{
-    {
+int GeoRun::launch_rounds(hipStream_t s, int nb, bool keep_open)
+{
+    if (!impl->span_open) {
         Impl &mm = *impl;
         hipEvent_t e0, e1;
         MH_HIP(hipEventCreate(&e0));
         MH_HIP(hipEventCreate(&e1));
         mm.span.emplace_back(e0, e1);
         MH_HIP(hipEventRecord(e0, s));
+        mm.span_open = true;
     }
     struct CloseSpan {
-        Impl &m;
+        GeoRun &g;
         hipStream_t s;
-        ~CloseSpan() { (void)hipEventRecord(m.span.back().second, s); }
-    } close_span{*impl, s};
+        bool keep;
+        ~CloseSpan() { if (!keep) g.close_span(s); }
+    } closer{*this, s, keep_open};
     Impl &m = *impl;
     GeoArgs a;
     a.H = H; a.W = W; a.ntr = m.ntr; a.ntc = m.ntc; a.nt = (int)m.nt; a.F = filled; a.d = dist; a.tab = m.d_tab; a.counters = m.d_cnt;
@@ -1371,10 +1372,10 @@
     a.append = 0; a.round_next = 0; a.amark = m.d_amark; a.list_next = nullptr; a.count_next = nullptr;
     a.ho_dem = nullptr; a.ho_bslot = nullptr; a.ho_tabV = nullptr; a.ho_F = nullptr; a.ho_depths = nullptr;
     const unsigned grid = (unsigned)std::min<int64_t>((m.nt + 3) / 4, 512);
-    for (int k = 0; k < nb; ++k, ++m.round) {
+    for (int k = 0; k < nb; ++k, ++m.rp.round) {
         a.maxcyc = m.maxcyc;
-        a.count = m.d_any + m.round;
-        if (!m.round && handover && handover->pending) {
+        a.count = m.d_any + m.rp.round;
+        if (!m.rp.round && handover && handover->pending) {
             a.ho_dem = handover->dem; a.ho_bslot = handover->bslot; a.ho_tabV = handover->tabV;
             a.ho_F = handover->filled; a.ho_depths = handover->depths;
             hipLaunchKernelGGL(ng_handover_kernel, dim3(grid), dim3(256), m.lds, s, a);
@@ -1382,29 +1383,35 @@
             (void)hipEventRecord(m.span.back().first, s);
             continue;
         }
-        if (!m.round) {
+        if (!m.rp.round) {
             hipLaunchKernelGGL(ng_first_kernel, dim3(grid), dim3(256), m.lds, s, a);
             (void)hipEventRecord(m.span.back().first, s);
             continue;
         }
-        if (!m.light || m.round == m.light_from)
+        if (!m.rp.light || m.rp.round == m.rp.light_from)
             hipLaunchKernelGGL(ng_compact_kernel, dim3((unsigned)(((m.nt + 7) / 8 + 255) / 256)), dim3(256), 0, s, reinterpret_cast<unsigned long long *>(m.d_mark),
-                               (int)((m.nt + 7) / 8), m.d_list, m.d_any + m.round);
-        if (m.light) {
-            const bool odd = ((m.round - m.light_from) & 1) != 0;
+                               (int)((m.nt + 7) / 8), m.d_list, m.d_any + m.rp.round);
+        if (m.rp.light) {
+            const bool odd = ((m.rp.round - m.rp.light_from) & 1) != 0;
             a.append = 1;
-            a.round_next = m.round + 1;
+            a.round_next = m.rp.round + 1;
             a.list = odd ? m.d_list2 : m.d_list;
             a.list_next = odd ? m.d_list : m.d_list2;
-            a.count_next = m.d_any + m.round + 1;
-        }
-        if (m.light && tail_hook && tail_hook->at == StageHook::TAIL_ROUNDS)
+            a.count_next = m.d_any + m.rp.round + 1;
+        }
+        if (m.rp.light && tail_hook && tail_hook->at == StageHook::TAIL_ROUNDS)
             hipLaunchKernelGGL(ng_round_w1_kernel, dim3((unsigned)std::min<int64_t>(m.nt, 2048)), dim3(64), (WN * (WN + 1) + 512) * sizeof(uint32_t), s, a);
         else
             hipLaunchKernelGGL(ng_round_kernel, dim3(grid), dim3(256), m.lds, s, a);
     }
     MH_HIP(hipGetLastError());
     return MHIP_OK;
+}
+
+void GeoRun::close_span(hipStream_t s)
+{
+    if (impl->span_open) (void)hipEventRecord(impl->span.back().second, s);
+    impl->span_open = false;
 }
 
 int GeoRun::begin(hipStream_t s, bool *applicable, bool *active)
@@ -1468,18 +1475,24 @@
             if (dev >= 0 && dev < 64) attr_done[dev] = true;
         }
     }
-    m.round = 0;
-    m.last_count = 0xffffffffu;
-    m.used = 0;
+    m.rp = RoundPipe();
     if (handover && handover->pending &&
         !(handover->ntr == m.ntr && handover->ntc == m.ntc && handover->H == H && handover->W == W && handover->filled == filled && handover->dem == dem &&
           !fixed_top && !fixed_bot))
         MH_TRY(fill_handover_complete(handover, s));
     const bool took = handover && handover->pending;
     MH_TRY(launch_rounds(s, 1));
+    m.rp.seen = m.rp.round;
     unsigned long long h_c[5] = {0, 0, 0, 0, 0};
-    MH_HIP(hipMemcpyAsync(h_c, m.d_cnt, sizeof(h_c), hipMemcpyDeviceToHost, s));
-    MH_HIP(stream_sync(s));
+    Mailbox *mb = mailbox();
+    if (mb) {
+        MH_TRY(mail_fetch(mb, MAIL_GEO_CNT, m.d_cnt, sizeof(h_c), s));
+        MH_HIP(mail_wait(mb));
+        memcpy(h_c, mb->at<unsigned long long>(MAIL_GEO_CNT), sizeof(h_c));
+    } else {
+        MH_HIP(hipMemcpyAsync(h_c, m.d_cnt, sizeof(h_c), hipMemcpyDeviceToHost, s));
+        MH_HIP(stream_sync(s));
+    }
     if (took) {
         if (h_c[C_PROOF] != 0 || dev_env("MHIP_HO_RECHECK") != nullptr) {
             handover->suspect = true;
@@ -1488,7 +1501,7 @@
         }
         handover->release();
     }
-    m.used = 1;
+    m.rp.used = 1;
     m.irregular = h_c[C_IRREGULAR];
     if (h_c[C_FATAL] || (m.irregular && !allow_partial)) {
         if (m.debug) fprintf(stderr, "[noflat geodesic] %llu irregular flat cells, %llu NaN cells: float64 relaxation\n", m.irregular, h_c[C_FATAL]);
@@ -1504,29 +1517,33 @@
     Impl &m = *impl;
     const char *eb = dev_env("MHIP_NG_BATCH");
     const int nb_env = eb && atoi(eb) >= 1 && atoi(eb) <= BATCH ? atoi(eb) : 0;
+    Mailbox *mb = mailbox();
+    const bool pipelined = mb && mb->on(AHEAD_ROUNDS) && !fixed_top && !fixed_bot;
     for (;;) {
-        const int nb = nb_env ? nb_env : (!m.light ? BATCH_HEAD : (m.last_count <= 64 ? 8 : (m.last_count <= 512 ? 16 : BATCH)));
-        if (m.round + BATCH > MAXR) {
+        RoundPipe::Plan p;
+        if (!m.rp.plan(nb_env, pipelined, &p)) {
+            close_span(s);
             set_error("no-flats fill (geodesic) did not converge within %d rounds", MAXR);
             return MHIP_ENOTCONV;
         }
-        MH_TRY(launch_rounds(s, nb));
+        if (p.head) MH_TRY(launch_rounds(s, p.head, p.ahead > 0));
+        if (tail_hook && p.head) tail_hook->fire_at(StageHook::TAIL_ROUNDS, s);
+        const int n = m.rp.round - m.rp.seen;
+        uint32_t h_any[RoundPipe::COUNT_WORDS];
+        const uint32_t *cnt = h_any;
+        if (mb) {
+            MH_TRY(mail_fetch(mb, MAIL_GEO_ANY, m.d_any + m.rp.seen, sizeof(uint32_t) * n, s));
+            cnt = mb->at<uint32_t>(MAIL_GEO_ANY);
+        } else
+            MH_HIP(hipMemcpyAsync(h_any, m.d_any + m.rp.seen, sizeof(uint32_t) * n, hipMemcpyDeviceToHost, s));
+        if (p.ahead) MH_TRY(launch_rounds(s, p.ahead, true));
         if (tail_hook) tail_hook->fire_at(StageHook::TAIL_ROUNDS, s);
-        uint32_t h_any[BATCH];
-        MH_HIP(hipMemcpyAsync(h_any, m.d_any + (m.round - nb), sizeof(uint32_t) * nb, hipMemcpyDeviceToHost, s));
-        MH_HIP(stream_sync(s));
-        for (int k = 0; k < nb; ++k) {
-            if (!h_any[k]) {
-                *active = false;
-                m.light = false;
-                return MHIP_OK;
-            }
-            ++m.used;
-        }
-        m.last_count = h_any[nb - 1];
-        if (!m.light && h_any[nb - 1] <= LIGHT_TILES) {
-            m.light = true;
-            m.light_from = m.round;
+        if (mb) MH_HIP(mail_wait(mb));
+        else MH_HIP(stream_sync(s));
+        if (m.rp.collect(cnt, n)) {
+            close_span(s);
+            *active = false;
+            return MHIP_OK;
         }
     }
 }
@@ -1564,15 +1581,23 @@
         hipLaunchKernelGGL(ng_assemble_kernel, dim3((unsigned)((n + 1023) / 1024)), dim3(256), 0, s, filled, dist, out, n, seed_add, m.d_cnt);
     MH_HIP(hipGetLastError());
     unsigned long long h_all[C_STATS + 128 + 16];
-    MH_HIP(hipMemcpyAsync(h_all, m.d_cnt, sizeof(h_all), hipMemcpyDeviceToHost, s));
-    MH_HIP(stream_sync(s));
+    static_assert(MAIL_GEO_CNT + sizeof(h_all) <= MAIL_GEO_ANY && MAIL_GEO_ANY + 4 * RoundPipe::COUNT_WORDS <= MAIL_POUR, "the mailbox's places");
+    if (Mailbox *mb = mailbox()) {
+        MH_TRY(mail_fetch(mb, MAIL_GEO_CNT, m.d_cnt, sizeof(h_all), s));
+        if (with_d8 && d8_ahead) d8_ahead(d8_ahead_arg, s);
+        MH_HIP(mail_wait(mb));
+        memcpy(h_all, mb->at<unsigned long long>(MAIL_GEO_CNT), sizeof(h_all));
+    } else {
+        MH_HIP(hipMemcpyAsync(h_all, m.d_cnt, sizeof(h_all), hipMemcpyDeviceToHost, s));
+        MH_HIP(stream_sync(s));
+    }
     if (allow_partial && h_all[C_UNREACHED]) partial = true;
     if (st) {
         *st = FillStats();
         st->geo_irregular = (int64_t)m.irregular;
         st->geo_unreached = (int64_t)h_all[C_UNREACHED];
         st->geo_mismatch = (int64_t)h_all[C_MISMATCH];
-        st->rounds = m.used;
+        st->rounds = m.rp.used;
         st->tiles = m.nt;
         st->algorithm = partial ? 3 : 2;
         for (auto &e : m.span) {
@@ -1580,22 +1605,22 @@
             if (hipEventElapsedTime(&ms, e.first, e.second) == hipSuccess) st->hot_ms += ms;
             else (void)hipGetLastError();
         }
-        st->hot_launches = m.used > 0 ? m.used - 1 : 0;
+        st->hot_launches = m.rp.used > 0 ? m.rp.used - 1 : 0;
         for (int k = 0; k < 64; ++k) {
             st->visits += (int64_t)h_all[C_STATS + 2 * k];
             st->cycles += (int64_t)h_all[C_STATS + 2 * k + 1];
         }
     }
     if (m.debug) {
-        std::vector<uint32_t> cnt((size_t)m.round);
-        MH_HIP(hipMemcpy(cnt.data(), m.d_any, 4 * (size_t)m.round, hipMemcpyDeviceToHost));
+        std::vector<uint32_t> cnt((size_t)m.rp.round);
+        MH_HIP(hipMemcpy(cnt.data(), m.d_any, 4 * (size_t)m.rp.round, hipMemcpyDeviceToHost));
         unsigned long long v = 0, cy = 0;
         for (int k = 0; k < 64; ++k) {
             v += h_all[C_STATS + 2 * k];
             cy += h_all[C_STATS + 2 * k + 1];
         }
         fprintf(stderr, "[noflat geodesic] tiles %lld, visits %llu, cycles %llu; tiles per round:", (long long)m.nt, v, cy);
-        for (int k = 1; k < m.round && k < 200; ++k) fprintf(stderr, " %u", cnt[k]);
+        for (int k = 1; k < m.rp.round && k < 200; ++k) fprintf(stderr, " %u", cnt[k]);
 #ifdef NG_PROFILE
         for (int o = 0; o < 2; ++o) {
             const unsigned long long *q = h_all + C_STATS + 128 + 8 * o;
@@ -1603,7 +1628,7 @@
                               (double)q[1] / q[0], (double)q[2] / q[0], (double)q[3] / q[0], (double)q[4] / q[0]);
         }
 #endif
-        fprintf(stderr, "\n[noflat geodesic] %lld x %lld: rounds %d, unreached %llu, mismatches %llu\n", (long long)H, (long long)W, m.used, h_all[C_UNREACHED],
+        fprintf(stderr, "\n[noflat geodesic] %lld x %lld: rounds %d, unreached %llu, mismatches %llu\n", (long long)H, (long long)W, m.rp.used, h_all[C_UNREACHED],
                 h_all[C_MISMATCH]);
     }
     *ok = partial ? true : !(h_all[C_UNREACHED] || h_all[C_MISMATCH]);
@@ -1648,6 +1673,7 @@
     g.tail_hook = tail_hook;
     if (d8) {
         g.d8_out = d8->flowdir; g.d8_nodir = d8->nodir; d8->done = false; d8->deferred = false;
+        g.d8_ahead = d8->ahead; g.d8_ahead_arg = d8->ahead_arg;
         if (d8->dist) g.dist = d8->dist;
         g.defer_out = d8->defer && d8->dist;
     }
diff --git a/malstroem_amd/csrc/pflood.hip b/malstroem_amd/csrc/pflood.hip
--- a/malstroem_amd/csrc/pflood.hip
+++ b/malstroem_amd/csrc/pflood.hip
@@ -1528,8 +1528,15 @@
         MH_HIP(hipGetLastError());
         m.launches += 2;
         unsigned int h_hdr[256 * 4 / 4];
-        MH_HIP(hipMemcpyAsync(h_hdr, m.queue, sizeof(h_hdr), hipMemcpyDeviceToHost, s));
-        MH_HIP(stream_sync(s));
+        static_assert(MAIL_PF_HDR + sizeof(h_hdr) <= MAIL_GEO_CNT, "the mailbox's places");
+        if (Mailbox *mb = mailbox()) {
+            MH_TRY(mail_fetch(mb, MAIL_PF_HDR, m.queue, sizeof(h_hdr), s));
+            MH_HIP(mail_wait(mb));
+            memcpy(h_hdr, mb->at<unsigned int>(MAIL_PF_HDR), sizeof(h_hdr));
+        } else {
+            MH_HIP(hipMemcpyAsync(h_hdr, m.queue, sizeof(h_hdr), hipMemcpyDeviceToHost, s));
+            MH_HIP(stream_sync(s));
+        }
         const PfQueue *hq = reinterpret_cast<const PfQueue *>(h_hdr);
         const unsigned int h_q[4] = {hq->head, hq->tail, hq->finished, hq->abort};
         h_flag = hq->flags[0];
diff --git a/malstroem_amd/csrc/round_pipeline.hpp b/malstroem_amd/csrc/round_pipeline.hpp
--- /dev/null
+++ b/malstroem_amd/csrc/round_pipeline.hpp
@@ -0,0 +1,60 @@
+#pragma once
+#include <cstdint>
+
+namespace mh {
+
+struct RoundPipe {
+    static constexpr int MAXR = 8192;
+    static constexpr int BATCH = 32, BATCH_HEAD = 16;
+    static constexpr int AHEAD = 4;
+    static constexpr uint32_t LIGHT_TILES = 6144;
+    static constexpr int COUNT_WORDS = BATCH + AHEAD;
+
+    int round = 0;
+    int seen = 0;
+    int used = 0;
+    uint32_t last_count = 0xffffffffu;
+    bool light = false;
+    int light_from = 0;
+    int empty_at = -1;
+    int noops = 0;
+
+    struct Plan {
+        int head = 0, ahead = 0;
+    };
+
+    bool plan(int batch_env, bool pipelined, Plan *p) const
+    {
+        const int pend = round - seen;
+        p->head = p->ahead = 0;
+        if (round + BATCH > MAXR) return pend > 0;
+        const int nb = batch_env ? batch_env : (!light ? BATCH_HEAD : (last_count <= 64 ? 8 : (last_count <= 512 ? 16 : BATCH)));
+        p->ahead = (pipelined && light) ? (AHEAD < nb ? AHEAD : nb) : 0;
+        p->head = nb > pend ? nb - pend : 0;
+        if (p->head + p->ahead == 0) p->head = 1;
+        return true;
+    }
+    void launched(int n) { round += n; }
+    bool collect(const uint32_t *cnt, int n)
+    {
+        for (int k = 0; k < n; ++k) {
+            if (!cnt[k]) {
+                empty_at = seen + k;
+                noops = round - empty_at;
+                seen = round;
+                light = false;
+                return true;
+            }
+            ++used;
+        }
+        seen += n;
+        if (n > 0) last_count = cnt[n - 1];
+        if (!light && seen == round && last_count <= LIGHT_TILES) {
+            light = true;
+            light_from = round;
+        }
+        return false;
+    }
+};
+
+}
diff --git a/malstroem_amd/csrc/runtime.hip b/malstroem_amd/csrc/runtime.hip
--- a/malstroem_amd/csrc/runtime.hip
+++ b/malstroem_amd/csrc/runtime.hip
@@ -35,6 +35,49 @@
         }
     }
     return hipStreamSynchronize(s);
+}
+
+hipError_t event_sync(hipEvent_t ev)
+{
+    static const long spin_us = [] { const char *e = getenv("MALSTROEM_HIP_SPIN_US"); return e ? atol(e) : 3000L; }();
+    if (spin_us > 0) {
+        const auto t0 = std::chrono::steady_clock::now();
+        for (;;) {
+            const hipError_t e = hipEventQuery(ev);
+            if (e != hipErrorNotReady) return e;
+            if (std::chrono::duration_cast<std::chrono::microseconds>(std::chrono::steady_clock::now() - t0).count() > spin_us) break;
+        }
+    }
+    return hipEventSynchronize(ev);
+}
+
+int mailbox_create(Mailbox *mb)
+{
+    if (!mb->host) {
+        void *p = nullptr;
+        MH_HIP(hipHostMalloc(&p, MAIL_BYTES, hipHostMallocDefault));
+        memset(p, 0, MAIL_BYTES);
+        mb->host = static_cast<char *>(p);
+    }
+    if (!mb->ev) MH_HIP(hipEventCreateWithFlags(&mb->ev, hipEventDisableTiming));
+    return MHIP_OK;
+}
+void mailbox_destroy(Mailbox *mb)
+{
+    if (mb->ev) (void)hipEventDestroy(mb->ev);
+    if (mb->host) (void)hipHostFree(mb->host);
+    mb->ev = nullptr;
+    mb->host = nullptr;
+}
+static thread_local Mailbox *t_mailbox = nullptr;
+Mailbox *mailbox() { return t_mailbox; }
+MailScope::MailScope(Mailbox *mb) : prev(t_mailbox) { t_mailbox = (mb && mb->host && (mb->mask & AHEAD_MAILBOX)) ? mb : nullptr; }
+MailScope::~MailScope() { t_mailbox = prev; }
+int mail_fetch(Mailbox *mb, size_t off, const void *dev, size_t bytes, hipStream_t s)
+{
+    MH_HIP(hipMemcpyAsync(mb->host + off, dev, bytes, hipMemcpyDeviceToHost, s));
+    MH_HIP(hipEventRecord(mb->ev, s));
+    return MHIP_OK;
 }
 
 namespace {
```

Result: no change. 12860 Mcells/s, median of 6 (+0.3%).
